# Intsights/PySubstringSearch

Hardware: AMD Instinct MI355X
Metric: queries/sec (batched) + index-build GB/s on 512MB chunk, 1/2/4/8 GPU (higher is better)
Workload: dtype u64

## Files before the change

### pysubstringsearch_amd/csrc/common.cpp

```cpp
#include "common.h"
#include "knobs.h"

#include <atomic>
#include <cstring>
#include <cstdio>
#include <cstdlib>
#include <algorithm>
#include <cerrno>
#include <unistd.h>

#include <mutex>
#include <vector>

namespace pss {

static thread_local std::string g_err;

void set_error(const char *fmt, ...)
{
    char buf[1024];
    va_list ap;
    va_start(ap, fmt);
    vsnprintf(buf, sizeof buf, fmt, ap);
    va_end(ap);
    g_err = buf;
}

const std::string &last_error() { return g_err; }

int DevBuf::reserve(size_t bytes)
{
    if (bytes <= cap) return PSS_OK;
    if (p) {
        (void)hipFree(p);
        p = nullptr;
        cap = 0;
    }
    size_t want = round_up(bytes, (size_t)1 << 20);
    hipError_t e = hipMalloc(&p, want);
    if (e != hipSuccess) {
        p = nullptr;
        set_error("hipMalloc(%zu bytes) failed: %s", want, hipGetErrorString(e));
        (void)hipGetLastError();
        return PSS_ENOMEM;
    }
    cap = want;
    return PSS_OK;
}

void DevBuf::release()
{
    if (p) (void)hipFree(p);
    p = nullptr;
    cap = 0;
}

int DeviceCtx::ensure_staging()
{
    if (stage[0]) return PSS_OK;
    PSS_HIP(hipStreamCreateWithFlags(&copy_stream, hipStreamNonBlocking));
    for (int i = 0; i < 2; ++i) {
        PSS_HIP(hipHostMalloc(&stage[i], kStage, hipHostMallocDefault));
        PSS_HIP(hipEventCreateWithFlags(&stage_ev[i], hipEventDisableTiming));
    }
    return PSS_OK;
}

int DeviceCtx::ensure_io_ring()
{
    PSS_TRY(ensure_staging());
    if (io_ring[0]) return PSS_OK;
    for (int i = 0; i < kIoPieces; ++i) {
        PSS_HIP(hipHostMalloc(&io_ring[i], kIoPiece, hipHostMallocPortable));
        PSS_HIP(hipEventCreateWithFlags(&io_ev[i], hipEventDisableTiming));
    }
    return PSS_OK;
}

IoPool &IoPool::get()
{
    static IoPool pool;
    return pool;
}

IoPool::IoPool()
{
    int k = 0;
    if (const char *e = knob("PSS_IO_THREADS")) k = atoi(e);
    if (k <= 0) {
        const unsigned hw = std::thread::hardware_concurrency();
        k = (int)std::min<unsigned>(16u, std::max<unsigned>(8u, hw / 8));
    }
    if (k > 64) k = 64;
    for (int i = 0; i < k; ++i) workers_.emplace_back([this] { run(); });
}

IoPool::~IoPool()
{
    {
        std::lock_guard<std::mutex> lk(mu_);
        stop_ = true;
    }
    cv_.notify_all();
    for (auto &t : workers_)
        if (t.joinable()) t.join();
}

void IoPool::submit(Batch *b, int fd, bool write, void *buf, size_t len, int64_t off, std::atomic<int> *done)
{
    {
        std::lock_guard<std::mutex> lk(b->mu);
        b->submitted += 1;
    }
    if (done) done->store(0, std::memory_order_relaxed);
    {
        std::lock_guard<std::mutex> lk(mu_);
        q_.push_back(Task{b, fd, write, buf, len, off, done});
    }
    cv_.notify_one();
}

void IoPool::submit_copy(Batch *b, void *dst, const void *src, size_t len, std::atomic<int> *done)
{
    submit(b, -2, true, dst, len, (int64_t)reinterpret_cast<intptr_t>(src), done);
}

void IoPool::run()
{
    for (;;) {
        Task t;
        {
            std::unique_lock<std::mutex> lk(mu_);
            cv_.wait(lk, [&] { return stop_ || !q_.empty(); });
            if (q_.empty()) return;
            t = q_.front();
            q_.pop_front();
        }
        int err = 0;
        size_t at = 0;
        uint8_t *p = static_cast<uint8_t *>(t.buf);
        if (t.fd == -2) {
            memcpy(t.buf, reinterpret_cast<const void *>((intptr_t)t.off), t.len);
            at = t.len;
        }
        while (at < t.len) {
            const ssize_t k = t.write ? pwrite(t.fd, p + at, t.len - at, (off_t)(t.off + (int64_t)at))
                                      : pread(t.fd, p + at, t.len - at, (off_t)(t.off + (int64_t)at));
            if (k < 0) {
                if (errno == EINTR) continue;
                err = errno ? errno : EIO;
                break;
            }
            if (k == 0) {
                err = t.write ? ENOSPC : ENODATA;
                break;
            }
            at += (size_t)k;
        }
        {
            std::lock_guard<std::mutex> lk(t.b->mu);
            if (err && !t.b->err) t.b->err = err;
            t.b->finished += 1;
            if (t.done) t.done->store(1, std::memory_order_release);
            t.b->cv.notify_all();
        }
    }
}

int IoPool::wait_all(Batch *b)
{
    std::unique_lock<std::mutex> lk(b->mu);
    b->cv.wait(lk, [&] { return b->finished == b->submitted; });
    return b->err;
}

void IoPool::wait_flag(Batch *b, std::atomic<int> *done)
{
    std::unique_lock<std::mutex> lk(b->mu);
    b->cv.wait(lk, [&] { return done->load(std::memory_order_acquire) != 0; });
}

int DeviceCtx::ensure_search_stage()
{
    if (search_stage) return PSS_OK;
    PSS_HIP(hipHostMalloc(&search_stage, kStageQ + kStageR, hipHostMallocDefault));
    return PSS_OK;
}

void SearchKnobs::load()
{
    *this = SearchKnobs{};
    no_small_path = knob("PSS_NO_SMALL_PATH") != nullptr;
    no_block_path = knob("PSS_NO_BLOCK_PATH") != nullptr;
    no_search_stage = knob("PSS_NO_SEARCH_STAGE") != nullptr;
    wave_search = knob("PSS_WAVE_SEARCH") != nullptr;
    no_group_search = knob("PSS_NO_GROUP_SEARCH") != nullptr;
    no_mid_pipeline = knob("PSS_NO_MID_PIPELINE") != nullptr;
    no_pinned_results = knob("PSS_NO_PINNED_RESULTS") != nullptr;
    small_path_events = knob("PSS_SEARCH_EVENTS") != nullptr;
    if (const char *e = knob("PSS_LANE_SEARCH_MIN")) lane_search_min = strtoull(e, nullptr, 0);
    if (const char *e = knob("PSS_ICASE_SEED_LETTERS")) icase_seed_letters = (uint32_t)std::min(6ul, std::max(1ul, strtoul(e, nullptr, 0)));
    if (const char *e = knob("PSS_RESIDENT_IDLE_US")) resident_idle_us = (uint32_t)strtoul(e, nullptr, 0);
    if (const char *e = knob("PSS_RESIDENT_LIFE_US")) resident_life_us = (uint32_t)strtoul(e, nullptr, 0);
}

static SearchKnobs g_knobs;
static std::once_flag g_knobs_once;
const SearchKnobs &search_knobs()
{
    std::call_once(g_knobs_once, []() { g_knobs.load(); });
    return g_knobs;
}
void reload_search_knobs()
{
    (void)search_knobs();
    g_knobs.load();
}

namespace {
struct PinnedBlock {
    void *p;
    size_t bytes;
};
std::mutex g_pool_mu;
std::vector<PinnedBlock> g_pool;
constexpr size_t kPoolMaxBlocks = 24;
size_t pool_max_bytes()
{
    static const size_t v = [] {
        const char *e = knob("PSS_PINNED_POOL_BYTES");
        return e ? (size_t)strtoull(e, nullptr, 0) : ((size_t)40 << 30);
    }();
    return v;
}
}

void *pinned_pool_alloc(size_t bytes, size_t *granted)
{
    {
        std::lock_guard<std::mutex> lk(g_pool_mu);
        int best = -1;
        for (int i = 0; i < (int)g_pool.size(); ++i)
            if (g_pool[i].bytes >= bytes && (best < 0 || g_pool[i].bytes < g_pool[best].bytes)) best = i;
        if (best >= 0 && g_pool[best].bytes <= 2 * bytes + ((size_t)64 << 20)) {
            PinnedBlock b = g_pool[best];
            g_pool.erase(g_pool.begin() + best);
            *granted = b.bytes;
            return b.p;
        }
    }
    void *p = nullptr;
    const size_t want = round_up(bytes + bytes / 8, (size_t)2 << 20);
    if (hipHostMalloc(&p, want, hipHostMallocPortable) != hipSuccess) {
        (void)hipGetLastError();
        return nullptr;
    }
    *granted = want;
    return p;
}

void pinned_pool_free(void *p, size_t granted)
{
    if (!p) return;
    std::vector<PinnedBlock> drop;
    bool kept = false;
    {
        std::lock_guard<std::mutex> lk(g_pool_mu);
        size_t held = 0;
        for (const auto &b : g_pool) held += b.bytes;
        if (granted <= pool_max_bytes()) {
            while (!g_pool.empty() && (g_pool.size() >= kPoolMaxBlocks || held + granted > pool_max_bytes())) {
                size_t k = 0;
                for (size_t i = 1; i < g_pool.size(); ++i)
                    if (g_pool[i].bytes < g_pool[k].bytes) k = i;
                held -= g_pool[k].bytes;
                drop.push_back(g_pool[k]);
                g_pool.erase(g_pool.begin() + (long)k);
            }
            g_pool.push_back({p, granted});
            kept = true;
        }
    }
    for (auto &b : drop) (void)hipHostFree(b.p);
    if (!kept) (void)hipHostFree(p);
}

void pinned_pool_trim()
{
    std::vector<PinnedBlock> drop;
    {
        std::lock_guard<std::mutex> lk(g_pool_mu);
        drop.swap(g_pool);
    }
    for (auto &b : drop) (void)hipHostFree(b.p);
}

static constexpr int kMaxDevices = 64;
static DeviceCtx g_ctx[kMaxDevices];
static DeviceCtx g_bctx[kMaxDevices];
static std::mutex g_ctx_mu;

static int init_ctx(DeviceCtx &c, int device)
{
    PSS_HIP(hipStreamCreateWithFlags(&c.stream, hipStreamNonBlocking));
    hipDeviceProp_t prop;
    PSS_HIP(hipGetDeviceProperties(&prop, device));
    c.num_cus = prop.multiProcessorCount > 0 ? prop.multiProcessorCount : 256;
    c.pinned_cap = DeviceCtx::kPinnedBytes;
    PSS_HIP(hipHostMalloc(&c.pinned, c.pinned_cap, hipHostMallocDefault));
    PSS_HIP(hipHostGetDevicePointer(&c.pinned_dev, c.pinned, 0));
    for (hipEvent_t &e : c.search_ev) PSS_HIP(hipEventCreate(&e));
    c.device = device;
    return PSS_OK;
}

static int get_ctx_of(DeviceCtx *table, int device, DeviceCtx **out)
{
    int count = 0;
    hipError_t e = hipGetDeviceCount(&count);
    if (e != hipSuccess || count <= 0) {
        (void)hipGetLastError();
        set_error("no usable HIP device (%s); libpss has no CPU fallback",
                  e != hipSuccess ? hipGetErrorString(e) : "device count is 0");
        return PSS_EDEVICE;
    }
    if (device < 0 || device >= count || device >= kMaxDevices) {
        set_error("device %d out of range (have %d)", device, count);
        return PSS_EINVAL;
    }
    PSS_HIP(hipSetDevice(device));
    std::lock_guard<std::mutex> lk(g_ctx_mu);
    DeviceCtx &c = table[device];
    if (c.device < 0) PSS_TRY(init_ctx(c, device));
    *out = &c;
    return PSS_OK;
}

int get_helper_ctx(DeviceCtx *parent, DeviceCtx **out)
{
    if (!parent->helper) {
        DeviceCtx *h = new DeviceCtx();
        const int rc = init_ctx(*h, parent->device);
        if (rc != PSS_OK) {
            delete h;
            return rc;
        }
        parent->helper = h;
    }
    *out = parent->helper;
    return PSS_OK;
}

int get_ctx(int device, DeviceCtx **out) { return get_ctx_of(g_ctx, device, out); }
int get_build_ctx(int device, DeviceCtx **out) { return get_ctx_of(g_bctx, device, out); }

int DeviceCtx::ensure_resident()
{
    if (resident.arena) return PSS_OK;
    PSS_HIP(hipStreamCreateWithFlags(&resident.stream, hipStreamNonBlocking));
    PSS_HIP(hipHostMalloc(&resident.arena, kPinnedBytes, hipHostMallocCoherent | hipHostMallocMapped));
    PSS_HIP(hipHostGetDevicePointer(&resident.arena_dev, resident.arena, 0));
    memset(resident.arena, 0, kPinnedBytes);
    return PSS_OK;
}

void DeviceCtx::Resident::post(const uint8_t *q, uint32_t plen)
{
    ResidentMailbox *mb = reinterpret_cast<ResidentMailbox *>(static_cast<uint8_t *>(arena) + kResidentMailboxOff);
    if (plen != kResidentStop) {
        if (plen <= sizeof mb->post.bytes) {
            memcpy(mb->post.bytes, q, plen);
        } else {
            memcpy(mb->query, q, plen);
            memset(mb->query + plen, 0, 32);
        }
    }
    mb->post.plen = plen;
    ++seq;
    __atomic_store_n(&mb->post.seq_b, seq, __ATOMIC_RELEASE);
    __atomic_store_n(&mb->post.seq_a, seq, __ATOMIC_RELEASE);
}

void DeviceCtx::stop_resident()
{
    if (!resident.running) return;
    resident.post(nullptr, kResidentStop);
    (void)hipStreamSynchronize(resident.stream);
    resident.running = false;
}

const KnobDef kKnobs[] = {
    {"PSS_KEY_CHARS", "0 (chosen)", "1|2|3|5|8|12|16", "builder: force the symbols packed into the initial sort key"},
    {"PSS_KEY_DROP", "-1 (chosen)", "0|1|3|7", "builder: force the low bits of the last key symbol that are left out"},
    {"PSS_NO_SAMPLE", "unset", "1", "builder: size the initial key from symbol counts even for large texts (no sizing sample)"},
    {"PSS_NO_TIES_PASS", "unset", "1", "builder: plain 8-byte-key LSD passes and key comparison in the rerank (no tie flags)"},
    {"PSS_MODE", "chosen", "dense|sparse|text", "builder: how ties are resolved -- doubling over an inverse suffix array, sparse (hash), text rounds"},
    {"PSS_TEXT_ROUNDS", "5", "0|1|2|3", "builder: text rounds at most before the rank rounds"},
    {"PSS_MSD", "-1 (screened)", "0|1|1", "initial sort: never / whenever the key fits the hybrid MSD radix sort (msd_sort.hip)"},
    {"PSS_MSD_LSD", "1", "0|1", "MSD sort: 0 = digits in MSD order with a second histogram pass (rounds 2-5); else LSD order, second pass by look-back"},
    {"PSS_MSD_KEY_CAP", "48", "", "MSD sort: largest key width tried (bits; the element format bounds it further)"},
    {"PSS_MSD_PARTIAL_SYMBOL", "unset", "1", "MSD sort: fill the element with the high bits of one more symbol than fits whole (fewer ties; measured slower on lines)"},
    {"PSS_MSD_NO_FUSE", "unset", "1", "MSD sort: ties flagged in the suffix array instead of emitted from the local sort"},
    {"PSS_MSD_NO_FINISH", "unset", "1", "MSD sort: small tie groups go to the rounds instead of being finished by one more text key after the local sort"},
    {"PSS_MSD_SLOW_LOCAL", "unset", "1", "MSD sort: the general (ballot LSD) local-sort kernel for every tile"},
    {"PSS_MSD_SCATTER", "unset", "1", "MSD sort in MSD order: the 8192-element partition kernels of round 2"},
    {"PSS_SS", "-1 (n >= 2^24, MSD declined)", "0|1", "initial sort: never / whenever the text has the size for it the sample sort over 16-byte elements"},
    {"PSS_SS_SEG", "1", "0", "sample sort: 0 = every tile merge-sorted as one array instead of bucket by bucket"},
    {"PSS_SS_WINDOW_PLAN", "unset", "1", "sample sort: tiles by the window rule of the MSD sort instead of the greedy plan"},
    {"PSS_SS_DEBUG", "unset", "", "sample sort: print where a bucket beyond a tile came from (diagnostic)"},
    {"PSS_NO_PLAN_CACHE", "unset", "1", "builder: forget between chunks which initial sort and alphabet the previous chunk took"},
    {"PSS_NO_PLAN_FRONT", "unset", "1", "builder: remember the sort but not the alphabet (separate alphabet and recode passes)"},
    {"PSS_RLE", "-1 (runs average >= 8 bytes)", "0|1|1", "builder: never / always the run-length path (rle_build.hip)"},
    {"PSS_RLE_SORT", "unset", "1", "run-length path: expansion by the stable radix sort instead of the matrix walk"},
    {"PSS_PERIOD", "-1 (when the text repeats one word)", "0", "builder: 0 = never the closed form for a text that repeats one word"},
    {"PSS_ANCHOR", "-1 (texts of >= 2^20 bytes)", "0|1|1", "builder: never / whenever ties outlive the text rounds the anchor round (anchor_impl.h)"},
    {"PSS_ANCHOR_OMEGA", "0 (as wide as the common prefix allows)", "9|12|17|33", "anchor round: force the window of the minimizers"},
    {"PSS_ANCHOR_MIN_OMEGA", "11", "3|7|9", "anchor round: narrowest window it accepts by itself"},
    {"PSS_ANCHOR_SIDE", "-1 (>= 2^24 bytes, sampled ties show copies)", "0|1", "anchor round: never / always sort the anchors beside the text round (second stream)"},
    {"PSS_ANCHOR_SIDE_PCT", "8", "", "anchor round: share of sampled tied pairs that must be copies for the side line"},
    {"PSS_ANCHOR_CAP_DIV", "5", "3|4", "anchor round: declines above n / this many anchors"},
    {"PSS_NO_PROBE", "unset", "1", "builder: always a text round before the anchor round (no sampling of the ties)"},
    {"PSS_PROBE_SKIP_PCT", "50", "0|20|90", "builder: no text rounds when more than this share of the sampled tied pairs are repeats"},
    {"PSS_NO_MID_TIER", "unset", "1", "rounds: groups above 512 members all take the chained radix sorts"},
    {"PSS_NO_MID_MERGE", "unset", "1", "rounds: groups of 513 .. 4096 members with a crowded bin take the chained sorts (no LDS merge sort)"},
    {"PSS_BIG_MERGE", "-1 (by the average size of the large groups)", "0|1|2", "rounds: groups above 4096 members through the segmented merge sort (2: in text rounds only)"},
    {"PSS_NO_BIG_MERGE", "unset", "", "rounds: overrides PSS_BIG_MERGE"},
    {"PSS_COUNT_SORT", "unset", "1", "rank rounds: groups ranked by counting instead of the merge sort"},
    {"PSS_PERIODIC", "1", "0", "rank rounds: 0 = no periodic keys for the large groups"},
    {"PSS_TIMING", "unset", "", "builder / Writer: per-round and per-stage trace on stderr"},
    {"PSS_DEVICES", "all visible", "0|0,0|0,0,0|all", "devices of Reader(path) / Writer(path) without a device argument: all | comma-separated ordinals"},
    {"PSS_DEVICE", "unset", "", "default device of a process (launchers' LOCAL_RANK etc. are honoured the same way)"},
    {"PSS_IO_THREADS", "8 .. 16 by core count", "2|5", "file path: threads of the I/O pool"},
    {"PSS_INGEST_BLOCK", "32 MiB", "16|40|300", "Writer: size of the direct reads of add_entries_from_file_lines"},
    {"PSS_INGEST_MIN_ROOM", "1 MiB", "1|20", "Writer: room a chunk must have left for one direct read"},
    {"PSS_WRITER_MMAP", "tmpfs: 1, else 0", "0|1", "Writer: records through a shared mapping (1) or pwrite (0)"},
    {"PSS_WRITER_MMAP_MIN", "1 MiB", "16", "Writer: smallest record that goes through the mapping"},
    {"PSS_WRITER_HOST_BUDGET", "8 GiB", "", "multi-device Writer: host text of the chunks in flight (one chunk always goes through)"},
    {"PSS_STRIPES", "8", "", "striped container format 2: stripe files of a Writer"},
    {"PSS_EXPERIMENT_NO_FILE", "unset", "", "measurement only: the record thread copies without writing the file"},
    {"PSS_RESULT_ORDER", "text", "sa", "Reader: 'sa' = the reference's order inside a chunk (suffix-array order of every entry's first hit)"},
    {"PSS_READER_HBM_BUDGET", "whatever hipMalloc grants minus 2 GiB", "", "Reader: suffix arrays beyond this many bytes of HBM stay in pinned host memory"},
    {"PSS_READER_AUTO_RESIDENCY", "1", "", "Reader: 0 = the residency manager never moves a suffix array by itself"},
    {"PSS_NO_KEY_SAMPLES", "unset", "", "Reader: no key-sample table"},
    {"PSS_SAMPLE_SHIFT", "11", "", "Reader: one key sample per 2^shift suffixes"},
    {"PSS_LINE_BLOCK_SHIFT", "8", "6|7|9|10", "Reader: the line index behind entry ids keeps one newline rank per 2^shift bytes of text (6 .. 10)"},
    {"PSS_NO_SMALL_PATH", "unset", "1", "search: no fused single-query kernels"},
    {"PSS_NO_BLOCK_PATH", "unset", "1", "search: small batches one wave per pair instead of one workgroup"},
    {"PSS_NO_SEARCH_STAGE", "unset", "1", "search: no pinned staging of queries and results"},
    {"PSS_WAVE_SEARCH", "unset", "1", "search: interval kernel one wave per pair at every batch size"},
    {"PSS_NO_GROUP_SEARCH", "unset", "1", "search: never 16 lanes per pair"},
    {"PSS_NO_MID_PIPELINE", "unset", "1", "search: always the general multi-kernel pipeline"},
    {"PSS_PINNED_POOL_BYTES", "40 GiB", "", "search: pinned host memory the result pool keeps between batches"},
    {"PSS_NO_PINNED_RESULTS", "unset", "1", "search: large results into pageable memory"},
    {"PSS_LANE_SEARCH_MIN", "8192", "1|100000", "search: pairs from which one lane per pair searches"},
    {"PSS_ICASE_SEED_LETTERS", "5", "1|2|3|4|5|6", "case-insensitive search: ASCII letters of a pattern's seed at most (2^letters spellings probed per pattern and chunk)"},
    {"PSS_SEARCH_EVENTS", "unset", "", "single-query path: HIP events around the fused kernel (fills ms_device; ~4 us per query)"},
    {"PSS_RESIDENT_IDLE_US", "1000", "", "low-latency mode: the resident kernel leaves after this long without a query"},
    {"PSS_RESIDENT_LIFE_US", "50000", "", "low-latency mode: ... and after this long in any case"},
    {"PSS_TRACE_RESIDENT", "unset", "", "libpss_trace.so only: print the resident kernel's phase stamps"},
    {"PSS_RCCL_LIB", "librccl.so of the process", "", "gather inside the C ABI: the RCCL library to load"},
    {"PSS_RCCL_TIMEOUT_MS", "60000", "", "gather inside the C ABI: bound of every wait for the peers"},
};
const int kNumKnobs = (int)(sizeof(kKnobs) / sizeof(kKnobs[0]));

const char *knob(const char *name)
{
    for (int i = 0; i < kNumKnobs; ++i)
        if (strcmp(kKnobs[i].name, name) == 0) return getenv(name);
    static std::atomic<bool> said{false};
    if (!said.exchange(true)) fprintf(stderr, "[pss] %s is not in the switch registry (knobs.h): treated as unset\n", name);
    return nullptr;
}

uint64_t workspace_bytes(int device)
{
    if (device < 0 || device >= kMaxDevices) return 0;
    std::lock_guard<std::mutex> lk(g_ctx_mu);
    uint64_t total = 0;
    for (DeviceCtx *table : {g_ctx, g_bctx}) {
        DeviceCtx &c = table[device];
        if (c.device < 0) continue;
        for (auto &s : c.slot) total += s.cap;
        if (c.helper)
            for (auto &s : c.helper->slot) total += s.cap;
    }
    return total;
}

void trim_all()
{
    std::vector<DeviceCtx *> live;
    {
        std::lock_guard<std::mutex> lk(g_ctx_mu);
        for (DeviceCtx *table : {g_ctx, g_bctx})
            for (int d = 0; d < kMaxDevices; ++d)
                if (table[d].device >= 0) live.push_back(&table[d]);
    }
    for (DeviceCtx *cp : live) {
        {
            DeviceCtx &c = *cp;
            std::lock_guard<std::recursive_mutex> lk2(c.mu);
            (void)hipSetDevice(c.device);
            c.stop_resident();
            for (auto &s : c.slot) s.release();
            if (c.helper)
                for (auto &s : c.helper->slot) s.release();
            c.small_hdr_ready = nullptr;
        }
    }
    pinned_pool_trim();
}

}
```

### pysubstringsearch_amd/csrc/common.h

```cpp
#pragma once
#include <hip/hip_runtime.h>

#include <cstdarg>
#include <cstddef>
#include <cstdint>
#include <cstdio>
#include <cstdlib>
#include <cstring>
#include <atomic>
#include <condition_variable>
#include <deque>
#include <mutex>
#include <string>
#include <thread>
#include <vector>

#include "../../include/pss.h"

#include "knobs.h"

namespace pss {

void set_error(const char *fmt, ...);
const std::string &last_error();

#define PSS_HIP(expr)                                                                   \
    do {                                                                                \
        hipError_t _e = (expr);                                                         \
        if (_e != hipSuccess) {                                                         \
            pss::set_error("%s failed: %s (%s:%d)", #expr, hipGetErrorString(_e), __FILE__, __LINE__); \
            return (_e == hipErrorOutOfMemory) ? PSS_ENOMEM : PSS_EDEVICE;              \
        }                                                                               \
    } while (0)

#define PSS_TRY(expr)               \
    do {                            \
        int _rc = (expr);           \
        if (_rc != PSS_OK) return _rc; \
    } while (0)

struct DevBuf {
    void *p = nullptr;
    size_t cap = 0;
    int reserve(size_t bytes);
    void release();
    template <typename T> T *as() const { return static_cast<T *>(p); }
};

struct SearchKnobs {
    bool no_small_path = false;
    bool no_block_path = false;
    bool no_search_stage = false;
    bool wave_search = false;
    bool no_group_search = false;
    bool no_mid_pipeline = false;
    bool no_pinned_results = false;
    bool small_path_events = false;
    uint64_t lane_search_min = 8192;
    uint32_t icase_seed_letters = 5;
    uint32_t resident_idle_us = 1000;
    uint32_t resident_life_us = 50000;
    void load();
};
const SearchKnobs &search_knobs();
void reload_search_knobs();

void *pinned_pool_alloc(size_t bytes, size_t *granted);
void pinned_pool_free(void *p, size_t granted);
void pinned_pool_trim();

struct ResidentMailbox {
    struct Post {
        volatile uint32_t seq_a;
        volatile uint32_t plen;
        uint8_t bytes[52];
        volatile uint32_t seq_b;
    } post;
    uint8_t query[256 + 64];
    volatile uint64_t done_seq_echo;
    volatile uint32_t exited;
    volatile uint32_t closing;
    volatile uint32_t pad2[12];
};
static_assert(offsetof(ResidentMailbox, done_seq_echo) % 8 == 0, "one aligned 8-byte store");
static inline uint32_t resident_query_checksum(const uint8_t *q, uint32_t plen)
{
    uint32_t h = 0x811C9DC5u ^ plen;
    for (uint32_t i = 0; i < plen; i += 8) {
        uint64_t w = 0;
        for (uint32_t k = 0; k < 8 && i + k < plen; ++k) w |= (uint64_t)q[i + k] << (8 * k);
        h = (h ^ (uint32_t)w) * 0x01000193u;
        h = (h ^ (uint32_t)(w >> 32)) * 0x01000193u;
    }
    return h;
}
static_assert(sizeof(ResidentMailbox::Post) == 64, "the posted line is one cache line");
constexpr uint32_t kResidentStop = 0xffffffffu;

struct DeviceCtx {
    std::recursive_mutex mu;
    int device = -1;
    hipStream_t stream = nullptr;
    int num_cus = 256;
    static constexpr int kSlots = 57;
    DevBuf slot[kSlots];
    static constexpr size_t kPinnedBytes = (size_t)640 << 10;
    void *pinned = nullptr;
    size_t pinned_cap = 0;
    void *pinned_dev = nullptr;
    static constexpr size_t kStageQ = (size_t)2 << 20, kStageR = (size_t)4 << 20;
    void *search_stage = nullptr;
    int ensure_search_stage();
    hipEvent_t search_ev[3] = {nullptr, nullptr, nullptr};
    void *small_hdr_ready = nullptr;
    struct Resident {
        hipStream_t stream = nullptr;
        void *arena = nullptr, *arena_dev = nullptr;
        bool running = false;
        const void *chunks = nullptr;
        uint32_t nc = 0, spread = 0;
        void *d_arena = nullptr;
        uint32_t seq = 0;
        uint64_t launches = 0, served = 0, torn = 0;
        void post(const uint8_t *q, uint32_t plen);
    } resident;
    static constexpr size_t kResidentMailboxOff = 24576;
    int ensure_resident();
    void stop_resident();
    uint32_t plan_present[8] = {};
    uint32_t plan_logn = 0;
    int plan_path = 0;
    uint8_t plan_lut[256] = {};
    uint32_t plan_sigma = 0;
    uint64_t ss_plan_tag = 0;
    uint32_t ss_plan_radix = 0;
    bool ss_refused_note = false;
    uint32_t ss_plan_skip = 0, ss_plan_backoff = 0;
    uint64_t side_plan_heff = 0;
    uint32_t side_plan_logn = 0;
    int side_plan_b = 0;
    double restart_ms = 0.0;
    int restart_depth = 0;
    static constexpr size_t kStage = (size_t)64 << 20;
    void *stage[2] = {nullptr, nullptr};
    hipStream_t copy_stream = nullptr;
    hipEvent_t stage_ev[2] = {nullptr, nullptr};
    int ensure_staging();
    static constexpr size_t kIoPiece = (size_t)16 << 20;
    static constexpr int kIoPieces = 12;
    void *io_ring[kIoPieces] = {};
    hipEvent_t io_ev[kIoPieces] = {};
    int ensure_io_ring();
    DeviceCtx *helper = nullptr;
};
int get_helper_ctx(DeviceCtx *parent, DeviceCtx **out);

class IoPool {
public:
    struct Batch {
        std::mutex mu;
        std::condition_variable cv;
        size_t submitted = 0, finished = 0;
        int err = 0;
    };
    static IoPool &get();
    void submit(Batch *b, int fd, bool write, void *buf, size_t len, int64_t off, std::atomic<int> *done = nullptr);
    void submit_copy(Batch *b, void *dst, const void *src, size_t len, std::atomic<int> *done = nullptr);
    static int wait_all(Batch *b);
    static void wait_flag(Batch *b, std::atomic<int> *done);
    int threads() const { return (int)workers_.size(); }
    ~IoPool();

private:
    IoPool();
    struct Task {
        Batch *b;
        int fd;
        bool write;
        void *buf;
        size_t len;
        int64_t off;
        std::atomic<int> *done;
    };
    void run();
    std::mutex mu_;
    std::condition_variable cv_;
    std::deque<Task> q_;
    bool stop_ = false;
    std::vector<std::thread> workers_;
};

int get_ctx(int device, DeviceCtx **out);
int get_build_ctx(int device, DeviceCtx **out);
void trim_all();
uint64_t workspace_bytes(int device);

static inline size_t round_up(size_t x, size_t a) { return (x + a - 1) / a * a; }

}
```

### pysubstringsearch_amd/csrc/msd_sort.h

```cpp
#pragma once
#include "common.h"
#include "radix_sort.h"

namespace pss {

struct MsdStats {
    uint32_t buckets = 0;
    uint32_t max_bucket = 0;
    uint32_t tiles = 0;
    uint32_t slow_tiles = 0;
    uint32_t bad_symbol = 0;
    uint32_t lookback = 0;
    uint32_t finished = 0;
    double ms_g1 = 0, ms_g2 = 0, ms_local = 0;
};

constexpr int MSD_FIN_MAX = 4;
struct MsdActive {
    uint32_t *pos, *idx, *grp;
    uint32_t *st_pos, *st_idx;
    uint32_t count = 0;
};

size_t msd_workspace_bytes(uint32_t n);
int msd_max_key_bits(uint32_t n);

struct MsdFront {
    const uint8_t *raw;
    const uint8_t *lut;
    uint32_t *bad;
};
int msd_suffix_sort(DeviceCtx *ctx, const TextKeys *text, uint32_t n, int key_bits, uint64_t *A[2], uint32_t *sa_out,
                    void *work, uint32_t *h_small, bool profile, MsdStats *stats, bool *accepted, MsdActive *active = nullptr,
                    const MsdFront *front = nullptr);


struct SsStats {
    uint32_t buckets = 0, max_bucket = 0, tiles = 0;
    uint32_t b1 = 0, b2 = 0, samples = 0;
    int key_chars = 0;
    double ms_sample = 0, ms_g1 = 0, ms_g2 = 0, ms_local = 0;
};
struct SsBuffers {
    void *A[2];
    uint16_t *digits;
    void *E0, *E;
    uint64_t *K[2];
    uint32_t *V[2];
    void *sort_work;
    const void *sample_in = nullptr;
    void *sample_keep = nullptr;
};
uint32_t ss_sample_count(uint32_t n);
int ss_key_chars(uint32_t n, uint32_t radix);
uint64_t ss_geometry_tag(uint32_t n, uint32_t radix);
int ss_suffix_sort(DeviceCtx *ctx, const TextKeys *text, uint32_t radix, uint32_t n, const SsBuffers &buf, uint32_t *sa_out,
                   void *work, uint32_t *h_small, bool profile, SsStats *stats, bool *accepted, MsdActive *active);

}
```

### pysubstringsearch_amd/csrc/msd_sort.hip

```cpp
#include "msd_sort.h"

#include <algorithm>
#include <vector>

#include "prims.h"
#include "scan.h"
#include "text_keys.h"

namespace pss {

constexpr int MSD_D = 10;
constexpr u32 MSD_BINS = 1u << MSD_D;
constexpr int MSD_BLOCK = 512;
constexpr int MSD_WAVES = MSD_BLOCK / kWave;
constexpr int MSD_IPT = 16;
constexpr u32 MSD_TILE = MSD_BLOCK * MSD_IPT;
constexpr u32 MSD_WIN = 6144;
#ifndef PSS_LS_WINDOW
#define PSS_LS_WINDOW 8
#endif
constexpr u32 MSD_TILE_CAP = 8184 - PSS_LS_WINDOW;
constexpr u32 MSD_MAX_BUCKET = 4088;
constexpr int MSD_TAG_BITS = MSD_D + 1;
constexpr u32 MSD_TAG_SPAN = 1u << MSD_TAG_BITS;
constexpr int MSD_RAW_TAG_BITS = 6;
constexpr u32 MSD_RAW_TAG_SPAN = 1u << MSD_RAW_TAG_BITS;
constexpr u32 MSD_G1_RANGES = 1024;
constexpr u32 MSD_G2_RANGE = 16 * MSD_TILE;

struct MsdRange {
    u32 seg, start, end;
};

struct MsdTile2 {
    u32 start, count, d_last;
};

struct MsdArgs {
    const u8 *codes;
    int code_bits, key_chars, plus_one, key_drop;
    u32 n;
    int key_bits;
    int idx_bits;
    u32 tiles_per_range1, num_ranges1;
    u32 *T;
    u32 *J1;
    u32 *J;
    MsdRange *ranges2;
    u32 *seg_first;
    u32 *counters;
    const u64 *dense;
    const u64 *in;
    u64 *out;
    int lsd;
    u32 *T2;
    const u32 *Jb;
    const struct MsdTile2 *tiles2;
    u32 *status;
    const u8 *raw;
    const u8 *lut;
    u8 *codes_out;
    u32 *bad;
};


template <bool FROM_TEXT>
__device__ __forceinline__ void msd_load_tile(const MsdArgs &a, u32 base, u32 valid, u64 (&elem)[MSD_IPT], u32 (&dig)[MSD_IPT],
                                              int shift2)
{
    const u32 tid = threadIdx.x;
    if (FROM_TEXT) {
        const u32 i0 = base + tid * MSD_IPT;
        u64 key[MSD_IPT] = {};
        if (i0 < a.n) text_keys16(a.codes, i0, a.code_bits, a.key_chars, a.plus_one, a.key_drop, a.n, key);
        const int rest_bits = a.key_bits - MSD_D;
        const u64 rest_mask = (1ull << rest_bits) - 1ull;
#pragma unroll
        for (int r = 0; r < MSD_IPT; ++r) {
            dig[r] = (u32)(key[r] >> rest_bits) & (MSD_BINS - 1u);
            elem[r] = ((key[r] & rest_mask) << a.idx_bits) | (u64)(i0 + r);
        }
    } else {
#pragma unroll
        for (int r = 0; r < MSD_IPT; ++r) {
            const u32 p = r * MSD_BLOCK + tid;
            elem[r] = p < valid ? a.in[base + p] : 0ull;
            dig[r] = (u32)(elem[r] >> shift2) & (MSD_BINS - 1u);
        }
    }
}

template <bool FROM_TEXT>
__device__ __forceinline__ bool msd_valid(u32 base, u32 valid, int r, u32 n)
{
    const u32 tid = threadIdx.x;
    (void)base;
    (void)n;
    return FROM_TEXT ? (tid * MSD_IPT + r < valid) : (r * MSD_BLOCK + tid < valid);
}

template <bool FROM_TEXT>
__global__ __launch_bounds__(MSD_BLOCK) void msd_hist_kernel(MsdArgs a)
{
    __shared__ u32 hist[MSD_BINS];
    __shared__ u32 histb[FROM_TEXT ? MSD_BINS : 1];
    const u32 tid = threadIdx.x, r = blockIdx.x;
    u32 e0, e1;
    if (FROM_TEXT) {
        if (r >= a.num_ranges1) return;
        e0 = r * a.tiles_per_range1 * MSD_TILE;
        const u64 end = (u64)(r + 1) * a.tiles_per_range1 * MSD_TILE;
        e1 = end < a.n ? (u32)end : a.n;
    } else {
        if (r >= a.counters[0]) return;
        e0 = a.ranges2[r].start;
        e1 = a.ranges2[r].end;
    }
    for (u32 i = tid; i < MSD_BINS; i += MSD_BLOCK) {
        hist[i] = 0;
        if (FROM_TEXT) histb[i] = 0;
    }
    __syncthreads();
    const int shift2 = a.idx_bits + a.key_bits - 2 * MSD_D;
    if (FROM_TEXT) {
        const int b = a.code_bits;
        const int top = a.lsd ? 2 * MSD_D : MSD_D;
        const int m = (top + b - 1) / b;
        const u32 wmask = (m * b >= 32) ? ~0u : ((1u << (m * b)) - 1u);
        const int down = m * b - top;
        uint4 nlo = make_uint4(0, 0, 0, 0), nhi = nlo;
        if (e0 + tid * MSD_IPT < e1) {
            const uint4 *p = reinterpret_cast<const uint4 *>(a.codes + e0 + tid * MSD_IPT);
            nlo = p[0];
            nhi = p[1];
        }
        for (u32 base = e0; base < e1; base += MSD_TILE) {
            const u32 i0 = base + tid * MSD_IPT;
            const uint4 lo = nlo, hi = nhi;
            if ((u64)i0 + MSD_TILE < e1) {
                const uint4 *p = reinterpret_cast<const uint4 *>(a.codes + i0 + MSD_TILE);
                nlo = p[0];
                nhi = p[1];
            }
            if (i0 >= e1) continue;
            const u64 q[4] = {(u64)lo.x | ((u64)lo.y << 32), (u64)lo.z | ((u64)lo.w << 32),
                              (u64)hi.x | ((u64)hi.y << 32), (u64)hi.z | ((u64)hi.w << 32)};
            auto sym = [&](u32 j) -> u32 { return (u32)(q[j >> 3] >> ((j & 7u) * 8u)) & 0xffu; };
            u32 win = 0;
            for (int t = 0; t < m; ++t) win = (win << b) | sym((u32)t);
#pragma unroll
            for (int r = 0; r < MSD_IPT; ++r) {
                if (r > 0) win = ((win << b) | sym((u32)(m - 1 + r))) & wmask;
                if (i0 + r < e1) {
                    const u32 tp = win >> down;
                    atomicAdd(&hist[tp & (MSD_BINS - 1u)], 1u);
                    if (a.lsd) atomicAdd(&histb[tp >> MSD_D], 1u);
                }
            }
        }
    } else {
        for (u32 base = e0; base < e1; base += MSD_TILE) {
            const u32 valid = min(MSD_TILE, e1 - base);
            u64 elem[MSD_IPT];
            u32 dig[MSD_IPT];
            msd_load_tile<FROM_TEXT>(a, base, valid, elem, dig, shift2);
#pragma unroll
            for (int k = 0; k < MSD_IPT; ++k)
                if (msd_valid<FROM_TEXT>(base, valid, k, a.n)) atomicAdd(&hist[dig[k]], 1u);
        }
    }
    __syncthreads();
    for (u32 i = tid; i < MSD_BINS; i += MSD_BLOCK) {
        if (FROM_TEXT) {
            a.T[(size_t)i * a.num_ranges1 + r] = hist[i];
            if (a.lsd) a.T2[(size_t)i * a.num_ranges1 + r] = histb[i];
        } else {
            a.T[(size_t)r * MSD_BINS + i] = hist[i];
        }
    }
}

__global__ __launch_bounds__(MSD_BLOCK) void msd_hist_raw_kernel(MsdArgs a)
{
    __shared__ u32 hist[MSD_BINS];
    __shared__ u32 histb[MSD_BINS];
    __shared__ u8 s_lut[256];
    const u32 tid = threadIdx.x, r = blockIdx.x;
    if (r >= a.num_ranges1) return;
    const u32 e0 = r * a.tiles_per_range1 * MSD_TILE;
    const u64 end = (u64)(r + 1) * a.tiles_per_range1 * MSD_TILE;
    const u32 e1 = end < a.n ? (u32)end : a.n;
    for (u32 i = tid; i < MSD_BINS; i += MSD_BLOCK) hist[i] = histb[i] = 0;
    if (tid < 256) s_lut[tid] = a.lut[tid];
    __syncthreads();
    const int b = a.code_bits;
    const int top = a.lsd ? 2 * MSD_D : MSD_D;
    const int m = (top + b - 1) / b;
    const u32 wmask = (m * b >= 32) ? ~0u : ((1u << (m * b)) - 1u);
    const int down = m * b - top;
    auto tr = [&](u32 w) -> u32 {
        return (u32)s_lut[w & 0xffu] | ((u32)s_lut[(w >> 8) & 0xffu] << 8) | ((u32)s_lut[(w >> 16) & 0xffu] << 16) |
               ((u32)s_lut[w >> 24] << 24);
    };
    auto load32 = [&](u32 i, uint4 &lo, uint4 &hi) {
        if ((u64)i + 32 <= a.n) {
            const uint4 *p = reinterpret_cast<const uint4 *>(a.raw + i);
            lo = p[0];
            hi = p[1];
        } else {
            u32 w[8] = {};
            for (u32 k = 0; k < 32 && i + k < a.n; ++k) w[k >> 2] |= (u32)a.raw[i + k] << (8u * (k & 3u));
            lo = make_uint4(w[0], w[1], w[2], w[3]);
            hi = make_uint4(w[4], w[5], w[6], w[7]);
        }
    };
    bool bad = false;
    uint4 nlo = make_uint4(0, 0, 0, 0), nhi = nlo;
    if (e0 + tid * MSD_IPT < e1) load32(e0 + tid * MSD_IPT, nlo, nhi);
    for (u32 base = e0; base < e1; base += MSD_TILE) {
        const u32 i0 = base + tid * MSD_IPT;
        uint4 lo = nlo, hi = nhi;
        if ((u64)i0 + MSD_TILE < e1) load32(i0 + MSD_TILE, nlo, nhi);
        if (i0 >= e1) continue;
        lo = make_uint4(tr(lo.x), tr(lo.y), tr(lo.z), tr(lo.w));
        if (m <= 5) hi = make_uint4(tr(hi.x), 0u, 0u, 0u);
        else hi = make_uint4(tr(hi.x), tr(hi.y), tr(hi.z), tr(hi.w));
        const u32 own = min(16u, a.n - i0);
        if (own == 16) {
            *reinterpret_cast<uint4 *>(a.codes_out + i0) = lo;
            const u32 z = ((lo.x - 0x01010101u) & ~lo.x) | ((lo.y - 0x01010101u) & ~lo.y) | ((lo.z - 0x01010101u) & ~lo.z) |
                          ((lo.w - 0x01010101u) & ~lo.w);
            bad |= (z & 0x80808080u) != 0;
        } else {
            const u32 w[4] = {lo.x, lo.y, lo.z, lo.w};
            for (u32 k = 0; k < own; ++k) {
                const u8 c = (u8)(w[k >> 2] >> (8u * (k & 3u)));
                a.codes_out[i0 + k] = c;
                bad |= c == 0;
            }
            u32 ww[8] = {lo.x, lo.y, lo.z, lo.w, hi.x, hi.y, hi.z, hi.w};
            for (u32 k = own; k < 32; ++k) ww[k >> 2] &= ~(0xffu << (8u * (k & 3u)));
            lo = make_uint4(ww[0], ww[1], ww[2], ww[3]);
            hi = make_uint4(ww[4], ww[5], ww[6], ww[7]);
        }
        if (own == 16 && (u64)i0 + 32 > a.n) {
            u32 ww[4] = {hi.x, hi.y, hi.z, hi.w};
            for (u32 k = 0; k < 16; ++k)
                if (i0 + 16 + k >= a.n) ww[k >> 2] &= ~(0xffu << (8u * (k & 3u)));
            hi = make_uint4(ww[0], ww[1], ww[2], ww[3]);
        }
        const u64 q[4] = {(u64)lo.x | ((u64)lo.y << 32), (u64)lo.z | ((u64)lo.w << 32),
                          (u64)hi.x | ((u64)hi.y << 32), (u64)hi.z | ((u64)hi.w << 32)};
        auto sym = [&](u32 j) -> u32 { return (u32)(q[j >> 3] >> ((j & 7u) * 8u)) & 0xffu; };
        u32 win = 0;
        for (int t = 0; t < m; ++t) win = (win << b) | sym((u32)t);
#pragma unroll
        for (int k = 0; k < MSD_IPT; ++k) {
            if (k > 0) win = ((win << b) | sym((u32)(m - 1 + k))) & wmask;
            if (i0 + k < e1) {
                const u32 tp = win >> down;
                atomicAdd(&hist[tp & (MSD_BINS - 1u)], 1u);
                if (a.lsd) atomicAdd(&histb[tp >> MSD_D], 1u);
            }
        }
    }
    if (__ballot(bad) && (tid & 63u) == 0) atomicOr(a.bad, 1u);
    __syncthreads();
    for (u32 i = tid; i < MSD_BINS; i += MSD_BLOCK) {
        a.T[(size_t)i * a.num_ranges1 + r] = hist[i];
        if (a.lsd) a.T2[(size_t)i * a.num_ranges1 + r] = histb[i];
    }
}

__global__ __launch_bounds__(256) void msd_offsets1_kernel(u32 *T, u32 num_ranges, u32 *totals)
{
    __shared__ u32 scr[256 / kWave + 1];
    const u32 d = blockIdx.x, tid = threadIdx.x;
    u32 *row = T + (size_t)d * num_ranges;
    u32 v[4], sum = 0;
#pragma unroll
    for (int j = 0; j < 4; ++j) {
        const u32 r = tid * 4 + j;
        v[j] = r < num_ranges ? row[r] : 0u;
        sum += v[j];
    }
    u32 total = 0;
    u32 run = block_excl_sum<256 / kWave>(sum, scr, &total);
#pragma unroll
    for (int j = 0; j < 4; ++j) {
        const u32 r = tid * 4 + j;
        if (r < num_ranges) row[r] = run;
        run += v[j];
    }
    if (tid == 0) totals[d] = total;
}
__global__ __launch_bounds__(MSD_BINS) void msd_offsets1b_kernel(const u32 *totals, u32 *J1, u32 n)
{
    __shared__ u32 scr[MSD_BINS / kWave + 1];
    const u32 d = threadIdx.x;
    J1[d] = block_excl_sum<MSD_BINS / kWave>(totals[d], scr, nullptr);
    if (d == 0) J1[MSD_BINS] = n;
}

__global__ __launch_bounds__(MSD_BINS) void msd_offsets_kernel(u32 *T, const u32 *seg_first, const u32 *seg_start, u32 *joint,
                                                                u32 num_ranges_fixed, u32 n, u32 nseg)
{
    __shared__ u32 scr[MSD_BINS / kWave + 1];
    const u32 seg = blockIdx.x, d = threadIdx.x;
    const u32 r0 = seg_first ? seg_first[seg] : 0u;
    const u32 r1 = seg_first ? seg_first[seg + 1] : num_ranges_fixed;
    const u32 base = seg_start ? seg_start[seg] : 0u;
    u32 run = 0;
    for (u32 r = r0; r < r1; ++r) {
        const u32 c = T[(size_t)r * MSD_BINS + d];
        T[(size_t)r * MSD_BINS + d] = run;
        run += c;
    }
    const u32 binbase = base + block_excl_sum<MSD_BINS / kWave>(run, scr, nullptr);
    joint[(size_t)seg * MSD_BINS + d] = binbase;
    if (seg == nseg - 1 && d == 0) joint[(size_t)nseg * MSD_BINS] = n;
    for (u32 r = r0; r < r1; ++r) T[(size_t)r * MSD_BINS + d] += binbase;
}

__global__ __launch_bounds__(MSD_BINS) void msd_ranges_kernel(const u32 *J1, MsdRange *ranges, u32 *seg_first, u32 *counters)
{
    __shared__ u32 scr[MSD_BINS / kWave + 1];
    const u32 seg = threadIdx.x;
    const u32 s = J1[seg], e = J1[seg + 1];
    const u32 nr = (e - s + MSD_G2_RANGE - 1) / MSD_G2_RANGE;
    u32 total = 0;
    const u32 first = block_excl_sum<MSD_BINS / kWave>(nr, scr, &total);
    seg_first[seg] = first;
    if (seg == MSD_BINS - 1) seg_first[MSD_BINS] = total;
    if (seg == 0) counters[0] = total;
    for (u32 k = 0; k < nr; ++k) {
        const u32 rs = s + k * MSD_G2_RANGE;
        ranges[first + k] = MsdRange{seg, rs, min(e, rs + MSD_G2_RANGE)};
    }
}

template <bool FROM_TEXT>
__global__ __launch_bounds__(MSD_BLOCK, 4) void msd_scatter_kernel(MsdArgs a)
{
    __shared__ __attribute__((aligned(16))) u64 exch[MSD_TILE];
    __shared__ u32 hist[MSD_BINS], s_delta[MSD_BINS], s_off[MSD_BINS];
    __shared__ u16 s_start[MSD_BINS];
    __shared__ u32 scr[MSD_WAVES + 1];
    const u32 tid = threadIdx.x, r = blockIdx.x;
    u32 e0, e1;
    u32 tag0 = 0, tag1 = 0;
    if (FROM_TEXT) {
        if (r >= a.num_ranges1) return;
        e0 = r * a.tiles_per_range1 * MSD_TILE;
        const u64 end = (u64)(r + 1) * a.tiles_per_range1 * MSD_TILE;
        e1 = end < a.n ? (u32)end : a.n;
    } else {
        if (r >= a.counters[0]) return;
        e0 = a.ranges2[r].start;
        e1 = a.ranges2[r].end;
        const u64 *dn = a.dense + (size_t)a.ranges2[r].seg * MSD_BINS;
        tag0 = ((u32)dn[2 * tid] & (MSD_TAG_SPAN - 1u)) << 16;
        tag1 = ((u32)dn[2 * tid + 1] & (MSD_TAG_SPAN - 1u)) << 16;
        hist[2 * tid] = tag0;
        hist[2 * tid + 1] = tag1;
    }
    for (u32 i = tid; i < MSD_BINS; i += MSD_BLOCK) {
        if (FROM_TEXT) hist[i] = 0;
        s_off[i] = FROM_TEXT ? a.T[(size_t)i * a.num_ranges1 + r] + a.J1[i] : a.T[(size_t)r * MSD_BINS + i];
    }
    __syncthreads();
    const int shift2 = a.idx_bits + a.key_bits - 2 * MSD_D;
    const u64 low_mask2 = (1ull << shift2) - 1ull;
    for (u32 base = e0; base < e1; base += MSD_TILE) {
        const u32 valid = min(MSD_TILE, e1 - base);
        u64 elem[MSD_IPT];
        u32 dig[MSD_IPT];
        u32 rank[MSD_IPT];
        msd_load_tile<FROM_TEXT>(a, base, valid, elem, dig, shift2);
#pragma unroll
        for (int k = 0; k < MSD_IPT; ++k)
            rank[k] = msd_valid<FROM_TEXT>(base, valid, k, a.n) ? (atomicAdd(&hist[dig[k]], 1u) & 0xffffu) : 0u;
        __syncthreads();
        {
            const u32 c0 = hist[2 * tid] & 0xffffu, c1 = hist[2 * tid + 1] & 0xffffu;
            const u32 ex = block_excl_sum<MSD_WAVES>(c0 + c1, scr, nullptr);
            s_start[2 * tid] = (u16)ex;
            s_start[2 * tid + 1] = (u16)(ex + c0);
            const u32 o0 = s_off[2 * tid], o1 = s_off[2 * tid + 1];
            s_delta[2 * tid] = o0 - ex;
            s_delta[2 * tid + 1] = o1 - (ex + c0);
            s_off[2 * tid] = o0 + c0;
            s_off[2 * tid + 1] = o1 + c1;
            hist[2 * tid] = tag0;
            hist[2 * tid + 1] = tag1;
        }
        __syncthreads();
#pragma unroll
        for (int k = 0; k < MSD_IPT; ++k) {
            if (msd_valid<FROM_TEXT>(base, valid, k, a.n)) {
                const u32 lp = (u32)s_start[dig[k]] + rank[k];
                if (FROM_TEXT) exch[lp] = ((elem[k] >> a.idx_bits) << 23) | ((u64)dig[k] << 13) | (u64)(tid * MSD_IPT + k);
                else exch[lp] = elem[k];
            }
        }
        __syncthreads();
#pragma unroll
        for (int k = 0; k < MSD_IPT; ++k) {
            const u32 p = k * MSD_BLOCK + tid;
            if (p < valid) {
                u64 e = exch[p];
                u32 d;
                if (FROM_TEXT) {
                    d = (u32)(e >> 13) & (MSD_BINS - 1u);
                    e = ((e >> 23) << a.idx_bits) | (u64)(base + ((u32)e & (MSD_TILE - 1u)));
                } else {
                    d = (u32)(e >> shift2) & (MSD_BINS - 1u);
                    e = (e & low_mask2) | ((u64)(hist[d] >> 16) << shift2);
                }
                a.out[s_delta[d] + p] = e;
            }
        }
    }
}

constexpr u32 MSD_TILE2 = 16384;
constexpr int MSD_PIECES2 = MSD_TILE2 / MSD_TILE;

template <bool FROM_TEXT, int BLOCK, bool LSD = false>
__global__ __launch_bounds__(BLOCK) void msd_scatter2_kernel(MsdArgs a)
{
    constexpr int IPT = MSD_TILE2 / BLOCK;
    constexpr int BPT = MSD_BINS / BLOCK;
    __shared__ __attribute__((aligned(16))) u64 exch[MSD_TILE];
    __shared__ u32 hist[MSD_BINS], s_delta[MSD_BINS], s_off[MSD_BINS];
    __shared__ u16 s_start[MSD_BINS];
    __shared__ u32 scr[BLOCK / kWave + 1];
    const u32 tid = threadIdx.x, r = blockIdx.x;
    u32 e0, e1;
    u32 tag[BPT];
#pragma unroll
    for (int j = 0; j < BPT; ++j) tag[j] = 0;
    if (FROM_TEXT) {
        if (r >= a.num_ranges1) return;
        e0 = r * a.tiles_per_range1 * MSD_TILE;
        const u64 end = (u64)(r + 1) * a.tiles_per_range1 * MSD_TILE;
        e1 = end < a.n ? (u32)end : a.n;
    } else {
        if (r >= a.counters[0]) return;
        e0 = a.ranges2[r].start;
        e1 = a.ranges2[r].end;
#pragma unroll
        for (int j = 0; j < BPT; ++j)
            tag[j] = ((u32)a.dense[(size_t)a.ranges2[r].seg * MSD_BINS + BPT * tid + j] & (MSD_TAG_SPAN - 1u)) << 16;
    }
#pragma unroll
    for (int j = 0; j < BPT; ++j) {
        const u32 i = BPT * tid + j;
        hist[i] = tag[j];
        s_off[i] = FROM_TEXT ? a.T[(size_t)i * a.num_ranges1 + r] + a.J1[i] : a.T[(size_t)r * MSD_BINS + i];
    }
    __syncthreads();
    const int shift2 = a.idx_bits + a.key_bits - 2 * MSD_D;
    const u64 low_mask2 = (1ull << shift2) - 1ull;
    const int rest_bits = a.key_bits - MSD_D;
    const u64 rest_mask = (1ull << rest_bits) - 1ull;
    for (u32 base = e0; base < e1; base += MSD_TILE2) {
        const u32 valid = min(MSD_TILE2, e1 - base);
        u64 elem[IPT];
        u32 lp[IPT];
        if (FROM_TEXT) {
#pragma unroll
            for (int g = 0; g < IPT / 16; ++g) {
                const u32 i0 = base + tid * IPT + g * 16;
                u64 key[16] = {};
                if (i0 < a.n) text_keys16(a.codes, i0, a.code_bits, a.key_chars, a.plus_one, a.key_drop, a.n, key);
#pragma unroll
                for (int k = 0; k < 16; ++k) {
                    const u32 pos = tid * IPT + g * 16 + k;
                    u32 d;
                    u64 keep;
                    if (LSD) {
                        d = (u32)(key[k] >> (rest_bits - MSD_D)) & (MSD_BINS - 1u);
                        keep = ((key[k] >> rest_bits) << (rest_bits - MSD_D)) | (key[k] & (rest_mask >> MSD_D));
                    } else {
                        d = (u32)(key[k] >> rest_bits) & (MSD_BINS - 1u);
                        keep = key[k] & rest_mask;
                    }
                    elem[g * 16 + k] = (keep << 24) | ((u64)d << 14) | (u64)pos;
                    lp[g * 16 + k] = pos < valid ? ((atomicAdd(&hist[d], 1u) & 0xffffu) | (d << 22)) : 0xffffffffu;
                }
            }
        } else {
#pragma unroll
            for (int k = 0; k < IPT; ++k) {
                const u32 p = k * BLOCK + tid;
                elem[k] = p < valid ? a.in[base + p] : 0ull;
            }
#pragma unroll
            for (int k = 0; k < IPT; ++k) {
                const u32 p = k * BLOCK + tid;
                const u32 d = (u32)(elem[k] >> shift2) & (MSD_BINS - 1u);
                lp[k] = p < valid ? ((atomicAdd(&hist[d], 1u) & 0xffffu) | (d << 22)) : 0xffffffffu;
            }
        }
        __syncthreads();
        {
            u32 c[BPT], sum = 0;
#pragma unroll
            for (int j = 0; j < BPT; ++j) {
                c[j] = hist[BPT * tid + j] & 0xffffu;
                sum += c[j];
            }
            u32 ex = block_excl_sum<BLOCK / kWave>(sum, scr, nullptr);
#pragma unroll
            for (int j = 0; j < BPT; ++j) {
                const u32 i = BPT * tid + j;
                s_start[i] = (u16)ex;
                const u32 o = s_off[i];
                s_delta[i] = o - ex;
                s_off[i] = o + c[j];
                hist[i] = tag[j];
                ex += c[j];
            }
        }
        __syncthreads();
#pragma unroll
        for (int k = 0; k < IPT; ++k)
            if (lp[k] != 0xffffffffu) lp[k] = (lp[k] & 0xffffu) + (u32)s_start[lp[k] >> 22];
#pragma unroll
        for (int h = 0; h < MSD_PIECES2; ++h) {
            if (h * MSD_TILE >= valid) break;
            if (h) __syncthreads();
#pragma unroll
            for (int k = 0; k < IPT; ++k) {
                const u32 q = lp[k] - h * MSD_TILE;
                if (q < MSD_TILE) exch[q] = elem[k];
            }
            __syncthreads();
#pragma unroll
            for (int k = 0; k < (int)(MSD_TILE / BLOCK); ++k) {
                const u32 q = k * BLOCK + tid, p = h * MSD_TILE + q;
                if (p < valid) {
                    u64 e = exch[q];
                    u32 d;
                    if (FROM_TEXT) {
                        d = (u32)(e >> 14) & (MSD_BINS - 1u);
                        e = ((e >> 24) << a.idx_bits) | (u64)(base + ((u32)e & (MSD_TILE2 - 1u)));
                    } else {
                        d = (u32)(e >> shift2) & (MSD_BINS - 1u);
                        e = (e & low_mask2) | ((u64)(hist[d] >> 16) << shift2);
                    }
                    a.out[s_delta[d] + p] = e;
                }
            }
        }
    }
}

constexpr u32 LB_A = 1u << 30, LB_P = 2u << 30, LB_STATE = 3u << 30, LB_VALUE = LB_A - 1u;
constexpr int LB_WINDOW = 4;

struct LbAsk {
    u32 v[LB_WINDOW];
};
__device__ __forceinline__ void lb_ask(const u32 *status, u32 p, LbAsk &q)
{
#pragma unroll
    for (u32 w = 0; w < (u32)LB_WINDOW; ++w) {
        const u32 r = p > w ? p - 1 - w : 0u;
        q.v[w] = __hip_atomic_load(&status[(size_t)r * MSD_BINS + threadIdx.x], __ATOMIC_RELAXED, __HIP_MEMORY_SCOPE_AGENT);
    }
}
__device__ __forceinline__ void lb_begin(u32 *status, u32 t, u32 c, LbAsk &q)
{
    if (t == 0) return;
    __hip_atomic_store(&status[(size_t)t * MSD_BINS + threadIdx.x], LB_A | c, __ATOMIC_RELAXED, __HIP_MEMORY_SCOPE_AGENT);
    lb_ask(status, t, q);
}
__device__ __forceinline__ u32 lb_finish(u32 *status, u32 t, u32 c, u32 first, LbAsk &q)
{
    u32 off = first;
    if (t != 0) {
        u32 sum = 0, p = t;
        for (;;) {
            const u32 p0 = p;
            bool stop = false, done = false;
#pragma unroll
            for (u32 w = 0; w < (u32)LB_WINDOW; ++w) {
                if (!stop && w < p0) {
                    const u32 st = q.v[w] & LB_STATE;
                    if (st == 0) {
                        stop = true;
                    } else {
                        sum += q.v[w] & LB_VALUE;
                        --p;
                        if (st == LB_P) done = stop = true;
                    }
                }
            }
            if (done || p == 0) break;
            lb_ask(status, p, q);
        }
        off = sum;
    }
    __hip_atomic_store(&status[(size_t)t * MSD_BINS + threadIdx.x], LB_P | (off + c), __ATOMIC_RELAXED, __HIP_MEMORY_SCOPE_AGENT);
    return off;
}


__global__ __launch_bounds__(MSD_BINS) void msd_tiles2_kernel(const u32 *J1, MsdTile2 *tiles, u32 *counters)
{
    __shared__ u32 scr[MSD_BINS / kWave + 1];
    const u32 d = threadIdx.x;
    const u32 s = J1[d], e = J1[d + 1];
    const u32 nr = (e - s + MSD_TILE2 - 1) / MSD_TILE2;
    u32 total = 0, D = 0;
    const u32 first = block_excl_sum<MSD_BINS / kWave>(nr, scr, &total);
    const u32 dn = block_excl_sum<MSD_BINS / kWave>(nr ? 1u : 0u, scr, &D);
    if (d == 0) counters[0] = total + (MSD_BINS - D);
    if (nr == 0) {
        const u32 dd = D + (d - dn);
        tiles[total + (d - dn)] = MsdTile2{s, 0u, dd | 0x80000000u};
    }
    for (u32 k = 0; k < nr; ++k) {
        const u32 ts = s + k * MSD_TILE2;
        tiles[first + k] = MsdTile2{ts, min(MSD_TILE2, e - ts), dn | (k + 1 == nr ? 0x80000000u : 0u)};
    }
}

__global__ __launch_bounds__(1024) void msd_scatter_lb_kernel(MsdArgs a)
{
    constexpr int BLOCK = 1024;
    constexpr int IPT = MSD_TILE2 / BLOCK;
    __shared__ __attribute__((aligned(16))) u64 exch[MSD_TILE];
    __shared__ u32 hist[MSD_BINS], s_delta[MSD_BINS];
    __shared__ u16 s_start[MSD_BINS];
    __shared__ u32 scr[BLOCK / kWave + 1];
    __shared__ u32 s_ticket;
    const u32 tid = threadIdx.x;
    const u32 nt = a.counters[0];
    const int shift2 = a.idx_bits + a.key_bits - 2 * MSD_D;
    const u64 low_mask2 = (1ull << shift2) - 1ull;
    hist[tid] = 0;
    __syncthreads();
    for (;;) {
        if (tid == 0) s_ticket = atomicAdd(&a.counters[8], 1u);
        __syncthreads();
        const u32 t = s_ticket;
        if (t >= nt) break;
        const MsdTile2 td = a.tiles2[t];
        const u32 base = td.start, valid = td.count;
        u64 elem[IPT];
        u32 lp[IPT];
#pragma unroll
        for (int k = 0; k < IPT; ++k) {
            const u32 p = k * BLOCK + tid;
            elem[k] = p < valid ? a.in[base + p] : 0ull;
        }
#pragma unroll
        for (int k = 0; k < IPT; ++k) {
            const u32 p = k * BLOCK + tid;
            const u32 d = (u32)(elem[k] >> shift2) & (MSD_BINS - 1u);
            lp[k] = p < valid ? (atomicAdd(&hist[d], 1u) | (d << 22)) : 0xffffffffu;
        }
        __syncthreads();
        const u32 c = hist[tid];
        LbAsk ask;
        lb_begin(a.status, t, c, ask);
        const u32 ex = block_excl_sum<BLOCK / kWave>(c, scr, nullptr);
        s_start[tid] = (u16)ex;
        hist[tid] = 0;
        __syncthreads();
        const u64 tag = (u64)(td.d_last & (MSD_RAW_TAG_SPAN - 1u)) << shift2;
#pragma unroll
        for (int k = 0; k < IPT; ++k)
            if (lp[k] != 0xffffffffu) lp[k] = (lp[k] & 0xffffu) + (u32)s_start[lp[k] >> 22];
#pragma unroll
        for (int h = 0; h < MSD_PIECES2; ++h) {
            if (h && h * MSD_TILE >= valid) break;
            if (h) __syncthreads();
#pragma unroll
            for (int k = 0; k < IPT; ++k) {
                const u32 q = lp[k] - h * MSD_TILE;
                if (q < MSD_TILE) exch[q] = elem[k];
            }
            if (h == 0) {
                if (t == 0 && tid == 0) a.J[0] = 0;
                const u32 off = lb_finish(a.status, t, c, a.Jb[tid], ask);
                if (td.d_last >> 31) a.J[(size_t)tid * MSD_BINS + (td.d_last & (MSD_BINS - 1u)) + 1u] = off + c;
                s_delta[tid] = off - ex;
            }
            __syncthreads();
#pragma unroll
            for (int k = 0; k < (int)(MSD_TILE / BLOCK); ++k) {
                const u32 q = k * BLOCK + tid, p = h * MSD_TILE + q;
                if (p < valid) {
                    const u64 e = exch[q];
                    const u32 d = (u32)(e >> shift2) & (MSD_BINS - 1u);
                    a.out[s_delta[d] + p] = (e & low_mask2) | tag;
                }
            }
        }
    }
}


struct InNonEmpty {
    const u32 *J;
    __device__ u64 operator()(u64 j) const { return J[j + 1] > J[j] ? 1u : 0u; }
};

__global__ __launch_bounds__(256) void msd_compact_kernel(const u32 *J, u32 nb, const u64 *rank, u32 *cstart, u32 *counters, u32 *cj)
{
    u32 mx = 0;
    for (u32 j = blockIdx.x * blockDim.x + threadIdx.x; j < nb; j += gridDim.x * blockDim.x) {
        const u32 s = J[j], e = J[j + 1];
        if (e > s) {
            cstart[rank[j]] = s;
            if (cj) cj[rank[j]] = j;
            mx = max(mx, e - s);
        }
    }
    mx = wave_incl_max(mx);
    if (lane_id() == kWave - 1 && mx) atomicMax(&counters[1], mx);
}

struct TilePlan {
    u32 win, cap;
    const u32 *cj;
};
__device__ __forceinline__ bool msd_tile_head(const u32 *cstart, u32 ne, u32 n, u32 k, TilePlan tp)
{
    if (tp.cj) {
        if (k == 0 || (tp.cj[k] >> MSD_RAW_TAG_BITS) != (tp.cj[k - 1] >> MSD_RAW_TAG_BITS)) return true;
    } else if ((k & (MSD_TAG_SPAN - 1u)) == 0) {
        return true;
    }
    const u32 w = cstart[k] / tp.win;
    if (cstart[k - 1] / tp.win != w) return true;
    if (k + 1 < ne && cstart[k + 1] / tp.win == w) return false;
    u32 lo = 0, hi = k;
    const u32 ws = w * tp.win;
    while (lo < hi) {
        const u32 mid = (lo + hi) >> 1;
        if (cstart[mid] < ws) lo = mid + 1; else hi = mid;
    }
    const u32 end = k + 1 < ne ? cstart[k + 1] : n;
    return end - cstart[lo] > tp.cap;
}

struct InTileHead {
    const u32 *cstart;
    u32 ne, n;
    TilePlan tp;
    __device__ u64 operator()(u64 k) const { return msd_tile_head(cstart, ne, n, (u32)k, tp) ? 1u : 0u; }
};

struct InTileHeadDev {
    const u32 *cstart;
    const u64 *nep;
    u32 n;
    TilePlan tp;
    __device__ u64 operator()(u64 k) const
    {
        const u32 ne = (u32)*nep;
        return (k < ne && msd_tile_head(cstart, ne, n, (u32)k, tp)) ? 1u : 0u;
    }
};
__global__ __launch_bounds__(256) void msd_tiles_dev_kernel(const u32 *cstart, const u64 *nep, u32 n, const u64 *rank, const u64 *total,
                                                              u32 *tile_first, TilePlan tp)
{
    const u32 ne = (u32)*nep;
    if (blockIdx.x == 0 && threadIdx.x == 0) tile_first[*total] = ne;
    for (u32 k = blockIdx.x * blockDim.x + threadIdx.x; k < ne; k += gridDim.x * blockDim.x) {
        if (msd_tile_head(cstart, ne, n, k, tp)) tile_first[rank[k]] = k;
    }
}

__global__ __launch_bounds__(256) void msd_tiles_kernel(const u32 *cstart, u32 ne, u32 n, const u64 *rank, const u64 *total,
                                                          u32 *tile_first, TilePlan tp)
{
    if (blockIdx.x == 0 && threadIdx.x == 0) tile_first[*total] = ne;
    for (u32 k = blockIdx.x * blockDim.x + threadIdx.x; k < ne; k += gridDim.x * blockDim.x) {
        if (msd_tile_head(cstart, ne, n, k, tp)) tile_first[rank[k]] = k;
    }
}

struct MsdTile {
    u32 e0, count, tag0, nb;
};


struct MsdEmit {
    u32 *st_pos, *st_idx;
    u32 *blk_cnt;
};

__device__ __forceinline__ void msd_emit_tile(const u64 *exch, u32 count, u32 e0, int idx_bits, u32 *sa_out, const MsdEmit *em,
                                              u32 *s_count)
{
    const u32 tid = threadIdx.x, lane = tid & 63u;
    const u32 imask = (u32)((1ull << idx_bits) - 1ull);
    const u32 rows = (count + MSD_BLOCK - 1) / MSD_BLOCK;
#pragma unroll 1
    for (u32 r = 0; r < rows; ++r) {
        const u32 p = r * MSD_BLOCK + tid;
        const bool valid = p < count;
        u64 x = 0;
        bool tie = false;
        if (valid) {
            x = exch[p];
            tie = p > 0 && (exch[p - 1] >> idx_bits) == (x >> idx_bits);
            sa_out[e0 + p] = ((u32)x & imask) | ((tie && em == nullptr) ? 0x80000000u : 0u);
        }
        if (em != nullptr) {
            const u64 tm = __ballot(tie);
            const bool tie_next = lane < 63 ? ((tm >> (lane + 1)) & 1ull) != 0
                                            : (p + 1 < count && (exch[p + 1] >> idx_bits) == (x >> idx_bits));
            if (valid && (tie || tie_next)) {
                const u32 slot = e0 + atomicAdd(s_count, 1u);
                em->st_pos[slot] = e0 + p;
                em->st_idx[slot] = ((u32)x & imask) | (tie ? 0x80000000u : 0u);
            }
        }
    }
}

struct InBlkCnt {
    const u32 *c;
    __device__ u64 operator()(u64 t) const { return (u64)(c[t] & 0xffffu) | ((u64)(c[t] >> 16) << 32); }
};

constexpr u32 GA_WORDS = MSD_TILE / 32;
__global__ __launch_bounds__(256) void msd_gather_kernel(const MsdTile *tiles, const u32 *blk_cnt, const u64 *dst_off, u32 nt,
                                                           const u32 *st_pos, const u32 *st_idx, u32 *pos, u32 *idx, u32 *grp)
{
    __shared__ u32 s_occ[4][GA_WORDS], s_head[4][GA_WORDS], s_pre[4][GA_WORDS];
    const u32 w = wave_id(), lane = lane_id();
    const u32 t = blockIdx.x * 4 + w;
    if (t >= nt) return;
    const u32 c = blk_cnt[t] & 0xffffu;
    if (c == 0) return;
    const u32 e0 = tiles[t].e0;
    const u64 d = dst_off[t] & 0xffffffffull;
    u32 *occ = s_occ[w], *head = s_head[w], *pre = s_pre[w];
    for (u32 i = lane; i < GA_WORDS; i += kWave) occ[i] = head[i] = 0;
    __builtin_amdgcn_fence(__ATOMIC_ACQ_REL, "wavefront");
    __builtin_amdgcn_wave_barrier();
    for (u32 i = lane; i < c; i += kWave) {
        const u32 q = st_pos[e0 + i] - e0;
        atomicOr(&occ[q >> 5], 1u << (q & 31u));
        if (!(st_idx[e0 + i] >> 31)) atomicOr(&head[q >> 5], 1u << (q & 31u));
    }
    __builtin_amdgcn_fence(__ATOMIC_ACQ_REL, "wavefront");
    __builtin_amdgcn_wave_barrier();
    {
        const u32 c0 = __popc(occ[4 * lane]), c1 = __popc(occ[4 * lane + 1]), c2 = __popc(occ[4 * lane + 2]),
                  c3 = __popc(occ[4 * lane + 3]);
        const u32 ex = wave_incl_sum(c0 + c1 + c2 + c3) - (c0 + c1 + c2 + c3);
        pre[4 * lane] = ex;
        pre[4 * lane + 1] = ex + c0;
        pre[4 * lane + 2] = ex + c0 + c1;
        pre[4 * lane + 3] = ex + c0 + c1 + c2;
    }
    __builtin_amdgcn_fence(__ATOMIC_ACQ_REL, "wavefront");
    __builtin_amdgcn_wave_barrier();
    for (u32 i = lane; i < c; i += kWave) {
        const u32 ps = st_pos[e0 + i], q = ps - e0;
        const u32 below = (q & 31u) ? (occ[q >> 5] & ((1u << (q & 31u)) - 1u)) : 0u;
        const u32 rank = pre[q >> 5] + __popc(below);
        u32 wi = q >> 5;
        u32 m = head[wi] & ((q & 31u) == 31u ? ~0u : ((2u << (q & 31u)) - 1u));
        while (m == 0 && wi > 0) m = head[--wi];
        const u32 hq = wi * 32 + (31u - (u32)__builtin_clz(m | 1u));
        pos[d + rank] = ps;
        idx[d + rank] = st_idx[e0 + i] & 0x7fffffffu;
        grp[d + rank] = e0 + hq + 1;
    }
}


constexpr int FIN_MAX = MSD_FIN_MAX;
constexpr u32 FIN_WORDS = GA_WORDS + 2;
struct MsdFinish {
    const u8 *codes;
    int code_bits, key_syms, plus_one;
    u32 h0, n;
};

__global__ __launch_bounds__(256) void msd_finish_kernel(const MsdTile *tiles, u32 *blk_cnt, u32 nt, u32 *st_pos, u32 *st_idx,
                                                           u32 *sa_out, MsdFinish f)
{
    __shared__ u32 s_tie[4][FIN_WORDS], s_done[4][GA_WORDS];
    const u32 w = wave_id(), lane = lane_id();
    const u32 t = blockIdx.x * 4 + w;
    if (t >= nt) return;
    const u32 c = blk_cnt[t] & 0xffffu;
    const u32 e0 = tiles[t].e0;
    if (c == 0) return;
    u32 ps0 = 0, v0 = 0;
    if (lane < c) {
        ps0 = st_pos[e0 + lane];
        v0 = st_idx[e0 + lane];
    }
    auto record = [&](u32 i, u32 &ps, u32 &v) {
        if (i < (u32)kWave) {
            ps = ps0;
            v = v0;
        } else {
            ps = st_pos[e0 + i];
            v = st_idx[e0 + i];
        }
    };
    u32 *tie = s_tie[w], *done = s_done[w];
    for (u32 i = lane; i < FIN_WORDS; i += kWave) tie[i] = 0;
    for (u32 i = lane; i < GA_WORDS; i += kWave) done[i] = 0;
    __builtin_amdgcn_fence(__ATOMIC_ACQ_REL, "wavefront");
    __builtin_amdgcn_wave_barrier();
    for (u32 i = lane; i < c; i += kWave) {
        u32 ps, v;
        record(i, ps, v);
        const u32 q = ps - e0;
        if (v >> 31) atomicOr(&tie[q >> 5], 1u << (q & 31u));
    }
    __builtin_amdgcn_fence(__ATOMIC_ACQ_REL, "wavefront");
    __builtin_amdgcn_wave_barrier();
    bool settled = false;
    for (u32 i = lane; i < c; i += kWave) {
        u32 ps, v;
        record(i, ps, v);
        if (v >> 31) continue;
        const u32 q = ps - e0, a = q + 1u;
        const u64 win = (((u64)tie[(a >> 5) + 1u] << 32) | (u64)tie[a >> 5]) >> (a & 31u);
        const u32 g = win == ~0ull ? 65u : 1u + (u32)__builtin_ctzll(~win);
        if (g > (u32)FIN_MAX) continue;
        u32 sfx[FIN_MAX], rk[FIN_MAX];
        u64 key[FIN_MAX];
#pragma unroll
        for (int j = 0; j < FIN_MAX; ++j) {
            sfx[j] = 0;
            key[j] = 0;
            rk[j] = 0;
            if ((u32)j < g) {
                sfx[j] = j == 0 ? v : sa_out[ps + j];
                const u64 at = (u64)sfx[j] + f.h0;
                if (at < f.n) key[j] = text_key_at(f.codes, (u32)at, f.code_bits, f.key_syms, f.plus_one, f.n);
            }
        }
        bool same = false;
#pragma unroll
        for (int j = 0; j < FIN_MAX; ++j) {
#pragma unroll
            for (int l = j + 1; l < FIN_MAX; ++l) {
                if ((u32)l < g) {
                    same |= key[j] == key[l];
                    rk[l] += key[j] < key[l] ? 1u : 0u;
                    rk[j] += key[j] < key[l] ? 0u : 1u;
                }
            }
        }
        if (same) continue;
        settled = true;
#pragma unroll
        for (int j = 0; j < FIN_MAX; ++j) {
            if ((u32)j < g) {
                sa_out[ps + rk[j]] = sfx[j];
                atomicOr(&done[(q + j) >> 5], 1u << ((q + j) & 31u));
            }
        }
    }
    __builtin_amdgcn_fence(__ATOMIC_ACQ_REL, "wavefront");
    __builtin_amdgcn_wave_barrier();
    if (__ballot(settled) == 0) return;
    u32 kept = 0;
    for (u32 base = 0; base < c; base += kWave) {
        const u32 i = base + lane;
        u32 ps = 0, v = 0;
        bool keep = false;
        if (i < c) {
            record(i, ps, v);
            const u32 q = ps - e0;
            keep = ((done[q >> 5] >> (q & 31u)) & 1u) == 0;
        }
        const u64 km = __ballot(keep);
        __builtin_amdgcn_fence(__ATOMIC_ACQ_REL, "wavefront");
        __builtin_amdgcn_wave_barrier();
        if (keep) {
            const u32 o = e0 + kept + mbcnt(km);
            st_pos[o] = ps;
            st_idx[o] = v;
        }
        kept += (u32)__popcll(km);
    }
    if (lane == 0) blk_cnt[t] = kept | ((c - kept) << 16);
}


__global__ __launch_bounds__(MSD_BLOCK) void msd_local_sort_kernel(const u64 *in, const MsdTile *tiles, int rem_bits, int idx_bits,
                                                                     u32 *sa_out, const u32 *tile_list, int fused, MsdEmit em_val)
{
    const MsdEmit *em = fused ? &em_val : nullptr;
    __shared__ __attribute__((aligned(16))) u64 exch[MSD_TILE];
    __shared__ u32 wave_hist[MSD_WAVES][256];
    __shared__ u32 scr[MSD_WAVES + 1];
    const u32 tid = threadIdx.x, lane = tid & 63u, wave = tid >> 6;
    const u32 t = tile_list ? tile_list[blockIdx.x] : blockIdx.x;
    const MsdTile td = tiles[t];
    const u32 e0 = td.e0, count = td.count;
    for (u32 i = tid; i < MSD_WAVES * 256; i += MSD_BLOCK) (&wave_hist[0][0])[i] = 0;
    __syncthreads();
    int seg_bits = 0;
    while ((1u << seg_bits) < td.nb) ++seg_bits;
    const u64 tag_base = (u64)td.tag0 << (rem_bits + idx_bits);
    u64 key[MSD_IPT];
#pragma unroll
    for (int r = 0; r < MSD_IPT; ++r) {
        const u32 p = wave * (kWave * MSD_IPT) + r * kWave + lane;
        key[r] = p < count ? in[e0 + p] - tag_base : ~0ull;
    }
    const int sort_bits = rem_bits + seg_bits;
    for (int shift = idx_bits; shift < idx_bits + sort_bits; shift += 8) {
        const int left = idx_bits + sort_bits - shift;
        const u32 dmask = left >= 8 ? 0xffu : ((1u << left) - 1u);
        u32 rank[MSD_IPT], prev[MSD_IPT];
#pragma unroll
        for (int r = 0; r < MSD_IPT; ++r) {
            const bool pad = wave * (kWave * MSD_IPT) + r * kWave + lane >= count;
            const u32 d = pad ? dmask : ((u32)(key[r] >> shift) & dmask);
            const u64 peers = match_digit8(d, ~0ull);
            const u32 below = mbcnt(peers);
            prev[r] = 0;
            if (below == 0) prev[r] = atomicAdd(&wave_hist[wave][d], (u32)__popcll(peers));
            rank[r] = below | ((u32)__builtin_ctzll(peers) << 16);
        }
#pragma unroll
        for (int r = 0; r < MSD_IPT; ++r) rank[r] = __shfl(prev[r], (int)(rank[r] >> 16)) + (rank[r] & 0xffffu);
        __syncthreads();
        {
            u32 c[MSD_WAVES];
            u32 total = 0;
            if (tid < 256) {
#pragma unroll
                for (int w = 0; w < MSD_WAVES; ++w) {
                    c[w] = wave_hist[w][tid];
                    total += c[w];
                }
            }
            const u32 incl = wave_incl_sum(total);
            if (lane == kWave - 1) scr[wave] = incl;
            __syncthreads();
            if (tid < 256) {
                u32 run = incl - total;
                for (u32 w = 0; w < wave; ++w) run += scr[w];
#pragma unroll
                for (int w = 0; w < MSD_WAVES; ++w) {
                    wave_hist[w][tid] = run;
                    run += c[w];
                }
            }
        }
        __syncthreads();
#pragma unroll
        for (int r = 0; r < MSD_IPT; ++r) {
            const bool pad = wave * (kWave * MSD_IPT) + r * kWave + lane >= count;
            const u32 d = pad ? dmask : ((u32)(key[r] >> shift) & dmask);
            exch[wave_hist[wave][d] + rank[r]] = key[r];
        }
        __syncthreads();
        for (u32 i = tid; i < MSD_WAVES * 256; i += MSD_BLOCK) (&wave_hist[0][0])[i] = 0;
#pragma unroll
        for (int r = 0; r < MSD_IPT; ++r) key[r] = exch[wave * (kWave * MSD_IPT) + r * kWave + lane];
        __syncthreads();
    }
    if (sort_bits <= 0) {
#pragma unroll
        for (int r = 0; r < MSD_IPT; ++r) exch[wave * (kWave * MSD_IPT) + r * kWave + lane] = key[r];
        __syncthreads();
    }
    if (tid == 0) scr[0] = 0;
    __syncthreads();
    msd_emit_tile(exch, count, e0, idx_bits, sa_out, em, &scr[0]);
    __syncthreads();
    if (em && tid == 0) em->blk_cnt[t] = scr[0];
}


#ifndef PSS_LS_BIN_BITS
#define PSS_LS_BIN_BITS 12
#endif
constexpr int LS_BIN_BITS = PSS_LS_BIN_BITS;
constexpr u32 LS_BINS = 1u << LS_BIN_BITS;
constexpr u32 LS_WORDS = LS_BINS / 2;
constexpr u32 LS_KMAX = 64;
#ifndef PSS_LS_GROUP
#define PSS_LS_GROUP 1
#endif
constexpr int LS_GROUP = PSS_LS_GROUP;
constexpr int LS_WINDOW = PSS_LS_WINDOW;

__global__ __launch_bounds__(256) void msd_tile_desc_kernel(const u32 *cstart, const u32 *tile_first, u32 nt, u32 ne, u32 n,
                                                              MsdTile *tiles, const u32 *cj, const u64 *ntp, const u64 *nep)
{
    const u32 t = blockIdx.x * blockDim.x + threadIdx.x;
    if (ntp) {
        nt = (u32)*ntp;
        ne = (u32)*nep;
    }
    if (t >= nt) return;
    const u32 k0 = tile_first[t], k1 = tile_first[t + 1];
    const u32 e0 = cstart[k0], e1 = k1 < ne ? cstart[k1] : n;
    if (cj) {
        const u32 t0 = cj[k0] & (MSD_RAW_TAG_SPAN - 1u), t1 = cj[k1 - 1] & (MSD_RAW_TAG_SPAN - 1u);
        tiles[t] = MsdTile{e0, e1 - e0, t0, t1 - t0 + 1u};
    } else {
        tiles[t] = MsdTile{e0, e1 - e0, k0 & (MSD_TAG_SPAN - 1u), k1 - k0};
    }
}

__device__ __forceinline__ void keep_load(u64 &v) { asm volatile("" : "+v"(v)); }

__device__ __forceinline__ void lds_barrier()
{
    asm volatile("s_waitcnt lgkmcnt(0)\n\ts_barrier" ::: "memory");
}

__global__ __launch_bounds__(MSD_BLOCK, 4) void msd_local_fast_kernel(const u64 *in, const MsdTile *tiles, u32 nt, int rem_bits,
                                                                     int idx_bits, u32 *sa_out, u32 *fail_list, u32 *fail_count,
                                                                     int fused, MsdEmit em_val, const u64 *nt_dev,
                                                                     const u32 *counters_dev, const u32 *bad_dev)
{
    if (nt_dev) {
        if (counters_dev[1] > MSD_MAX_BUCKET || (bad_dev && *bad_dev)) return;
        nt = (u32)*nt_dev;
    }
    const MsdEmit *em = fused ? &em_val : nullptr;
    __shared__ __attribute__((aligned(16))) u64 lds_all[MSD_TILE + LS_WORDS];
    u64 *const exch = lds_all;
    u32 *const hist = reinterpret_cast<u32 *>(lds_all + MSD_TILE);
    u32 *const hist2 = hist + LS_WORDS;
    u32 *const scr = reinterpret_cast<u32 *>(&exch[MSD_TILE - 8]);
    u32 &s_fail = scr[MSD_WAVES + 2];
    const u32 tid = threadIdx.x;
    const u32 stride = gridDim.x;
    u32 t = blockIdx.x;
    if (t >= nt) return;
    MsdTile cur = tiles[t];
    MsdTile nxt = t + stride < nt ? tiles[t + stride] : MsdTile{0, 0, 0, 0};
    u64 pe[MSD_IPT];
    auto prefetch = [&](const MsdTile &d) {
#pragma unroll
        for (int r = 0; r < MSD_IPT; ++r) {
            const u32 p = r * MSD_BLOCK + tid;
            pe[r] = p < d.count ? in[d.e0 + p] : 0ull;
        }
    };
    prefetch(cur);
    for (u32 i = tid; i < LS_WORDS; i += MSD_BLOCK) hist[i] = 0;
    if (tid == 0) {
        s_fail = 0;
        scr[MSD_WAVES + 3] = 0;
    }
    lds_barrier();
    u32 prev_t = 0;
    bool prev_ok = false;
    for (;;) {
        const u32 count = cur.count, e0 = cur.e0;
        const u32 rows = (count + MSD_BLOCK - 1) / MSD_BLOCK;
        int seg_bits = 0;
        while ((1u << seg_bits) < cur.nb) ++seg_bits;
        const u64 tag_base = (u64)cur.tag0 << (rem_bits + idx_bits);
        const int sort_bits = rem_bits + seg_bits;
        const int bin_shift = idx_bits + (sort_bits > LS_BIN_BITS ? sort_bits - LS_BIN_BITS : 0);
        u64 e[MSD_IPT];
#pragma unroll
        for (int r = 0; r < MSD_IPT; ++r) {
            e[r] = ~0ull;
            if ((u32)r < rows) {
                const u32 p = r * MSD_BLOCK + tid;
                if (p < count) {
                    e[r] = pe[r] - tag_base;
                    const u32 bin = (u32)(e[r] >> bin_shift);
                    atomicAdd(&hist[bin >> 1], 1u << (16u * (bin & 1u)));
                }
            }
        }
        const bool more = t + stride < nt;
        if (more) prefetch(nxt);
        lds_barrier();
        if (tid == 0) {
            if (em && prev_ok) em->blk_cnt[prev_t] = scr[MSD_WAVES + 3];
            s_fail = 0;
            scr[MSD_WAVES + 3] = 0;
        }
        {
            constexpr int LS_WPT = LS_WORDS / MSD_BLOCK;
            static_assert(LS_WPT * MSD_BLOCK == (int)LS_WORDS && LS_WPT >= 1, "bins split evenly over the threads");
            u32 c[2 * LS_WPT];
            u32 sum = 0;
#pragma unroll
            for (int j = 0; j < LS_WPT; ++j) {
                const u32 wv = hist[LS_WPT * tid + j];
                c[2 * j] = wv & 0xffffu;
                c[2 * j + 1] = wv >> 16;
                sum += c[2 * j] + c[2 * j + 1];
            }
            const u32 incl = wave_incl_sum(sum);
            if (lane_id() == kWave - 1) scr[wave_id()] = incl;
            lds_barrier();
            u32 ex = incl - sum;
            for (int w = 0; w < wave_id(); ++w) ex += scr[w];
#pragma unroll
            for (int j = 0; j < LS_WPT; ++j) {
                const u32 lo = ex, hi = ex + c[2 * j];
                hist[LS_WPT * tid + j] = hist2[LS_WPT * tid + j] = lo | (hi << 16);
                ex = hi + c[2 * j + 1];
            }
        }
        lds_barrier();
#pragma unroll
        for (int r = 0; r < MSD_IPT; ++r) {
            if ((u32)r < rows) {
                const u32 p = r * MSD_BLOCK + tid;
                if (p < count) {
                    const u32 bin = (u32)(e[r] >> bin_shift), sh = 16u * (bin & 1u);
                    exch[(atomicAdd(&hist2[bin >> 1], 1u << sh) >> sh) & 0xffffu] = e[r];
                }
            }
        }
        if (tid < (u32)LS_WINDOW) exch[count + tid] = ~0ull;
        lds_barrier();
        const u16 *const starts16 = reinterpret_cast<const u16 *>(hist);
        u32 rk[MSD_IPT];
#pragma unroll
        for (int g = 0; g < MSD_IPT; g += LS_GROUP) {
            if ((u32)g < rows) {
                u64 x[LS_GROUP];
                u32 s0[LS_GROUP], sm[LS_GROUP];
#pragma unroll
                for (int j = 0; j < LS_GROUP; ++j) x[j] = exch[(g + j) * MSD_BLOCK + tid];
#pragma unroll
                for (int j = 0; j < LS_GROUP; ++j) {
                    const u32 bin = (u32)(x[j] >> bin_shift) & (LS_BINS - 1u);
                    s0[j] = starts16[bin];
                }
                u64 y[LS_GROUP][LS_WINDOW];
#pragma unroll
                for (int j = 0; j < LS_GROUP; ++j) {
#pragma unroll
                    for (int k = 0; k < LS_WINDOW; ++k) y[j][k] = exch[s0[j] + k];
                }
#pragma unroll
                for (int j = 0; j < LS_GROUP; ++j) {
                    u32 c = 0;
#pragma unroll
                    for (int k = 0; k < LS_WINDOW; ++k) {
                        keep_load(y[j][k]);
                        c += y[j][k] < x[j] ? 1u : 0u;
                    }
                    sm[j] = c;
                }
#pragma unroll
                for (int j = 0; j < LS_GROUP; ++j) {
                    const u32 p = (g + j) * MSD_BLOCK + tid;
                    if (p < count && ((y[j][LS_WINDOW - 1] ^ x[j]) >> bin_shift) == 0) {
                        const u32 bin = (u32)(x[j] >> bin_shift) & (LS_BINS - 1u);
                        const u32 s1 = bin + 1u < LS_BINS ? (u32)starts16[min(bin + 1u, LS_BINS - 1u)] : count;
                        const u32 len = s1 - s0[j];
                        if (len > LS_KMAX) {
                            s_fail = 1;
                        } else {
                            for (u32 q = s0[j] + LS_WINDOW; q < s0[j] + len; ++q) sm[j] += exch[q] < x[j] ? 1u : 0u;
                        }
                    }
                    e[g + j] = x[j];
                    rk[g + j] = s0[j] + sm[j];
                }
            } else {
#pragma unroll
                for (int j = 0; j < LS_GROUP; ++j) rk[g + j] = 0;
            }
        }
        lds_barrier();
        const bool failed = s_fail != 0;
        if (failed) {
            if (tid == 0) fail_list[atomicAdd(fail_count, 1u)] = t;
        } else {
#pragma unroll
            for (int r = 0; r < MSD_IPT; ++r) {
                if ((u32)r < rows) {
                    const u32 p = r * MSD_BLOCK + tid;
                    if (p < count) exch[rk[r]] = e[r];
                }
            }
        }
        for (u32 i = tid; i < LS_WORDS; i += MSD_BLOCK) hist[i] = 0;
        lds_barrier();
        if (!failed) {
            const u32 imask = (u32)((1ull << idx_bits) - 1ull);
            u32 *const s_count = &scr[MSD_WAVES + 3];
#pragma unroll
            for (int g = 0; g < MSD_IPT; g += LS_GROUP) {
                if ((u32)g < rows) {
                    u64 cur[LS_GROUP], prv[LS_GROUP], nxt[LS_GROUP];
#pragma unroll
                    for (int j = 0; j < LS_GROUP; ++j) {
                        const u32 p = (g + j) * MSD_BLOCK + tid;
                        cur[j] = exch[p];
                        prv[j] = exch[p ? p - 1 : 0];
                        nxt[j] = exch[p + 1];
                    }
#pragma unroll
                    for (int j = 0; j < LS_GROUP; ++j) {
                        keep_load(cur[j]);
                        keep_load(prv[j]);
                        keep_load(nxt[j]);
                    }
#pragma unroll
                    for (int j = 0; j < LS_GROUP; ++j) {
                        const u32 p = (g + j) * MSD_BLOCK + tid;
                        if (p < count) {
                            const u64 kx = cur[j] >> idx_bits;
                            const bool tie = p > 0 && (prv[j] >> idx_bits) == kx;
                            const u32 sfx = (u32)cur[j] & imask;
                            sa_out[e0 + p] = sfx | ((tie && em == nullptr) ? 0x80000000u : 0u);
                            if (em != nullptr) {
                                const bool tie_next = p + 1 < count && (nxt[j] >> idx_bits) == kx;
                                if (tie || tie_next) {
                                    const u32 slot = e0 + atomicAdd(s_count, 1u);
                                    em->st_pos[slot] = e0 + p;
                                    em->st_idx[slot] = sfx | (tie ? 0x80000000u : 0u);
                                }
                            }
                        }
                    }
                }
            }
        }
        prev_t = t;
        prev_ok = !failed;
        if (!more) break;
        t += stride;
        cur = nxt;
        nxt = t + stride < nt ? tiles[t + stride] : MsdTile{0, 0, 0, 0};
    }
    if (em) {
        lds_barrier();
        if (tid == 0 && prev_ok) em->blk_cnt[prev_t] = scr[MSD_WAVES + 3];
    }
}

#include "ss_sort_impl.h"


static size_t msd_max_tiles(uint32_t n)
{
    return (size_t)n / (SS_WIN / 2) + ((size_t)MSD_BINS * MSD_BINS) / MSD_RAW_TAG_SPAN + 8;
}

static size_t msd_max_tiles2(uint32_t n) { return (size_t)n / MSD_TILE2 + MSD_BINS + 8; }

static bool msd_use_lsd(uint32_t n)
{
    const char *e = knob("PSS_MSD_LSD");
    return !(e && atoi(e) == 0) && n < (1u << 30);
}

size_t msd_workspace_bytes(uint32_t n)
{
    const size_t max_ranges2 = (size_t)n / MSD_G2_RANGE + MSD_BINS + 8;
    const size_t nbk = (size_t)MSD_BINS * MSD_BINS;
    return max_ranges2 * MSD_BINS * 4
           + (MSD_BINS + 8) * 4
           + (nbk + 8) * 4
           + max_ranges2 * sizeof(MsdRange) + (MSD_BINS + 8) * 4 + 64
           + (nbk + 8) * 8
           + (nbk + 8) * 4
           + (msd_max_tiles(n) + 32) * 8
           + (msd_max_tiles(n) + 32) * 16
           + (msd_max_tiles(n) + 32) * sizeof(MsdTile)
           + (SC_MAX_BLOCKS + 8) * 8 + 8192
           + (size_t)MSD_BINS * MSD_G1_RANGES * 4 + (MSD_BINS + 8) * 4
           + msd_max_tiles2(n) * (sizeof(MsdTile2) + (size_t)MSD_BINS * 4)
           + (nbk + 8) * 4 + 4096;
}

int msd_max_key_bits(uint32_t n)
{
    int ib = 1;
    while ((1ull << ib) < (u64)n) ++ib;
    const int after2 = 64 + MSD_D - (msd_use_lsd(n) ? MSD_RAW_TAG_BITS : MSD_TAG_BITS) - ib + MSD_D;
    return std::min(after2, 64 + MSD_D - ib);
}

int msd_suffix_sort(DeviceCtx *ctx, const TextKeys *text, uint32_t n, int key_bits, uint64_t *A[2], uint32_t *sa_out,
                    void *work, uint32_t *h_small, bool profile, MsdStats *stats, bool *accepted, MsdActive *active,
                    const MsdFront *front)
{
    *accepted = false;
    hipStream_t s = ctx->stream;
    int ib = 1;
    while ((1ull << ib) < (u64)n) ++ib;
    if (key_bits < 2 * MSD_D + 1 || key_bits > msd_max_key_bits(n) || n < 2) {
        set_error("msd_suffix_sort: key of %d bits does not fit (n = %u)", key_bits, n);
        return PSS_EINVAL;
    }
    const size_t max_ranges2 = (size_t)n / MSD_G2_RANGE + MSD_BINS + 8;
    const size_t nbk = (size_t)MSD_BINS * MSD_BINS;
    u8 *w = static_cast<u8 *>(work);
    size_t o = 0;
    auto carve = [&](size_t bytes) { u8 *p = w + o; o = round_up(o + bytes, 256); return p; };
    u32 *T = reinterpret_cast<u32 *>(carve(max_ranges2 * MSD_BINS * 4));
    u32 *J1 = reinterpret_cast<u32 *>(carve((MSD_BINS + 8) * 4));
    u32 *J = reinterpret_cast<u32 *>(carve((nbk + 8) * 4));
    MsdRange *ranges2 = reinterpret_cast<MsdRange *>(carve(max_ranges2 * sizeof(MsdRange)));
    u32 *seg_first = reinterpret_cast<u32 *>(carve((MSD_BINS + 8) * 4));
    u32 *counters = reinterpret_cast<u32 *>(carve(64));
    u64 *ranks = reinterpret_cast<u64 *>(carve((nbk + 8) * 8));
    u32 *cstart = reinterpret_cast<u32 *>(carve((nbk + 8) * 4));
    const size_t max_tiles = msd_max_tiles(n);
    MsdTile *tiles_all = reinterpret_cast<MsdTile *>(carve((max_tiles + 16) * sizeof(MsdTile)));
    u32 *tile_first = reinterpret_cast<u32 *>(carve((max_tiles + 16) * 8));
    u32 *blk_cnt = reinterpret_cast<u32 *>(carve((max_tiles + 8) * 4));
    u64 *dst_off = reinterpret_cast<u64 *>(carve((max_tiles + 8) * 8));
    u64 *partial = reinterpret_cast<u64 *>(carve((SC_MAX_BLOCKS + 8) * 8));
    u64 *d_total = partial + SC_MAX_BLOCKS;
    const bool lsd = msd_use_lsd(n);
    const size_t max_tiles2 = msd_max_tiles2(n);
    u32 *T2 = nullptr, *Jb = nullptr, *status = nullptr, *cj = nullptr;
    MsdTile2 *tiles2 = nullptr;
    if (lsd) {
        T2 = reinterpret_cast<u32 *>(carve((size_t)MSD_BINS * MSD_G1_RANGES * 4));
        Jb = reinterpret_cast<u32 *>(carve((MSD_BINS + 8) * 4));
        tiles2 = reinterpret_cast<MsdTile2 *>(carve(max_tiles2 * sizeof(MsdTile2)));
        status = reinterpret_cast<u32 *>(carve(max_tiles2 * MSD_BINS * 4));
        cj = reinterpret_cast<u32 *>(carve((nbk + 8) * 4));
    }

    MsdArgs a;
    memset(&a, 0, sizeof a);
    a.codes = text->codes;
    a.code_bits = text->code_bits;
    a.key_chars = text->key_chars;
    a.plus_one = text->plus_one;
    a.key_drop = text->drop;
    a.n = n;
    a.key_bits = key_bits;
    a.idx_bits = ib;
    const u32 num_tiles = (u32)(((u64)n + MSD_TILE - 1) / MSD_TILE);
    a.tiles_per_range1 = (num_tiles + MSD_G1_RANGES - 1) / MSD_G1_RANGES;
    a.num_ranges1 = (num_tiles + a.tiles_per_range1 - 1) / a.tiles_per_range1;
    a.T = T;
    a.J1 = J1;
    a.J = J;
    a.ranges2 = ranges2;
    a.seg_first = seg_first;
    a.counters = counters;
    a.lsd = lsd ? 1 : 0;
    a.T2 = T2;
    a.Jb = Jb;
    a.tiles2 = tiles2;
    a.status = status;

    hipEvent_t ev[8] = {};
    int nev = 0;
    struct EvGuard {
        hipEvent_t *e;
        int *n;
        ~EvGuard()
        {
            for (int i = 0; i < *n; ++i) (void)hipEventDestroy(e[i]);
        }
    } guard{ev, &nev};
    auto mark = [&]() -> int {
        if (profile && nev < 8) {
            PSS_HIP(hipEventCreate(&ev[nev]));
            PSS_HIP(hipEventRecord(ev[nev], s));
            ++nev;
        }
        return PSS_OK;
    };

    PSS_HIP(hipMemsetAsync(counters, 0, 64, s));
    a.out = A[0];
    if (front) {
        a.raw = front->raw;
        a.lut = front->lut;
        a.codes_out = const_cast<u8 *>(text->codes);
        a.bad = front->bad;
        hipLaunchKernelGGL(msd_hist_raw_kernel, dim3(a.num_ranges1), dim3(MSD_BLOCK), 0, s, a);
    } else {
        hipLaunchKernelGGL(msd_hist_kernel<true>, dim3(a.num_ranges1), dim3(MSD_BLOCK), 0, s, a);
    }
    static_assert(MSD_G1_RANGES <= 1024, "msd_offsets1_kernel takes four ranges per thread");
    hipLaunchKernelGGL(msd_offsets1_kernel, dim3(MSD_BINS), dim3(256), 0, s, T, a.num_ranges1, seg_first);
    hipLaunchKernelGGL(msd_offsets1b_kernel, dim3(1), dim3(MSD_BINS), 0, s, (const u32 *)seg_first, J1, n);
    if (lsd) {
        hipLaunchKernelGGL(msd_offsets1_kernel, dim3(MSD_BINS), dim3(256), 0, s, T2, a.num_ranges1, seg_first);
        hipLaunchKernelGGL(msd_offsets1b_kernel, dim3(1), dim3(MSD_BINS), 0, s, (const u32 *)seg_first, Jb, n);
        PSS_HIP(hipMemsetAsync(status, 0, max_tiles2 * MSD_BINS * 4, s));
    }
    PSS_TRY(mark());
    const bool wide = lsd || !(knob("PSS_MSD_SCATTER") && atoi(knob("PSS_MSD_SCATTER")) == 1);
    if (lsd) hipLaunchKernelGGL((msd_scatter2_kernel<true, 1024, true>), dim3(a.num_ranges1), dim3(1024), 0, s, a);
    else if (wide) hipLaunchKernelGGL((msd_scatter2_kernel<true, 1024>), dim3(a.num_ranges1), dim3(1024), 0, s, a);
    else hipLaunchKernelGGL(msd_scatter_kernel<true>, dim3(a.num_ranges1), dim3(MSD_BLOCK), 0, s, a);
    PSS_TRY(mark());
    a.in = A[0];
    a.out = A[1];
    if (lsd) {
        hipLaunchKernelGGL(msd_tiles2_kernel, dim3(1), dim3(MSD_BINS), 0, s, (const u32 *)J1, tiles2, counters);
        PSS_TRY(mark());
        const u32 grid2 = std::min<u32>((u32)max_tiles2, (u32)ctx->num_cus);
        hipLaunchKernelGGL(msd_scatter_lb_kernel, dim3(grid2), dim3(1024), 0, s, a);
        PSS_TRY(mark());
    } else {
        hipLaunchKernelGGL(msd_ranges_kernel, dim3(1), dim3(MSD_BINS), 0, s, J1, ranges2, seg_first, counters);
        a.dense = ranks;
        hipLaunchKernelGGL(msd_hist_kernel<false>, dim3((u32)max_ranges2), dim3(MSD_BLOCK), 0, s, a);
        hipLaunchKernelGGL(msd_offsets_kernel, dim3(MSD_BINS), dim3(MSD_BINS), 0, s, T, (const u32 *)seg_first, (const u32 *)J1, J,
                           0u, n, MSD_BINS);
    }
    PSS_TRY(device_excl_scan(ctx, InNonEmpty{J}, nbk, partial, d_total, ranks));
    hipLaunchKernelGGL(msd_compact_kernel, dim3(1024), dim3(256), 0, s, J, (u32)nbk, ranks, cstart, counters, cj);
    const int rem_bits = key_bits - 2 * MSD_D;
    MsdEmit em{};
    const int fused = active != nullptr;
    if (fused) em = MsdEmit{active->st_pos, active->st_idx, blk_cnt};
    const bool one_trip = lsd && !knob("PSS_MSD_SLOW_LOCAL");
    u64 *d_total2 = d_total + 1;
    u32 *const fail_list_dev = tile_first + max_tiles + 16;
    if (one_trip) {
        const TilePlan tpd{MSD_WIN, MSD_TILE_CAP, cj};
        PSS_TRY(device_excl_scan(ctx, InTileHeadDev{cstart, d_total, n, tpd}, nbk, partial, d_total2, ranks));
        hipLaunchKernelGGL(msd_tiles_dev_kernel, dim3(1024), dim3(256), 0, s, cstart, (const u64 *)d_total, n, ranks, (const u64 *)d_total2,
                           tile_first, tpd);
        hipLaunchKernelGGL(msd_tile_desc_kernel, dim3((u32)((max_tiles + 255) / 256)), dim3(256), 0, s, cstart, tile_first, 0u, 0u, n,
                           tiles_all, (const u32 *)cj, (const u64 *)d_total2, (const u64 *)d_total);
        PSS_TRY(mark());
        hipLaunchKernelGGL(msd_local_fast_kernel, dim3(2u * (u32)ctx->num_cus), dim3(MSD_BLOCK), 0, s, A[1], (const MsdTile *)tiles_all, 0u,
                           rem_bits, ib, sa_out, fail_list_dev, counters + 4, fused, em, (const u64 *)d_total2, (const u32 *)counters,
                           front ? (const u32 *)front->bad : (const u32 *)nullptr);
        PSS_TRY(mark());
        PSS_HIP(hipMemcpyAsync(h_small + 8, d_total2, 8, hipMemcpyDeviceToHost, s));
        PSS_HIP(hipMemcpyAsync(h_small + 10, counters + 4, 4, hipMemcpyDeviceToHost, s));
    }
    PSS_HIP(hipMemcpyAsync(h_small, d_total, 8, hipMemcpyDeviceToHost, s));
    PSS_HIP(hipMemcpyAsync(h_small + 2, counters, 16, hipMemcpyDeviceToHost, s));
    if (front) PSS_HIP(hipMemcpyAsync(h_small + 6, front->bad, 4, hipMemcpyDeviceToHost, s));
    PSS_HIP(hipStreamSynchronize(s));
    const u32 ne = h_small[0];
    const u32 maxb = h_small[3];
    if (stats) {
        stats->buckets = ne;
        stats->max_bucket = maxb;
        stats->bad_symbol = front ? h_small[6] : 0u;
    }
    if (front && h_small[6]) return PSS_OK;
    if (maxb > MSD_MAX_BUCKET) return PSS_OK;
    if (!lsd) {
        PSS_TRY(mark());
        if (wide) hipLaunchKernelGGL((msd_scatter2_kernel<false, 1024>), dim3((u32)max_ranges2), dim3(1024), 0, s, a);
        else hipLaunchKernelGGL(msd_scatter_kernel<false>, dim3((u32)max_ranges2), dim3(MSD_BLOCK), 0, s, a);
        PSS_TRY(mark());
    }
    const auto local_sort = msd_local_sort_kernel;
    const auto local_fast = msd_local_fast_kernel;
    u32 nt = 0;
    u32 *fail_list = fail_list_dev;
    if (one_trip) {
        nt = h_small[8];
        if ((size_t)nt > max_tiles) {
            set_error("msd_suffix_sort: %u tiles planned, tables hold %zu (internal error)", nt, max_tiles);
            return PSS_EDEVICE;
        }
        const u32 nfail = h_small[10];
        if (stats) stats->slow_tiles = nfail;
        if (nfail)
            hipLaunchKernelGGL(local_sort, dim3(nfail), dim3(MSD_BLOCK), 0, s, A[1], (const MsdTile *)tiles_all, rem_bits,
                               ib, sa_out, (const u32 *)fail_list, fused, em);
    } else {
    const TilePlan tp{MSD_WIN, MSD_TILE_CAP, cj};
    PSS_TRY(device_excl_scan(ctx, InTileHead{cstart, ne, n, tp}, ne, partial, d_total, ranks));
    hipLaunchKernelGGL(msd_tiles_kernel, dim3(1024), dim3(256), 0, s, cstart, ne, n, ranks, (const u64 *)d_total, tile_first, tp);
    PSS_HIP(hipMemcpyAsync(h_small, d_total, 8, hipMemcpyDeviceToHost, s));
    PSS_HIP(hipStreamSynchronize(s));
    nt = h_small[0];
    if ((size_t)nt > max_tiles) {
        set_error("msd_suffix_sort: %u tiles planned, tables hold %zu (internal error)", nt, max_tiles);
        return PSS_EDEVICE;
    }
    PSS_TRY(mark());
    fail_list = tile_first + nt + 8;
    hipLaunchKernelGGL(msd_tile_desc_kernel, dim3((nt + 255) / 256), dim3(256), 0, s, cstart, tile_first, nt, ne, n, tiles_all,
                       (const u32 *)cj, (const u64 *)nullptr, (const u64 *)nullptr);
    if (knob("PSS_MSD_SLOW_LOCAL")) {
        hipLaunchKernelGGL(local_sort, dim3(nt), dim3(MSD_BLOCK), 0, s, A[1], (const MsdTile *)tiles_all, rem_bits, ib,
                           sa_out, (const u32 *)nullptr, fused, em);
    } else {
        MsdTile *tiles = tiles_all;
        const u32 grid = std::min<u32>(nt, 2u * (u32)ctx->num_cus);
        hipLaunchKernelGGL(local_fast, dim3(grid), dim3(MSD_BLOCK), 0, s, A[1], (const MsdTile *)tiles, nt, rem_bits, ib,
                           sa_out, fail_list, counters + 4, fused, em, (const u64 *)nullptr, (const u32 *)nullptr, (const u32 *)nullptr);
        PSS_TRY(mark());
        PSS_HIP(hipMemcpyAsync(h_small, counters + 4, 4, hipMemcpyDeviceToHost, s));
        PSS_HIP(hipStreamSynchronize(s));
        const u32 nfail = h_small[0];
        if (stats) stats->slow_tiles = nfail;
        if (nfail)
            hipLaunchKernelGGL(local_sort, dim3(nfail), dim3(MSD_BLOCK), 0, s, A[1], (const MsdTile *)tiles_all, rem_bits,
                               ib, sa_out, (const u32 *)fail_list, fused, em);
    }
    if (knob("PSS_MSD_SLOW_LOCAL")) PSS_TRY(mark());
    }
    if (fused) {
        const bool finish = knob("PSS_MSD_NO_FINISH") == nullptr;
        if (finish) {
            const int ks = std::min(64 / text->code_bits, 16);
            const MsdFinish fin{text->codes, text->code_bits, ks, text->plus_one,
                                (u32)(text->drop ? text->key_chars - 1 : text->key_chars), n};
            hipLaunchKernelGGL(msd_finish_kernel, dim3((nt + 3) / 4), dim3(256), 0, s, (const MsdTile *)tiles_all, blk_cnt, nt,
                               active->st_pos, active->st_idx, sa_out, fin);
        }
        PSS_TRY(device_excl_scan(ctx, InBlkCnt{blk_cnt}, nt, partial, d_total, dst_off));
        hipLaunchKernelGGL(msd_gather_kernel, dim3((nt + 3) / 4), dim3(256), 0, s, (const MsdTile *)tiles_all, blk_cnt, dst_off, nt,
                           active->st_pos, active->st_idx, active->pos, active->idx, active->grp);
        PSS_HIP(hipMemcpyAsync(h_small, d_total, 8, hipMemcpyDeviceToHost, s));
        PSS_HIP(hipStreamSynchronize(s));
        active->count = h_small[0];
        if (stats) stats->finished = h_small[1];
    }
    PSS_HIP(hipGetLastError());
    if (stats) {
        stats->tiles = nt;
        stats->lookback = lsd ? 1u : 0u;
    }
    if (profile && nev >= 6) {
        PSS_HIP(hipStreamSynchronize(s));
        float ms = 0.f;
        PSS_HIP(hipEventElapsedTime(&ms, ev[0], ev[1]));
        if (stats) stats->ms_g1 = ms;
        PSS_HIP(hipEventElapsedTime(&ms, ev[2], ev[3]));
        if (stats) stats->ms_g2 = ms;
        PSS_HIP(hipEventElapsedTime(&ms, ev[4], ev[5]));
        if (stats) stats->ms_local = ms;
    }
    *accepted = true;
    return PSS_OK;
}


struct SsGeometry {
    u32 B1, B2, os, S;
    int ib, kc, key_bits;
    u64 plo, phi;
};
static bool ss_geometry(uint32_t n, uint32_t radix, SsGeometry *g)
{
    if (n < (1u << 16) || n > (1u << 30) || radix < 2 || radix > 257) return false;
    int ib = 1;
    while ((1ull << ib) < (u64)n) ++ib;
    const unsigned __int128 limit = (unsigned __int128)1 << (128 - ib);
    unsigned __int128 pw = 1;
    int kc = 0;
    while (kc < SS_MAX_CHARS && pw <= limit / radix) {
        pw *= radix;
        ++kc;
    }
    if (kc < 2) return false;
    unsigned __int128 lead = 1;
    for (int i = 0; i + 1 < kc; ++i) lead *= radix;
    g->plo = (u64)lead;
    g->phi = (u64)(lead >> 64);
    int kb = 0;
    while (kb < 128 && ((pw - 1) >> kb) != 0) ++kb;
    g->key_bits = kb;
    int lb = 4;
    while (((u64)512 << lb) < (u64)n && lb < 20) ++lb;
    const u32 B1 = 1u << ((lb + 1) / 2), B2 = 1u << (lb / 2);
    const u32 os = ((u64)n > (u64)768 * B1 * B2) ? 8u : 4u;
    g->B1 = B1;
    g->B2 = B2;
    g->os = os;
    g->S = os * B1 * B2;
    g->ib = ib;
    g->kc = kc;
    return (u64)g->S * 4 <= (u64)n;
}
uint32_t ss_sample_count(uint32_t n)
{
    SsGeometry g;
    return ss_geometry(n, 257, &g) ? g.S : 0u;
}
uint64_t ss_geometry_tag(uint32_t n, uint32_t radix)
{
    SsGeometry g;
    if (!ss_geometry(n, radix, &g)) return 0;
    return ((uint64_t)g.S << 32) | ((uint64_t)g.B1 << 20) | ((uint64_t)g.B2 << 8) | ((uint64_t)g.ib << 2) | (uint64_t)(g.os == 8) | ((uint64_t)g.kc << 58);
}
int ss_key_chars(uint32_t n, uint32_t radix)
{
    SsGeometry g;
    return ss_geometry(n, radix, &g) ? g.kc : 0;
}

int ss_suffix_sort(DeviceCtx *ctx, const TextKeys *text, uint32_t radix, uint32_t n, const SsBuffers &buf, uint32_t *sa_out,
                   void *work, uint32_t *h_small, bool profile, SsStats *stats, bool *accepted, MsdActive *active)
{
    *accepted = false;
    hipStream_t s = ctx->stream;
    SsGeometry g;
    if (!ss_geometry(n, radix, &g)) return PSS_OK;
    static_assert(SS_SBLOCK == (int)MSD_BINS, "one bin per thread in the scatter passes");
    const size_t max_ranges2 = (size_t)n / MSD_G2_RANGE + MSD_BINS + 8;
    const size_t nbk = (size_t)MSD_BINS * MSD_BINS;
    u8 *w = static_cast<u8 *>(work);
    size_t o = 0;
    auto carve = [&](size_t bytes) { u8 *p = w + o; o = round_up(o + bytes, 256); return p; };
    u32 *T = reinterpret_cast<u32 *>(carve(max_ranges2 * MSD_BINS * 4));
    u32 *J1 = reinterpret_cast<u32 *>(carve((MSD_BINS + 8) * 4));
    u32 *J = reinterpret_cast<u32 *>(carve((nbk + 8) * 4));
    MsdRange *ranges2 = reinterpret_cast<MsdRange *>(carve(max_ranges2 * sizeof(MsdRange)));
    u32 *seg_first = reinterpret_cast<u32 *>(carve((MSD_BINS + 8) * 4));
    u32 *counters = reinterpret_cast<u32 *>(carve(64));
    u64 *ranks = reinterpret_cast<u64 *>(carve((nbk + 8) * 8));
    u32 *cstart = reinterpret_cast<u32 *>(carve((nbk + 8) * 4));
    const size_t max_tiles = msd_max_tiles(n);
    MsdTile *tiles_all = reinterpret_cast<MsdTile *>(carve((max_tiles + 16) * sizeof(MsdTile)));
    u32 *tile_first = reinterpret_cast<u32 *>(carve((max_tiles + 16) * 8));
    u32 *blk_cnt = reinterpret_cast<u32 *>(carve((max_tiles + 8) * 4));
    u64 *dst_off = reinterpret_cast<u64 *>(carve((max_tiles + 8) * 8));
    u64 *partial = reinterpret_cast<u64 *>(carve((SC_MAX_BLOCKS + 8) * 8));
    u64 *d_total = partial + SC_MAX_BLOCKS;

    hipEvent_t ev[8] = {};
    int nev = 0;
    struct EvGuard {
        hipEvent_t *e;
        int *n;
        ~EvGuard()
        {
            for (int i = 0; i < *n; ++i) (void)hipEventDestroy(e[i]);
        }
    } guard{ev, &nev};
    auto mark = [&]() -> int {
        if (profile && nev < 8) {
            PSS_HIP(hipEventCreate(&ev[nev]));
            PSS_HIP(hipEventRecord(ev[nev], s));
            ++nev;
        }
        return PSS_OK;
    };

    SsText tx{text->codes, n, text->code_bits, g.kc, text->plus_one, g.ib, radix, g.plo, g.phi};
    const u32 S = g.S;
    E16 *E0 = static_cast<E16 *>(buf.E0), *E = static_cast<E16 *>(buf.E);
    PSS_TRY(mark());
    if (buf.sample_in) {
        E = const_cast<E16 *>(static_cast<const E16 *>(buf.sample_in));
    } else {
    hipLaunchKernelGGL(ss_sample_kernel, dim3((S + 255) / 256), dim3(256), 0, s, tx, S, E0, buf.K[0], buf.V[0]);
    if (S <= 8192) {
        std::vector<E16> hs(S);
        PSS_HIP(hipMemcpyAsync(hs.data(), E0, (size_t)S * 16, hipMemcpyDeviceToHost, s));
        PSS_HIP(hipStreamSynchronize(s));
        std::sort(hs.begin(), hs.end(), [](const E16 &x, const E16 &y) { return x.hi < y.hi || (x.hi == y.hi && x.lo < y.lo); });
        PSS_HIP(hipMemcpyAsync(E, hs.data(), (size_t)S * 16, hipMemcpyHostToDevice, s));
        PSS_HIP(hipStreamSynchronize(s));
    } else {
        u64 *K[2] = {buf.K[0], buf.K[1]};
        u32 *V[2] = {buf.V[0], buf.V[1]};
        SortStats ss1;
        int d1 = 0, d2 = 0;
        PSS_TRY(radix_sort_pairs(ctx, K, V, S, 64, 0xffu, nullptr, 0, buf.sort_work, &d1, false, &ss1));
        hipLaunchKernelGGL(ss_gather_hi_kernel, dim3((S + 255) / 256), dim3(256), 0, s, E0, (const u32 *)V[d1], S, K[d1]);
        const int hi_bits = std::min(64, std::max(1, g.key_bits + g.ib - 64));
        PSS_TRY(radix_sort_pairs(ctx, K, V, S, hi_bits, 0xffu, nullptr, d1, buf.sort_work, &d2, false, &ss1));
        hipLaunchKernelGGL(ss_gather_elems_kernel, dim3((S + 255) / 256), dim3(256), 0, s, E0, (const u32 *)V[d2], S, E);
    }
    if (buf.sample_keep) PSS_HIP(hipMemcpyAsync(buf.sample_keep, E, (size_t)S * 16, hipMemcpyDeviceToDevice, s));
    }
    PSS_TRY(mark());

    SsArgs a;
    memset(&a, 0, sizeof a);
    a.text = tx;
    a.sample = E;
    a.B1 = g.B1;
    a.B2 = g.B2;
    a.spb = S / g.B1;
    a.st2 = g.os;
    a.zl = (u32)std::max(0, std::min(64 - SS_CELL_BITS, 128 - g.key_bits - g.ib));
    const u32 num_tiles = (u32)(((u64)n + SS_DTILE1 - 1) / SS_DTILE1);
    a.tiles_per_range1 = (num_tiles + MSD_G1_RANGES - 1) / MSD_G1_RANGES;
    a.num_ranges1 = (num_tiles + a.tiles_per_range1 - 1) / a.tiles_per_range1;
    a.T = T;
    a.J1 = J1;
    a.ranges2 = ranges2;
    a.counters = counters;
    a.digits = buf.digits;
    PSS_HIP(hipMemsetAsync(counters, 0, 64, s));
    hipLaunchKernelGGL(ss_digits1_kernel, dim3(a.num_ranges1), dim3(SS_DBLOCK), 0, s, a);
    hipLaunchKernelGGL(msd_offsets1_kernel, dim3(MSD_BINS), dim3(256), 0, s, T, a.num_ranges1, seg_first);
    hipLaunchKernelGGL(msd_offsets1b_kernel, dim3(1), dim3(MSD_BINS), 0, s, (const u32 *)seg_first, J1, n);
    a.out = static_cast<E16 *>(buf.A[0]);
    hipLaunchKernelGGL(ss_scatter_kernel<true>, dim3(a.num_ranges1), dim3(SS_SBLOCK), 0, s, a);
    PSS_TRY(mark());
    hipLaunchKernelGGL(msd_ranges_kernel, dim3(1), dim3(MSD_BINS), 0, s, (const u32 *)J1, ranges2, seg_first, counters);
    a.in = static_cast<const E16 *>(buf.A[0]);
    a.out = static_cast<E16 *>(buf.A[1]);
    hipLaunchKernelGGL(ss_digits2_kernel, dim3((u32)max_ranges2), dim3(SS_DBLOCK), 0, s, a);
    hipLaunchKernelGGL(msd_offsets_kernel, dim3(MSD_BINS), dim3(MSD_BINS), 0, s, T, (const u32 *)seg_first, (const u32 *)J1, J,
                       0u, n, MSD_BINS);
    PSS_TRY(device_excl_scan(ctx, InNonEmpty{J}, nbk, partial, d_total, ranks));
    hipLaunchKernelGGL(msd_compact_kernel, dim3(1024), dim3(256), 0, s, J, (u32)nbk, ranks, cstart, counters, (u32 *)nullptr);
    PSS_HIP(hipMemcpyAsync(h_small, d_total, 8, hipMemcpyDeviceToHost, s));
    PSS_HIP(hipMemcpyAsync(h_small + 2, counters, 16, hipMemcpyDeviceToHost, s));
    PSS_HIP(hipStreamSynchronize(s));
    const u32 ne = h_small[0];
    const u32 maxb = h_small[3];
    if (stats) {
        stats->buckets = ne;
        stats->max_bucket = maxb;
        stats->b1 = g.B1;
        stats->b2 = g.B2;
        stats->samples = S;
        stats->key_chars = g.kc;
    }
    if (maxb > SS_MAX_BUCKET && knob("PSS_SS_DEBUG")) {
        std::vector<u32> hj1(MSD_BINS + 1), hj((size_t)nbk + 1);
        (void)hipMemcpy(hj1.data(), J1, (MSD_BINS + 1) * 4, hipMemcpyDeviceToHost);
        (void)hipMemcpy(hj.data(), J, ((size_t)nbk + 1) * 4, hipMemcpyDeviceToHost);
        u32 m1 = 0, a1 = 0;
        for (u32 i = 0; i < g.B1; ++i) { const u32 c = hj1[i + 1] - hj1[i]; if (c > m1) { m1 = c; a1 = i; } }
        fprintf(stderr, "[pss] ss declined: n=%u S=%u B1=%u B2=%u kc=%d ib=%d | largest first-level bucket %u (#%u, average %u) | joint buckets above the cap:", n, S,
                g.B1, g.B2, g.kc, g.ib, m1, a1, n / g.B1);
        int shown = 0;
        for (u64 i = 0; i < nbk && shown < 12; ++i) {
            const u32 c = hj[i + 1] - hj[i];
            if (c > SS_MAX_BUCKET) { fprintf(stderr, " #%llu:%u@%u", (unsigned long long)i, c, hj[i]); ++shown; }
        }
        fprintf(stderr, "\n");
    }
    if (maxb > SS_MAX_BUCKET) return PSS_OK;
    hipLaunchKernelGGL(ss_scatter_kernel<false>, dim3((u32)max_ranges2), dim3(SS_SBLOCK), 0, s, a);
    PSS_TRY(mark());
    const char *seg_env = knob("PSS_SS_SEG");
    const bool seg = !knob("PSS_SS_WINDOW_PLAN") && !(seg_env && atoi(seg_env) == 0);
    u32 *pstart = nullptr;
    if (knob("PSS_SS_WINDOW_PLAN")) {
        const TilePlan tp{SS_WIN, SS_TILE_CAP, nullptr};
        PSS_TRY(device_excl_scan(ctx, InTileHead{cstart, ne, n, tp}, ne, partial, d_total, ranks));
        hipLaunchKernelGGL(msd_tiles_kernel, dim3(1024), dim3(256), 0, s, cstart, ne, n, ranks, (const u64 *)d_total, tile_first, tp);
    } else {
        const size_t row = (size_t)ne + 1;
        u32 *pl = reinterpret_cast<u32 *>(buf.A[0]);
        const u32 *starts = cstart;
        u32 total = n, cap = SS_TILE_CAP;
        if (seg) {
            PSS_TRY(device_excl_scan(ctx, InPad8{cstart, ne, n}, ne, partial, d_total, ranks));
            PSS_HIP(hipMemcpyAsync(h_small, d_total, 8, hipMemcpyDeviceToHost, s));
            pstart = pl;
            hipLaunchKernelGGL(ss_pad_starts_kernel, dim3((u32)((row + 255) / 256)), dim3(256), 0, s, (const u64 *)ranks, (const u64 *)d_total, ne,
                               pstart);
            PSS_HIP(hipStreamSynchronize(s));
            total = h_small[0];
            starts = pstart;
            cap = SS_TILE;
            pl += round_up(row, 64);
        }
        const u32 nseg = (u32)(((u64)total + SS_PLAN_SEG - 1) / SS_PLAN_SEG);
        u32 levels = 0;
        while ((1u << levels) < nseg) ++levels;
        u32 *nxt = pl, *heads = pl + row, *jumps = pl + 2 * row;
        const u32 gb = (u32)((row + 255) / 256);
        PSS_HIP(hipMemsetAsync(heads, 0, row * 4, s));
        hipLaunchKernelGGL(ss_plan_next_kernel, dim3(gb), dim3(256), 0, s, starts, ne, total, cap, nxt);
        hipLaunchKernelGGL(ss_plan_exit_kernel, dim3(gb), dim3(256), 0, s, starts, ne, (const u32 *)nxt, jumps);
        for (u32 i = 1; i < levels; ++i)
            hipLaunchKernelGGL(ss_plan_double_kernel, dim3(gb), dim3(256), 0, s, (const u32 *)(jumps + (size_t)(i - 1) * row), (u32)row,
                               jumps + (size_t)i * row);
        hipLaunchKernelGGL(ss_plan_mark_kernel, dim3((nseg + 255) / 256), dim3(256), 0, s, starts, ne, (const u32 *)nxt,
                           (const u32 *)jumps, levels, nseg, heads);
        PSS_TRY(device_excl_scan(ctx, InU32{heads}, ne, partial, d_total, ranks));
        hipLaunchKernelGGL(ss_plan_tiles_kernel, dim3(1024), dim3(256), 0, s, (const u32 *)heads, ne, (const u64 *)ranks,
                           (const u64 *)d_total, tile_first);
    }
    PSS_HIP(hipMemcpyAsync(h_small, d_total, 8, hipMemcpyDeviceToHost, s));
    PSS_HIP(hipStreamSynchronize(s));
    const u32 nt = h_small[0];
    if ((size_t)nt > max_tiles) {
        set_error("ss_suffix_sort: %u tiles planned, tables hold %zu (internal error)", nt, max_tiles);
        return PSS_EDEVICE;
    }
    hipLaunchKernelGGL(msd_tile_desc_kernel, dim3((nt + 255) / 256), dim3(256), 0, s, cstart, tile_first, nt, ne, n, tiles_all,
                       (const u32 *)nullptr, (const u64 *)nullptr, (const u64 *)nullptr);
    (void)active;
    (void)blk_cnt;
    (void)dst_off;
    PSS_TRY(mark());
    if (pstart)
        hipLaunchKernelGGL(ss_local_seg_kernel, dim3(nt), dim3(SL_BLOCK), 0, s, (const E16 *)buf.A[1], (const MsdTile *)tiles_all, nt, g.ib,
                           (const u32 *)cstart, (const u32 *)pstart, (const u32 *)tile_first, ne, n, sa_out);
    else
        hipLaunchKernelGGL(ss_local_kernel, dim3(nt), dim3(SL_BLOCK), 0, s, (const E16 *)buf.A[1], (const MsdTile *)tiles_all, nt, g.ib,
                           sa_out);
    PSS_TRY(mark());
    hipLaunchKernelGGL(ss_boundary_kernel, dim3((nt + 255) / 256), dim3(256), 0, s, (const MsdTile *)tiles_all, nt, tx, sa_out);
    PSS_HIP(hipGetLastError());
    if (stats) stats->tiles = nt;
    if (profile && nev >= 6 && stats) {
        PSS_HIP(hipStreamSynchronize(s));
        float ms = 0.f;
        PSS_HIP(hipEventElapsedTime(&ms, ev[0], ev[1]));
        stats->ms_sample = ms;
        PSS_HIP(hipEventElapsedTime(&ms, ev[1], ev[2]));
        stats->ms_g1 = ms;
        PSS_HIP(hipEventElapsedTime(&ms, ev[2], ev[3]));
        stats->ms_g2 = ms;
        PSS_HIP(hipEventElapsedTime(&ms, ev[4], ev[5]));
        stats->ms_local = ms;
    }
    *accepted = true;
    return PSS_OK;
}

}
```

### pysubstringsearch_amd/csrc/sa_build.hip

```cpp
#include "prims.h"
#include "msd_sort.h"
#include "rle_build.h"
#include "radix_sort.h"
#include "sa_build.h"
#include "scan.h"
#include "text_keys.h"
#include "anchor_impl.h"

#include <algorithm>
#include <cmath>
#include <string>
#include <thread>

namespace pss {


constexpr u32 DUP_SAMPLES = 8192, DUP_SLOTS = 16384;
__global__ __launch_bounds__(1024) void dup_screen_kernel(const u8 *T, u32 n, u32 *dups)
{
    __shared__ u32 table[DUP_SLOTS];
    for (u32 i = threadIdx.x; i < DUP_SLOTS; i += 1024) table[i] = 0;
    __syncthreads();
    u32 mine = 0;
    if (n >= 64) {
        const u32 stride = (n - 32) / DUP_SAMPLES;
        for (u32 k = threadIdx.x; k < DUP_SAMPLES; k += 1024) {
            u64 x = ((u64)k + 1) * 0x9E3779B97F4A7C15ull;
            x ^= x >> 29;
            x *= 0xBF58476D1CE4E5B9ull;
            x ^= x >> 32;
            const u32 pos = stride ? k * stride + (u32)(x % stride) : k % (n - 32);
            const u64 a = load_u64_unaligned(T + pos), b = load_u64_unaligned(T + pos + 8);
            u64 hsh = (a ^ (b * 0x9E3779B97F4A7C15ull)) * 0xD6E8FEB86659FD93ull;
            hsh ^= hsh >> 32;
            u32 f = (u32)hsh;
            if (f == 0) f = 1;
            u32 slot = (f * 2654435761u) >> (32 - 14);
            static_assert(DUP_SLOTS == (1u << 14), "14-bit slot");
            for (;;) {
                const u32 old = atomicCAS(&table[slot], 0u, f);
                if (old == 0u) break;
                if (old == f) { ++mine; break; }
                slot = (slot + 1) & (DUP_SLOTS - 1);
            }
        }
    }
    const u32 tot = wave_incl_sum(mine);
    if (lane_id() == kWave - 1 && tot) atomicAdd(dups, tot);
}

__global__ __launch_bounds__(256) void sa_symbols_kernel(const u8 *T, u32 n, u32 *present, u32 *counts, u32 *runs)
{
    __shared__ u32 seen[256];
    __shared__ u32 cnt[256];
    const u32 tid = threadIdx.x;
    seen[tid] = 0;
    cnt[tid] = 0;
    u32 nruns = 0;
    __syncthreads();
    const u32 nvec = n / 16;
    const uint4 *Tv = reinterpret_cast<const uint4 *>(T);
    const bool aligned = ((uintptr_t)T & 15) == 0;
    if (aligned) {
        auto take = [&](const uint4 v, u32 i) {
            const u32 w[4] = {v.x, v.y, v.z, v.w};
            const bool sample = (i & 15u) == 0;
            u32 prev = __shfl_up(v.w >> 24, 1);
            if (lane_id() == 0) prev = i ? (u32)T[i * 16 - 1] : (~v.x & 0xffu);
#pragma unroll
            for (int k = 0; k < 4; ++k) {
                const u32 diff = w[k] ^ ((w[k] << 8) | prev);
                prev = w[k] >> 24;
                nruns += (u32)__popc((((diff & 0x7f7f7f7fu) + 0x7f7f7f7fu) | diff) & 0x80808080u);
#pragma unroll
                for (int s = 0; s < 32; s += 8) {
                    const u32 c = (w[k] >> s) & 0xffu;
                    if (!seen[c]) seen[c] = 1;
                    if (sample) atomicAdd(&cnt[c], 1u);
                }
            }
        };
        const u32 stride = gridDim.x * blockDim.x;
        u32 i = blockIdx.x * blockDim.x + tid;
        for (; (u64)(i - lane_id() + kWave - 1) + 3ull * stride < nvec; i += 4 * stride) {
            const uint4 v0 = Tv[i], v1 = Tv[i + stride], v2 = Tv[i + 2 * stride], v3 = Tv[i + 3 * stride];
            take(v0, i);
            take(v1, i + stride);
            take(v2, i + 2 * stride);
            take(v3, i + 3 * stride);
        }
        for (; i < nvec; i += stride) take(Tv[i], i);
    }
    const u32 tail0 = aligned ? nvec * 16 : 0;
    for (u32 i = tail0 + blockIdx.x * blockDim.x + tid; i < n; i += gridDim.x * blockDim.x) {
        const u32 c = T[i];
        if (!seen[c]) seen[c] = 1;
        atomicAdd(&cnt[c], 1u);
        if (i == 0 || (u32)T[i - 1] != c) ++nruns;
    }
    __syncthreads();
    if (seen[tid]) present[tid] = 1;
    if (cnt[tid]) atomicAdd(&counts[tid], cnt[tid]);
#pragma unroll
    for (int o = 32; o > 0; o >>= 1) nruns += __shfl_xor(nruns, o);
    if (lane_id() == 0 && nruns) atomicAdd(runs, nruns);
}

__global__ __launch_bounds__(256) void sa_recode_kernel(const u8 *T, u32 n, u32 n_pad, const u8 *lut, u8 *codes)
{
    __shared__ u8 s_lut[256];
    s_lut[threadIdx.x] = lut[threadIdx.x];
    __syncthreads();
    const u32 nvec = n_pad / 16;
    const bool aligned = ((uintptr_t)T & 15) == 0;
    for (u32 v = blockIdx.x * blockDim.x + threadIdx.x; v < nvec; v += gridDim.x * blockDim.x) {
        const u32 i0 = v * 16;
        u32 w[4] = {0, 0, 0, 0};
        if (aligned && i0 + 16 <= n) {
            const uint4 x = reinterpret_cast<const uint4 *>(T)[v];
            w[0] = x.x; w[1] = x.y; w[2] = x.z; w[3] = x.w;
#pragma unroll
            for (int k = 0; k < 4; ++k) {
                u32 o = 0;
#pragma unroll
                for (int s = 0; s < 32; s += 8) o |= (u32)s_lut[(w[k] >> s) & 0xffu] << s;
                w[k] = o;
            }
        } else {
#pragma unroll
            for (int k = 0; k < 4; ++k) {
                u32 o = 0;
#pragma unroll
                for (int s = 0; s < 4; ++s) {
                    const u32 i = i0 + k * 4 + s;
                    const u32 c = (i < n) ? (u32)s_lut[T[i]] : 0u;
                    o |= c << (s * 8);
                }
                w[k] = o;
            }
        }
        reinterpret_cast<uint4 *>(codes)[v] = make_uint4(w[0], w[1], w[2], w[3]);
    }
}

#include "sa_rerank_impl.h"

#include "sa_rounds_impl.h"

#include "sa_plan_impl.h"

#include "sa_refine_impl.h"

int suffix_rounds_integer(DeviceCtx *ctx, uint32_t m, uint64_t *K[2], uint32_t *V[2], int cur, uint32_t *SA_out,
                          pss_sa_stats *st)
{
    const Knobs knobs = Knobs::read();
    PSS_TRY(ctx->slot[S_ISA].reserve((size_t)m * 4 + 64));
    PSS_TRY(ctx->slot[S_P0].reserve((size_t)m * 4));
    PSS_TRY(ctx->slot[S_P1].reserve((size_t)m * 4));
    PSS_TRY(ctx->slot[S_GRP].reserve((size_t)m * 4));
    const size_t sort_ws = radix_sort_workspace_bytes();
    PSS_TRY(ctx->slot[S_WORK].reserve(sort_ws + 65536));
    u8 *work = ctx->slot[S_WORK].as<u8>();
    u8 *small = work + sort_ws;
    RoundsIO io;
    io.n = m;
    io.SA = SA_out;
    io.K[0] = K[0]; io.K[1] = K[1];
    io.V[0] = V[0]; io.V[1] = V[1];
    io.ISA = ctx->slot[S_ISA].as<u32>();
    io.P[0] = ctx->slot[S_P0].as<u32>(); io.P[1] = ctx->slot[S_P1].as<u32>();
    io.GRP = ctx->slot[S_GRP].as<u32>();
    io.codes = nullptr;
    io.b = 8; io.plus_one = 0; io.key_chars = 1; io.key_drop = 0;
    io.h0 = 1;
    io.cur = cur;
    io.final_buf = -1;
    io.v_scratch = nullptr;
    io.ties = false;
    io.msd_fused = false;
    io.msd_active = 0;
    io.no_sparse = false;
    io.work = work;
    io.d_agg_head = reinterpret_cast<u32 *>(small + 4096);
    io.d_agg_cnt = reinterpret_cast<u32 *>(small + 8192);
    io.d_red = reinterpret_cast<u64 *>(small + 12288);
    io.d_counters = reinterpret_cast<u32 *>(small + 12288 + 64);
    io.h_small = static_cast<u32 *>(ctx->pinned);
    io.profile = false;
    SortStats ss;
    pss_sa_stats local;
    memset(&local, 0, sizeof local);
    PSS_TRY(refine_rounds(ctx, knobs, io, ss, st ? *st : local));
    return PSS_OK;
}

int sa_build_device(DeviceCtx *ctx, const void *d_T, void *d_SA, int32_t n_in, uint32_t flags, pss_sa_stats *stats)
{
    pss_sa_stats st;
    memset(&st, 0, sizeof st);
    if (n_in < 0 || (n_in > 0 && (d_T == nullptr || d_SA == nullptr))) {
        set_error("pss_sa_build: bad arguments");
        return PSS_EINVAL;
    }
    const u32 n = (u32)n_in;
    const bool profile = flags & 1u;
    if (flags & 8u) {
        ctx->plan_path = 0;
        ctx->ss_plan_skip = ctx->ss_plan_backoff = 0;
        ctx->side_plan_heff = 0;
        flags &= ~8u;
    }
    const Knobs knobs = Knobs::read();
    hipStream_t s = ctx->stream;
    if (n < 2) {
        if (n == 1) PSS_HIP(hipMemsetAsync(d_SA, 0, 4, s));
        PSS_HIP(hipStreamSynchronize(s));
        if (stats) *stats = st;
        return PSS_OK;
    }
    const u8 *T = static_cast<const u8 *>(d_T);
    u32 *SA = static_cast<u32 *>(d_SA);

    const size_t n_pad = round_up((size_t)n, 16) + 64;
    PSS_TRY(ctx->slot[S_CODES].reserve(n_pad));
    PSS_TRY(ctx->slot[S_K0].reserve((size_t)n * 8));
    PSS_TRY(ctx->slot[S_K1].reserve((size_t)n * 8));
    PSS_TRY(ctx->slot[S_V0].reserve((size_t)n * 4));
    PSS_TRY(ctx->slot[S_V1].reserve((size_t)n * 4));
    PSS_TRY(ctx->slot[S_ISA].reserve((size_t)n * 4 + 64));
    PSS_TRY(ctx->slot[S_P0].reserve(std::max((size_t)n * 4, msd_workspace_bytes(n))));
    PSS_TRY(ctx->slot[S_P1].reserve((size_t)n * 4));
    PSS_TRY(ctx->slot[S_GRP].reserve((size_t)n * 4));
    const size_t sort_ws = radix_sort_workspace_bytes();
    PSS_TRY(ctx->slot[S_WORK].reserve(sort_ws + 65536));
    u8 *work = ctx->slot[S_WORK].as<u8>();
    u8 *small = work + sort_ws;
    u32 *d_present = reinterpret_cast<u32 *>(small);
    u8 *d_lut = small + 2048;
    u32 *d_agg_head = reinterpret_cast<u32 *>(small + 4096);
    u32 *d_agg_cnt = reinterpret_cast<u32 *>(small + 8192);
    u64 *d_red = reinterpret_cast<u64 *>(small + 12288);
    u32 *d_counters = reinterpret_cast<u32 *>(small + 12288 + 64);

    u8 *codes = ctx->slot[S_CODES].as<u8>();
    u64 *K[2] = {ctx->slot[S_K0].as<u64>(), ctx->slot[S_K1].as<u64>()};
    u32 *V[2] = {ctx->slot[S_V0].as<u32>(), ctx->slot[S_V1].as<u32>()};
    u32 *ISA = ctx->slot[S_ISA].as<u32>();
    u32 *P[2] = {ctx->slot[S_P0].as<u32>(), ctx->slot[S_P1].as<u32>()};
    u32 *GRP = ctx->slot[S_GRP].as<u32>();
    u32 *h_small = static_cast<u32 *>(ctx->pinned);

    BuildTimer timer;
    PSS_HIP(hipEventCreate(&timer.ev0));
    PSS_HIP(hipEventCreate(&timer.ev1));
    PSS_HIP(hipEventCreate(&timer.ev_mid));
    PSS_HIP(hipEventRecord(timer.ev0, s));
    if (ctx->restart_depth == 0) {
        ctx->restart_ms = 0.0;
        ctx->ss_refused_note = false;
    }
    SideAnchors side;
    auto start_over = [&](uint32_t new_flags) -> int {
        side.join();
        PSS_HIP(hipEventRecord(timer.ev1, s));
        PSS_HIP(hipStreamSynchronize(s));
        float gone = 0.f;
        PSS_HIP(hipEventElapsedTime(&gone, timer.ev0, timer.ev1));
        ctx->restart_ms += gone;
        ctx->restart_depth += 1;
        const int rc = sa_build_device(ctx, d_T, d_SA, n_in, new_flags, stats);
        ctx->restart_depth -= 1;
        return rc;
    };

    const int grid_stream = ctx->num_cus * 8;
    u32 *d_runs = d_counters + 40;
    uint32_t logn = 0;
    while ((2u << logn) <= n && logn < 31) ++logn;
    const bool plain = knobs.key_chars == 0 && !knobs.no_sample && !knobs.no_flags && knobs.msd < 0 && knobs.ss < 0 &&
                       knobs.key_drop < 0 && knobs.mode < 0 && !knobs.no_msd_fuse && !knobs.no_plan && knobs.rle < 0 &&
                       knobs.period != 0 && (flags & 2u) == 0;
    const bool fronted = plain && !knobs.no_front && n >= (1u << 24) && ctx->plan_path == 1 && ctx->plan_logn == logn &&
                         (reinterpret_cast<uintptr_t>(T) & 15u) == 0;
    if (!fronted) {
        PSS_HIP(hipMemsetAsync(d_present, 0, 2048, s));
        PSS_HIP(hipMemsetAsync(d_runs, 0, 4, s));
        hipLaunchKernelGGL(sa_symbols_kernel, dim3(grid_stream), dim3(256), 0, s, T, n, d_present, d_present + 256, d_runs);
        const bool screen_dups = plain && !knobs.no_front && (flags & 4u) == 0 && n >= (1u << 24);
        PSS_HIP(hipMemsetAsync(d_runs + 1, 0, 4, s));
        if (screen_dups) hipLaunchKernelGGL(dup_screen_kernel, dim3(1), dim3(1024), 0, s, T, n, d_runs + 1);
        PSS_HIP(hipMemcpyAsync(h_small, d_present, 2048, hipMemcpyDeviceToHost, s));
        PSS_HIP(hipMemcpyAsync(h_small + 512, d_runs, 8, hipMemcpyDeviceToHost, s));
        u8 *h_head = static_cast<u8 *>(ctx->pinned) + 32768;
        const u32 head_len = std::min<u32>(n, kPeriodProbe);
        const bool look_for_period = knobs.period != 0 && n >= 4 * kPeriodProbe;
        if (look_for_period) PSS_HIP(hipMemcpyAsync(h_head, T, head_len, hipMemcpyDeviceToHost, s));
        PSS_HIP(hipStreamSynchronize(s));
        const u32 text_runs = h_small[512];
        st.runs = text_runs;
        if (knobs.rle == 1 || (knobs.rle < 0 && n >= 4096 && (u64)text_runs * 8 <= (u64)n)) {
            RleStats rls;
            PSS_TRY(rle_suffix_array(ctx, T, n, text_runs, SA, profile, &rls, &st));
            st.rle = rls.columns ? 2 : 1;
            st.rle_id_bits = rls.id_bits;
            st.rle_ms_table = rls.ms_table;
            st.rle_ms_reduced = rls.ms_reduced;
            st.rle_ms_expand = rls.ms_expand;
            for (int c = 0; c < 256; ++c) st.sigma += h_small[c] ? 1u : 0u;
            PSS_HIP(hipEventRecord(timer.ev1, s));
            PSS_HIP(hipStreamSynchronize(s));
            float ms = 0.f;
            PSS_HIP(hipEventElapsedTime(&ms, timer.ev0, timer.ev1));
            st.ms_total = ms + ctx->restart_ms;
            st.ms_restarts = ctx->restart_ms;
            if (stats) *stats = st;
            return PSS_OK;
        }
        if (look_for_period) {
            const u32 p = period_of_head(h_head, head_len);
            if (p) {
                u32 m = 0;
                PSS_TRY(period_extent(ctx, T, n, p, &m));
                st.period = p;
                st.period_extent = m;
                bool accepted = false;
                if (n - m <= kPeriodTailMax) {
                    std::vector<u8> word(h_head, h_head + p);
                    PSS_TRY(period_suffix_array(ctx, T, n, p, m, word.data(), SA, &accepted));
                }
                if (accepted) {
                    st.period_path = 1;
                    for (int c = 0; c < 256; ++c) st.sigma += h_small[c] ? 1u : 0u;
                    PSS_HIP(hipEventRecord(timer.ev1, s));
                    PSS_HIP(hipStreamSynchronize(s));
                    float ms = 0.f;
                    PSS_HIP(hipEventElapsedTime(&ms, timer.ev0, timer.ev1));
                    st.ms_total = ms + ctx->restart_ms;
            st.ms_restarts = ctx->restart_ms;
                    if (stats) *stats = st;
                    return PSS_OK;
                }
            }
        }
    }
    u8 lut[256];
    u32 sigma = 0;
    if (fronted) {
        memcpy(lut, ctx->plan_lut, 256);
        sigma = ctx->plan_sigma;
    } else {
        for (int c = 0; c < 256; ++c) lut[c] = h_small[c] ? (u8)(++sigma) : 0;
    }
    int b = 1;
    while ((1u << b) <= sigma) ++b;
    int plus_one = 0;
    if (sigma == 256) {
        b = 9;
        plus_one = 1;
        for (int c = 0; c < 256; ++c) lut[c] = (u8)c;
    }
    int kmax = 64 / b;
    if (kmax > 16) kmax = 16;
    bool fresh = false;
    if (!fronted && plain && !knobs.no_front && (flags & 4u) == 0 && n >= (1u << 24) && sigma >= 2 && sigma < 256 &&
        (reinterpret_cast<uintptr_t>(T) & 15u) == 0) {
        double tot = 0, c2 = 0;
        for (int c = 0; c < 256; ++c) tot += h_small[256 + c];
        for (int c = 0; c < 256 && tot > 0; ++c) {
            const double pr = h_small[256 + c] / tot;
            c2 += pr * pr;
        }
        fresh = tot > 0 && c2 < 0.035 && h_small[513] < 8;
        st.dup_screen = h_small[513];
    }
    const bool front_any = fronted || fresh;
    int key_chars = front_any ? kmax : choose_key_chars(h_small + 256, n, b, kmax);
    const bool forced_chars = knobs.key_chars >= 1 && knobs.key_chars <= kmax;
    if (forced_chars) key_chars = knobs.key_chars;
    st.sigma = sigma;
    st.code_bits = (u32)b;
    st.key_chars = (u32)key_chars;
    memcpy(h_small + 1024, lut, 256);
    PSS_HIP(hipMemcpyAsync(d_lut, h_small + 1024, 256, hipMemcpyHostToDevice, s));
    u32 *d_bad = d_counters + 44;
    if (front_any) {
        const size_t tail0 = (size_t)n & ~(size_t)15;
        PSS_HIP(hipMemsetAsync(codes + tail0, 0, n_pad - tail0, s));
        PSS_HIP(hipMemsetAsync(d_bad, 0, 4, s));
    } else {
        hipLaunchKernelGGL(sa_recode_kernel, dim3(grid_stream), dim3(256), 0, s, T, n, (u32)n_pad, d_lut, codes);
        if (plain && knobs.side != 0 && knobs.anchor != 0 && ctx->side_plan_heff != 0 && ctx->side_plan_logn == logn &&
            ctx->side_plan_b == b && n >= (1u << 24) && (flags & 2u) == 0) {
            int kt0 = 64 / b;
            if (kt0 > 16) kt0 = 16;
            const int kc0 = ss_key_chars(n, plus_one ? 257u : sigma + 1u);
            if (kc0 > 0 && (u64)kc0 + (u64)kt0 == ctx->side_plan_heff) {
                PSS_HIP(hipEventRecord(timer.ev_mid, s));
                PSS_TRY(side_start(ctx, knobs, side, n, codes, b, plus_one, ctx->side_plan_heff, timer.ev_mid));
            }
        }
    }

    SortStats ss;
    int key_drop = 0;
    bool msd_screen_ok = false, sampled = false;
    uint32_t present_bits[8] = {};
    for (int c = 0; c < 256; ++c)
        if (plus_one || lut[c]) present_bits[c >> 5] |= 1u << (c & 31);
    int hint = 0;
    if (front_any) hint = 1;
    else if (plain && n >= (1u << 24) && ctx->plan_path && ctx->plan_logn == logn && memcmp(ctx->plan_present, present_bits, 32) == 0)
        hint = ctx->plan_path;
    st.plan_hint = (uint64_t)(fronted ? 2 : (fresh ? 3 : hint));
    if (hint) {
        sampled = true;
        msd_screen_ok = hint == 1;
    } else if (n >= (1u << 24) && !forced_chars && knobs.key_chars == 0 && !knobs.no_sample) {
        PSS_TRY(size_initial_key(ctx, codes, n, b, kmax, plus_one, K, V, work, d_counters + 16, h_small, profile, &ss,
                                 &key_chars, &key_drop, &msd_screen_ok));
        st.key_chars = (u32)key_chars;
        sampled = true;
    }
    if (knobs.key_drop >= 0 && knobs.key_drop < b && key_chars > 1) key_drop = knobs.key_drop;
    TextKeys tk{codes, b, key_chars, plus_one, key_drop};
    const int key_bits0 = key_chars * b - key_drop;
    st.key_bits = (u64)key_bits0;
    const int passes0 = (key_bits0 + 7) / 8;
    const int final_buf = (passes0 - 1) & 1;
    u32 *const v_scratch = V[final_buf];
    V[final_buf] = SA;
    int cur = 0;
    const bool ties = passes0 >= 2 && !knobs.no_flags;
    bool msd_done = false, msd_fused = false;
    u32 msd_active = 0;
    if (ties && knobs.msd != 0) {
        const char *cap_env = knob("PSS_MSD_KEY_CAP");
        const int key_cap = cap_env ? atoi(cap_env) : 48;
        const bool whole = knob("PSS_MSD_PARTIAL_SYMBOL") == nullptr;
        int kb = std::min(msd_max_key_bits(n), std::max(key_cap, 21));
        int kc = std::min(whole ? kb / b : (kb + b - 1) / b, kmax);
        int mdrop = kc * b - kb;
        if (mdrop < 0 || kc <= 1) {
            kb = kc * b;
            mdrop = 0;
        }
        const bool fits = kc >= 1 && kb >= 21 && !plus_one;
        const bool auto_ok = sampled && msd_screen_ok && (hint == 1 || (key_bits0 <= 48 && kb + 8 >= key_bits0));
        if (fits && (knobs.msd == 1 || (knobs.msd < 0 && auto_ok))) {
            TextKeys mk{codes, b, kc, plus_one, mdrop};
            MsdStats ms;
            bool accepted = false;
            PSS_TRY(ctx->slot[S_GRP2].reserve((size_t)n * 4));
            MsdActive act;
            act.pos = ctx->slot[S_P1].as<u32>();
            act.idx = (final_buf == 0) ? V[1] : V[0];
            act.grp = ctx->slot[S_GRP2].as<u32>();
            act.st_pos = reinterpret_cast<u32 *>(K[0]);
            act.st_idx = reinterpret_cast<u32 *>(K[0]) + n;
            const MsdFront front{T, d_lut, d_bad};
            PSS_TRY(msd_suffix_sort(ctx, &mk, n, kb, K, SA, ctx->slot[S_P0].p, h_small, profile, &ms, &accepted,
                                    knobs.no_msd_fuse ? nullptr : &act, front_any ? &front : nullptr));
            if (front_any && !accepted) {
                ctx->plan_path = 0;
                return start_over(fresh ? (flags | 4u) : flags);
            }
            msd_fused = accepted && !knobs.no_msd_fuse;
            msd_active = act.count;
            st.msd_buckets = ms.buckets;
            st.msd_max_bucket = ms.max_bucket;
            if (accepted) {
                msd_done = true;
                key_chars = kc;
                key_drop = mdrop;
                st.key_chars = (u32)kc;
                st.key_bits = (u64)kb;
                st.msd = 1;
                st.msd_tiles = ms.tiles;
                st.msd_slow_tiles = ms.slow_tiles;
                st.msd_lookback = ms.lookback;
                st.msd_finished = ms.finished;
                st.msd_ms_g1 = ms.ms_g1;
                st.msd_ms_g2 = ms.ms_g2;
                st.msd_ms_local = ms.ms_local;
                cur = final_buf;
                ss.launches = 3;
                ss.elems = 3ull * n;
            }
        }
    }
    if (front_any && !msd_done) {
        ctx->plan_path = 0;
        return start_over(fresh ? (flags | 4u) : flags);
    }
    if (!msd_done && ties && knobs.ss != 0 && (knobs.ss == 1 || (n >= (1u << 24) && !forced_chars && knobs.key_chars == 0)) &&
        ss_sample_count(n) != 0) {
        const u32 S = ss_sample_count(n);
        bool ss_room = ctx->slot[S_SSA].reserve((size_t)n * 16 + 256) == PSS_OK && ctx->slot[S_SSB].reserve((size_t)n * 16 + 256) == PSS_OK;
        if (!ss_room) {
            (void)hipGetLastError();
            ctx->slot[S_SSA].release();
            ctx->slot[S_SSB].release();
            set_error("%s", "");
            st.ss_declined_nomem = 1;
        }
        if (ss_room) {
        PSS_TRY(ctx->slot[S_GRP2].reserve((size_t)n * 4));
        SsBuffers sb;
        sb.A[0] = ctx->slot[S_SSA].p;
        sb.A[1] = ctx->slot[S_SSB].p;
        sb.digits = reinterpret_cast<uint16_t *>(ctx->slot[S_P1].p);
        sb.E0 = GRP;
        sb.E = ISA;
        sb.K[0] = K[0]; sb.K[1] = K[1];
        sb.V[0] = v_scratch; sb.V[1] = (final_buf == 0) ? V[1] : V[0];
        sb.sort_work = work;
        const u32 radix = plus_one ? 257u : sigma + 1u;
        const u64 tag = ss_geometry_tag(n, radix);
        const bool planned = hint == 2 && tag != 0 && ctx->ss_plan_tag == tag && ctx->ss_plan_radix == radix && ctx->slot[S_SSPLAN].p != nullptr &&
                             ctx->ss_plan_skip == 0;
        if (planned) sb.sample_in = ctx->slot[S_SSPLAN].p;
        else if (plain && ctx->slot[S_SSPLAN].reserve((size_t)S * 16) == PSS_OK) sb.sample_keep = ctx->slot[S_SSPLAN].p;
        ctx->ss_plan_tag = 0;
        MsdActive act;
        act.pos = ctx->slot[S_P1].as<u32>();
        act.idx = (final_buf == 0) ? V[1] : V[0];
        act.grp = ctx->slot[S_GRP2].as<u32>();
        act.st_pos = reinterpret_cast<u32 *>(K[0]);
        act.st_idx = reinterpret_cast<u32 *>(K[0]) + n;
        TextKeys sk{codes, b, 0, plus_one, 0};
        SsStats sst;
        bool accepted = false;
        PSS_TRY(ss_suffix_sort(ctx, &sk, plus_one ? 257u : sigma + 1u, n, sb, SA, ctx->slot[S_P0].p, h_small, profile, &sst, &accepted,
                               &act));
        if (planned && !accepted) {
            ctx->ss_plan_backoff = std::min(63u, 2 * ctx->ss_plan_backoff + 1);
            ctx->ss_plan_skip = ctx->ss_plan_backoff;
            ctx->ss_refused_note = true;
            ctx->plan_path = 0;
            return start_over(flags);
        } else if (accepted) {
            if (planned) ctx->ss_plan_backoff = 0;
            else if (hint == 2 && ctx->ss_plan_skip) --ctx->ss_plan_skip;
        }
        st.ss_buckets = sst.buckets;
        st.ss_max_bucket = sst.max_bucket;
        st.ss_samples = sst.samples;
        if (accepted) {
            msd_done = true;
            msd_fused = false;
            key_chars = sst.key_chars;
            key_drop = 0;
            st.key_chars = (u32)key_chars;
            st.key_bits = (u64)key_chars * b;
            st.ss = 1;
            st.ss_tiles = sst.tiles;
            st.ss_ms_sample = sst.ms_sample;
            st.ss_ms_g1 = sst.ms_g1;
            st.ss_ms_g2 = sst.ms_g2;
            st.ss_ms_local = sst.ms_local;
            cur = final_buf;
            ss.launches = 4;
            ss.elems = 4ull * n;
            if (sb.sample_in || sb.sample_keep) {
                ctx->ss_plan_tag = tag;
                ctx->ss_plan_radix = radix;
            }
            st.ss_planned = sb.sample_in ? 1 : 0;
        }
        }
    }
    if (hint && !msd_done) {
        ctx->plan_path = 0;
        return start_over(flags);
    }
    if (plain && n >= (1u << 24) && !fronted) {
        ctx->plan_path = st.msd ? 1 : (st.ss && ctx->ss_plan_tag != 0 ? 2 : 0);
        ctx->plan_logn = logn;
        memcpy(ctx->plan_present, present_bits, 32);
        memcpy(ctx->plan_lut, lut, 256);
        ctx->plan_sigma = sigma;
    }
    if (msd_done) {
    } else if (ties) PSS_TRY(suffix_sort_flags(ctx, K, V, n, key_bits0, &tk, work, &cur, profile, &ss));
    else PSS_TRY(radix_sort_pairs(ctx, K, V, n, key_bits0, 0xffffffffu, &tk, 0, work, &cur, profile, &ss));
    st.initial_passes = (u32)ss.launches;
    PSS_HIP(hipEventRecord(timer.ev_mid, s));
    RoundsIO io;
    io.n = n;
    io.SA = SA;
    io.K[0] = K[0]; io.K[1] = K[1];
    io.V[0] = V[0]; io.V[1] = V[1];
    io.ISA = ISA;
    io.P[0] = P[0]; io.P[1] = P[1];
    io.GRP = GRP;
    io.codes = codes;
    io.b = b; io.plus_one = plus_one; io.key_chars = key_chars; io.key_drop = key_drop;
    io.h0 = (u64)(key_drop ? key_chars - 1 : key_chars);
    io.cur = cur;
    io.final_buf = final_buf;
    io.v_scratch = v_scratch;
    io.ties = ties;
    io.msd_fused = msd_fused;
    io.msd_active = msd_active;
    io.no_sparse = st.ss != 0;
    io.work = work;
    io.d_agg_head = d_agg_head; io.d_agg_cnt = d_agg_cnt; io.d_red = d_red; io.d_counters = d_counters; io.h_small = h_small;
    io.profile = profile;
    io.side = &side;
    PSS_TRY(refine_rounds(ctx, knobs, io, ss, st));
    side.join();
    if (side.started && st.anchor_side == 0) st.anchor_side = 2;
    if (plain && n >= (1u << 24)) {
        ctx->side_plan_heff = st.anchor_side == 1 ? side.h_eff : 0;
        ctx->side_plan_logn = logn;
        ctx->side_plan_b = b;
    }
    PSS_HIP(hipEventRecord(timer.ev1, s));
    PSS_HIP(hipStreamSynchronize(s));
    float ms = 0.f;
    PSS_HIP(hipEventElapsedTime(&ms, timer.ev0, timer.ev1));
    st.ss_plan_refused = ctx->ss_refused_note ? 1 : 0;
    st.ms_total = ms + ctx->restart_ms;
            st.ms_restarts = ctx->restart_ms;
    PSS_HIP(hipEventElapsedTime(&ms, timer.ev0, timer.ev_mid));
    st.ms_initial = ms;
    st.ms_sort = ss.ms;
    st.sort_launches = ss.launches;
    st.sort_elems = ss.elems;
    st.ms_pairs = ss.ms_pairs;
    st.pairs_launches = ss.pairs_launches;
    st.pairs_elems = ss.pairs_elems;
    st.ms_text = ss.ms_text;
    st.text_launches = ss.text_launches;
    for (int i = 0; i < 9; ++i) {
        st.fs_ms[i] = ss.fs_ms[i];
        st.fs_launches[i] = ss.fs_launches[i];
        st.fs_elems[i] = ss.fs_elems[i];
    }
    if (stats) *stats = st;
    return PSS_OK;
}

}
```

### pysubstringsearch_amd/csrc/sa_plan_impl.h

```cpp

__global__ __launch_bounds__(256) void sample_keys_kernel(const u8 *codes, u32 n, u32 S, int b, int kmax, int plus_one,
                                                            u64 *keys, u32 *vals)
{
    const u32 t = blockIdx.x * blockDim.x + threadIdx.x;
    if (t >= S) return;
    const u32 stride = n / S;
    u64 x = ((u64)t + 1) * 0x9E3779B97F4A7C15ull;
    x ^= x >> 29;
    x *= 0xBF58476D1CE4E5B9ull;
    x ^= x >> 32;
    const u32 pos = t * stride + (u32)(x % stride);
    const int bits = kmax * b;
    keys[t] = text_key_at(codes, pos, b, kmax, plus_one, n) << (64 - bits);
    vals[t] = t;
}

constexpr u32 kMsdScreenRun = 48;
__global__ __launch_bounds__(256) void sample_ties_kernel(const u64 *keys, u32 S, u32 *tied )
{
    __shared__ u32 s_c[8];
    if (threadIdx.x < 8) s_c[threadIdx.x] = 0;
    __syncthreads();
    u32 c[8] = {};
    u32 crowded = 0, distinct = 0;
    for (u32 t = blockIdx.x * blockDim.x + threadIdx.x; t < S; t += gridDim.x * blockDim.x) {
        const u64 k = keys[t];
        const u64 dp = t > 0 ? (keys[t - 1] ^ k) : ~0ull, dn = t + 1 < S ? (keys[t + 1] ^ k) : ~0ull;
        const int lz = max(dp ? __builtin_clzll(dp) : 64, dn ? __builtin_clzll(dn) : 64);
#pragma unroll
        for (int w = 0; w < 8; ++w) c[w] += lz >= 8 * (w + 1) ? 1u : 0u;
        if (t + kMsdScreenRun < S && ((keys[t + kMsdScreenRun] ^ k) >> 44) == 0) ++crowded;
        if (t == 0 || (dp >> 44) != 0) ++distinct;
    }
    if (crowded) atomicAdd(&tied[8], crowded);
    if (distinct) atomicAdd(&tied[9], distinct);
#pragma unroll
    for (int w = 0; w < 8; ++w)
        if (c[w]) atomicAdd(&s_c[w], c[w]);
    __syncthreads();
    if (threadIdx.x < 8 && s_c[threadIdx.x]) atomicAdd(&tied[threadIdx.x], s_c[threadIdx.x]);
}


static void rerank_geometry(u32 m, RerankArgs &a)
{
    a.m = m;
    a.num_tiles = (u32)(((u64)m + RR_TILE - 1) / RR_TILE);
    a.tiles_per_range = (a.num_tiles + RR_MAX_RANGES - 1) / RR_MAX_RANGES;
    if (a.tiles_per_range == 0) a.tiles_per_range = 1;
    a.num_ranges = (a.num_tiles + a.tiles_per_range - 1) / a.tiles_per_range;
}

enum Slot { S_CODES = 0, S_K0, S_K1, S_V0, S_V1, S_ISA, S_P0, S_P1, S_GRP, S_WORK, S_GRP2 = 26, S_BIG = 27, S_SCR = 29, S_SSA = 30, S_SSB = 31, S_ANC = 32 , S_X0 = 39 , S_SSPLAN = 48, S_PER = 49, S_BGT = 54, S_ANCW = 55 };

static int choose_key_chars(const u32 *counts, u32 n, int b, int kmax)
{
    double tot = 0, c = 0;
    for (int i = 0; i < 256; ++i) tot += counts[i];
    if (tot <= 0) return kmax;
    for (int i = 0; i < 256; ++i) {
        const double p = counts[i] / tot;
        c += p * p;
    }
    if (c >= 0.999999) return kmax;
    const double need = (12.0 + log2((double)n)) / -log2(c);
    int k = (int)ceil(need);
    if (k < 1) k = 1;
    if (k > kmax) k = kmax;
    const int passes = (k * b + 7) / 8;
    k = (passes * 8) / b;
    if (k > kmax) k = kmax;
    if ((kmax * b + 7) / 8 - passes <= 1) k = kmax;
    return k;
}

struct Knobs {
    int key_chars = 0;
    int key_drop = -1;
    bool no_sample = false;
    bool no_flags = false;
    int mode = -1;
    int text_rounds_max = 5;
    int msd = -1;
    bool no_plan = false;
    bool no_front = false;
    int ss = -1;
    bool no_msd_fuse = false;
    bool no_mid_tier = false;
    int big_merge = -1;
    bool no_mid_merge = false;
    int period = -1;
    int rle = -1;
    int anchor = -1;
    int anchor_omega = 0;
    bool no_probe = false;
    int anchor_min_omega = 11;
    int probe_skip_pct = 50;
    int side = -1;
    int side_pct = 8;
    int anchor_cap_div = 5;
    bool count_sort = false;
    bool no_periodic = false;
    bool timing = false;
    static Knobs read()
    {
        Knobs k;
        if (const char *e = knob("PSS_KEY_CHARS")) k.key_chars = atoi(e);
        if (const char *e = knob("PSS_KEY_DROP")) k.key_drop = atoi(e);
        k.no_sample = knob("PSS_NO_SAMPLE") != nullptr;
        k.no_flags = knob("PSS_NO_TIES_PASS") != nullptr;
        if (const char *e = knob("PSS_MODE")) {
            if (!strcmp(e, "dense")) k.mode = 0;
            else if (!strcmp(e, "sparse")) k.mode = 1;
            else if (!strcmp(e, "text")) k.mode = 2;
        }
        if (const char *e = knob("PSS_TEXT_ROUNDS")) k.text_rounds_max = atoi(e);
        if (const char *e = knob("PSS_MSD")) k.msd = atoi(e);
        if (const char *e = knob("PSS_SS")) k.ss = atoi(e);
        k.no_plan = knob("PSS_NO_PLAN_CACHE") != nullptr;
        k.no_front = knob("PSS_NO_PLAN_FRONT") != nullptr;
        k.no_msd_fuse = knob("PSS_MSD_NO_FUSE") != nullptr;
        k.no_mid_tier = knob("PSS_NO_MID_TIER") != nullptr;
        k.no_mid_merge = knob("PSS_NO_MID_MERGE") != nullptr;
        if (const char *e = knob("PSS_BIG_MERGE")) k.big_merge = atoi(e);
        if (knob("PSS_NO_BIG_MERGE")) k.big_merge = 0;
        if (const char *e = knob("PSS_RLE")) k.rle = atoi(e);
        if (const char *e = knob("PSS_PERIOD")) k.period = atoi(e);
        if (const char *e = knob("PSS_ANCHOR")) k.anchor = atoi(e);
        if (const char *e = knob("PSS_ANCHOR_OMEGA")) k.anchor_omega = atoi(e);
        k.no_probe = knob("PSS_NO_PROBE") != nullptr;
        if (const char *e = knob("PSS_PROBE_SKIP_PCT")) k.probe_skip_pct = atoi(e);
        if (const char *e = knob("PSS_ANCHOR_MIN_OMEGA")) k.anchor_min_omega = std::max(2, atoi(e));
        if (const char *e = knob("PSS_ANCHOR_SIDE")) k.side = atoi(e);
        if (const char *e = knob("PSS_ANCHOR_SIDE_PCT")) k.side_pct = atoi(e);
        if (const char *e = knob("PSS_ANCHOR_CAP_DIV")) k.anchor_cap_div = std::min(5, std::max(3, atoi(e)));
        k.count_sort = knob("PSS_COUNT_SORT") != nullptr;
        { const char *e = knob("PSS_PERIODIC"); k.no_periodic = e && atoi(e) == 0; }
        k.timing = knob("PSS_TIMING") != nullptr;
        return k;
    }
};

struct BuildTimer {
    hipEvent_t ev0 = nullptr, ev1 = nullptr, ev_mid = nullptr;
    ~BuildTimer()
    {
        if (ev0) (void)hipEventDestroy(ev0);
        if (ev1) (void)hipEventDestroy(ev1);
        if (ev_mid) (void)hipEventDestroy(ev_mid);
    }
};

static int size_initial_key(DeviceCtx *ctx, const u8 *codes, u32 n, int b, int kmax, int plus_one, u64 *K[2], u32 *V[2],
                            void *work, u32 *d_tied, u32 *h_small, bool profile, SortStats *ss, int *key_chars,
                            int *key_drop, bool *msd_screen_ok)
{
    hipStream_t s = ctx->stream;
    const u32 S = 1u << 21;
    const int bits_max = kmax * b, pmax = (bits_max + 7) / 8;
    PSS_HIP(hipMemsetAsync(d_tied, 0, 64, s));
    hipLaunchKernelGGL(sample_keys_kernel, dim3(S / 256), dim3(256), 0, s, codes, n, S, b, kmax, plus_one, K[0], V[0]);
    u32 mask = 0;
    for (int p = 0; p < 8; ++p)
        if (8 * (p + 1) > 64 - 8 * (pmax - 1)) mask |= 1u << p;
    int sd = 0;
    const u64 launches = ss->launches, elems = ss->elems;
    PSS_TRY(radix_sort_pairs(ctx, K, V, S, 64, mask, nullptr, 0, work, &sd, profile, ss));
    ss->launches = launches;
    ss->elems = elems;
    hipLaunchKernelGGL(sample_ties_kernel, dim3(256), dim3(256), 0, s, K[sd], S, d_tied);
    PSS_HIP(hipMemcpyAsync(h_small, d_tied, 64, hipMemcpyDeviceToHost, s));
    PSS_HIP(hipStreamSynchronize(s));
    *msd_screen_ok = h_small[8] == 0 && h_small[9] != 0 && (double)n / (double)h_small[9] <= 3400.0;
    *key_chars = kmax;
    *key_drop = 0;
    for (int p = 2; p < pmax; ++p) {
        const double est = (double)h_small[p - 1] / S * ((double)n / S);
        if (est <= 0.02) {
            *key_chars = (8 * p + b - 1) / b;
            *key_drop = *key_chars * b - 8 * p;
            break;
        }
    }
    return PSS_OK;
}
```

### pysubstringsearch_amd/csrc/scan.h

```cpp
#pragma once
#include "common.h"
#include "prims.h"

namespace pss {

constexpr u32 SC_BLOCK = 256;
constexpr u32 SC_MAX_BLOCKS = 1024;

__device__ __forceinline__ u64 block_excl_sum64(u64 v, u64 *scr, u64 *total)
{
    const u64 incl = wave_incl_sum64(v);
    if (lane_id() == kWave - 1) scr[wave_id()] = incl;
    __syncthreads();
    u64 base = 0, tot = 0;
    for (u32 w = 0; w < SC_BLOCK / kWave; ++w) {
        const u64 s = scr[w];
        if (w < (u32)wave_id()) base += s;
        tot += s;
    }
    __syncthreads();
    *total = tot;
    return base + incl - v;
}

struct InU32 {
    const u32 *p;
    __device__ u64 operator()(u64 i) const { return p[i]; }
};
template <typename In>
__global__ __launch_bounds__(SC_BLOCK) void scan_reduce_kernel(In in, u64 n, u64 per_block, u64 *partial)
{
    __shared__ u64 scr[SC_BLOCK / kWave];
    const u64 b0 = (u64)blockIdx.x * per_block, b1 = (b0 + per_block < n) ? b0 + per_block : n;
    u64 acc = 0;
    for (u64 i = b0 + threadIdx.x; i < b1; i += SC_BLOCK) acc += in(i);
    u64 tot;
    (void)block_excl_sum64(acc, scr, &tot);
    if (threadIdx.x == 0) partial[blockIdx.x] = tot;
}

template <int DUMMY>
__global__ __launch_bounds__(1024) void scan_partials_kernel(u64 *partial, u32 nb, u64 *total)
{
    __shared__ u64 s[16];
    const u32 t = threadIdx.x, lane = lane_id(), w = wave_id();
    const u64 v = t < nb ? partial[t] : 0;
    const u64 incl = wave_incl_sum64(v);
    if (lane == 63) s[w] = incl;
    __syncthreads();
    u64 base = 0, tot = 0;
    for (u32 k = 0; k < 16; ++k) {
        if (k < w) base += s[k];
        tot += s[k];
    }
    if (t < nb) partial[t] = base + incl - v;
    if (t == 0) *total = tot;
}

template <typename In>
__global__ __launch_bounds__(SC_BLOCK) void scan_apply_kernel(In in, u64 n, u64 per_block, const u64 *partial,
                                                                u64 *out, const u64 *total)
{
    __shared__ u64 scr[SC_BLOCK / kWave];
    const u64 b0 = (u64)blockIdx.x * per_block, b1 = (b0 + per_block < n) ? b0 + per_block : n;
    u64 carry = partial[blockIdx.x];
    for (u64 base = b0; base < b1; base += SC_BLOCK) {
        const u64 i = base + threadIdx.x;
        const u64 v = i < b1 ? in(i) : 0;
        u64 tot;
        const u64 ex = block_excl_sum64(v, scr, &tot);
        if (i < b1) out[i] = carry + ex;
        carry += tot;
    }
    if (blockIdx.x == 0 && threadIdx.x == 0) out[n] = *total;
}

template <typename In>
inline int device_excl_scan(DeviceCtx *ctx, In in, u64 n, u64 *partial, u64 *d_total, u64 *out)
{
    u64 per_block = (n + SC_MAX_BLOCKS - 1) / SC_MAX_BLOCKS;
    per_block = round_up(per_block ? per_block : 1, SC_BLOCK);
    const u32 nb = (u32)((n + per_block - 1) / per_block);
    const u32 nbl = nb ? nb : 1;
    hipLaunchKernelGGL(scan_reduce_kernel<In>, dim3(nbl), dim3(SC_BLOCK), 0, ctx->stream, in, n, per_block, partial);
    hipLaunchKernelGGL(scan_partials_kernel<0>, dim3(1), dim3(1024), 0, ctx->stream, partial, nbl, d_total);
    hipLaunchKernelGGL(scan_apply_kernel<In>, dim3(nbl), dim3(SC_BLOCK), 0, ctx->stream, in, n, per_block, partial, out,
                       d_total);
    PSS_HIP(hipGetLastError());
    return PSS_OK;
}

}
```

Baseline: 67.86.

## Keep MSD sort tail on device with chained scans and gated kernels

Replaces the three-kernel reduce/partials/apply scan with a single-pass decoupled look-back scan, and gates the finish, scan and gather kernels on device-side counters. The MSD tail can then be enqueued behind the local sort without a host round trip. Tile planning is split into a prefix kernel and a multi-block starts kernel. Several small host costs are also removed: per-build event creation, the repeated LUT upload (skipped when the work buffer generation is unchanged), and the separate memsets, now folded into a begin kernel. This adds complexity, persistent-style loops and generation tracking, with the risk of stale-LUT or look-back ordering bugs.

New measurement: 68.17, median of 6. No clear change (+0.5%).

```diff
diff --git a/pysubstringsearch_amd/csrc/common.cpp b/pysubstringsearch_amd/csrc/common.cpp
--- a/pysubstringsearch_amd/csrc/common.cpp
+++ b/pysubstringsearch_amd/csrc/common.cpp
@@ -45,6 +45,7 @@
         return PSS_ENOMEM;
     }
     cap = want;
+    ++gen;
     return PSS_OK;
 }
 
@@ -310,6 +311,7 @@
     PSS_HIP(hipHostMalloc(&c.pinned, c.pinned_cap, hipHostMallocDefault));
     PSS_HIP(hipHostGetDevicePointer(&c.pinned_dev, c.pinned, 0));
     for (hipEvent_t &e : c.search_ev) PSS_HIP(hipEventCreate(&e));
+    for (hipEvent_t &e : c.build_ev) PSS_HIP(hipEventCreate(&e));
     c.device = device;
     return PSS_OK;
 }
@@ -403,6 +405,7 @@
     {"PSS_MSD_NO_FUSE", "unset", "1", "MSD sort: ties flagged in the suffix array instead of emitted from the local sort"},
     {"PSS_MSD_NO_FINISH", "unset", "1", "MSD sort: small tie groups go to the rounds instead of being finished by one more text key after the local sort"},
     {"PSS_MSD_SLOW_LOCAL", "unset", "1", "MSD sort: the general (ballot LSD) local-sort kernel for every tile"},
+    {"PSS_MSD_HOST_TAIL", "unset", "1", "MSD sort in LSD order: finish, scan and gather launched by the host after its wait for the local sort (the sequence a declined tile takes) instead of standing behind it"},
     {"PSS_MSD_SCATTER", "unset", "1", "MSD sort in MSD order: the 8192-element partition kernels of round 2"},
     {"PSS_SS", "-1 (n >= 2^24, MSD declined)", "0|1", "initial sort: never / whenever the text has the size for it the sample sort over 16-byte elements"},
     {"PSS_SS_SEG", "1", "0", "sample sort: 0 = every tile merge-sorted as one array instead of bucket by bucket"},
diff --git a/pysubstringsearch_amd/csrc/common.h b/pysubstringsearch_amd/csrc/common.h
--- a/pysubstringsearch_amd/csrc/common.h
+++ b/pysubstringsearch_amd/csrc/common.h
@@ -42,6 +42,7 @@
 struct DevBuf {
     void *p = nullptr;
     size_t cap = 0;
+    uint64_t gen = 0;
     int reserve(size_t bytes);
     void release();
     template <typename T> T *as() const { return static_cast<T *>(p); }
@@ -112,6 +113,7 @@
     void *search_stage = nullptr;
     int ensure_search_stage();
     hipEvent_t search_ev[3] = {nullptr, nullptr, nullptr};
+    hipEvent_t build_ev[3] = {nullptr, nullptr, nullptr};
     void *small_hdr_ready = nullptr;
     struct Resident {
         hipStream_t stream = nullptr;
@@ -131,6 +133,7 @@
     uint32_t plan_logn = 0;
     int plan_path = 0;
     uint8_t plan_lut[256] = {};
+    uint64_t plan_lut_gen = 0;
     uint32_t plan_sigma = 0;
     uint64_t ss_plan_tag = 0;
     uint32_t ss_plan_radix = 0;
diff --git a/pysubstringsearch_amd/csrc/msd_sort.h b/pysubstringsearch_amd/csrc/msd_sort.h
--- a/pysubstringsearch_amd/csrc/msd_sort.h
+++ b/pysubstringsearch_amd/csrc/msd_sort.h
@@ -28,7 +28,7 @@
 struct MsdFront {
     const uint8_t *raw;
     const uint8_t *lut;
-    uint32_t *bad;
+    uint32_t pad0, pad1;
 };
 int msd_suffix_sort(DeviceCtx *ctx, const TextKeys *text, uint32_t n, int key_bits, uint64_t *A[2], uint32_t *sa_out,
                     void *work, uint32_t *h_small, bool profile, MsdStats *stats, bool *accepted, MsdActive *active = nullptr,
diff --git a/pysubstringsearch_amd/csrc/msd_sort.hip b/pysubstringsearch_amd/csrc/msd_sort.hip
--- a/pysubstringsearch_amd/csrc/msd_sort.hip
+++ b/pysubstringsearch_amd/csrc/msd_sort.hip
@@ -15,6 +15,7 @@
 constexpr int MSD_WAVES = MSD_BLOCK / kWave;
 constexpr int MSD_IPT = 16;
 constexpr u32 MSD_TILE = MSD_BLOCK * MSD_IPT;
+constexpr u32 MSD_TILE2 = 16384;
 constexpr u32 MSD_WIN = 6144;
 #ifndef PSS_LS_WINDOW
 #define PSS_LS_WINDOW 8
@@ -302,6 +303,93 @@
     if (d == 0) J1[MSD_BINS] = n;
 }
 
+__global__ __launch_bounds__(256) void msd_begin_kernel(u32 *zero, u32 words, u8 *codes_out, u32 pad0, u32 pad1)
+{
+    for (u32 i = threadIdx.x; i < words; i += 256) zero[i] = 0;
+    if (codes_out)
+        for (u32 i = pad0 + threadIdx.x; i < pad1; i += 256) codes_out[i] = 0;
+}
+
+__device__ __forceinline__ bool msd_plan_refused(const u32 *counters, const u32 *bad)
+{
+    return counters[1] > MSD_MAX_BUCKET || (bad && *bad);
+}
+__device__ __forceinline__ bool msd_tail_declined(const u32 *counters, const u32 *bad)
+{
+    return msd_plan_refused(counters, bad) || counters[4] != 0;
+}
+
+__global__ __launch_bounds__(256) void msd_prefix2_kernel(u32 *T, const u32 *T2, u32 num_ranges, u32 *totals)
+{
+    __shared__ u32 scr[256 / kWave + 1];
+    const u32 tid = threadIdx.x;
+    const bool second = blockIdx.x >= MSD_BINS;
+    const u32 d = second ? blockIdx.x - MSD_BINS : blockIdx.x;
+    u32 *row = T + (size_t)d * num_ranges;
+    const u32 *src = second ? T2 + (size_t)d * num_ranges : row;
+    u32 v[4], sum = 0;
+#pragma unroll
+    for (int j = 0; j < 4; ++j) {
+        const u32 r = tid * 4 + j;
+        v[j] = r < num_ranges ? src[r] : 0u;
+        sum += v[j];
+    }
+    u32 total = 0;
+    u32 run = block_excl_sum<256 / kWave>(sum, scr, &total);
+    if (!second) {
+#pragma unroll
+        for (int j = 0; j < 4; ++j) {
+            const u32 r = tid * 4 + j;
+            if (r < num_ranges) row[r] = run;
+            run += v[j];
+        }
+    }
+    if (tid == 0) totals[blockIdx.x] = total;
+}
+
+constexpr u32 MSD_STARTS_GRID = 32;
+__global__ __launch_bounds__(MSD_BINS) void msd_starts_kernel(const u32 *totals, u32 *J1, u32 *Jb, u32 n, MsdTile2 *tiles, u32 *counters)
+{
+    constexpr u32 TILE2 = MSD_TILE2;
+    constexpr u32 REGIONS = MSD_BINS / MSD_STARTS_GRID, TPR = MSD_BINS / REGIONS;
+    __shared__ u32 scr[MSD_BINS / kWave + 1];
+    __shared__ u32 s_start[MSD_BINS], s_cnt[MSD_BINS], s_first[MSD_BINS], s_dn[MSD_BINS];
+    const u32 d = threadIdx.x;
+    const u32 c = totals[d];
+    const u32 s = block_excl_sum<MSD_BINS / kWave>(c, scr, nullptr);
+    const u32 nr = (c + TILE2 - 1) / TILE2;
+    u32 total = 0, D = 0;
+    const u32 first = block_excl_sum<MSD_BINS / kWave>(nr, scr, &total);
+    const u32 dn = block_excl_sum<MSD_BINS / kWave>(nr ? 1u : 0u, scr, &D);
+    if (blockIdx.x == 0) {
+        J1[d] = s;
+        if (d == 0) {
+            J1[MSD_BINS] = n;
+            counters[0] = total + (MSD_BINS - D);
+        }
+    }
+    if (blockIdx.x == 1) {
+        Jb[d] = block_excl_sum<MSD_BINS / kWave>(totals[MSD_BINS + d], scr, nullptr);
+        if (d == 0) Jb[MSD_BINS] = n;
+    }
+    s_start[d] = s;
+    s_cnt[d] = c;
+    s_first[d] = first;
+    s_dn[d] = dn;
+    __syncthreads();
+    const u32 r = blockIdx.x * REGIONS + d / TPR, l = d % TPR;
+    const u32 rs = s_start[r], rc = s_cnt[r], rn = s_dn[r];
+    const u32 rnr = (rc + TILE2 - 1) / TILE2;
+    if (rnr == 0 && l == 0) {
+        const u32 dd = D + (r - rn);
+        tiles[total + (r - rn)] = MsdTile2{rs, 0u, dd | 0x80000000u};
+    }
+    for (u32 k = l; k < rnr; k += TPR) {
+        const u32 ts = rs + k * TILE2;
+        tiles[s_first[r] + k] = MsdTile2{ts, min(TILE2, rs + rc - ts), rn | (k + 1 == rnr ? 0x80000000u : 0u)};
+    }
+}
+
 __global__ __launch_bounds__(MSD_BINS) void msd_offsets_kernel(u32 *T, const u32 *seg_first, const u32 *seg_start, u32 *joint,
                                                                 u32 num_ranges_fixed, u32 n, u32 nseg)
 {
@@ -423,7 +511,6 @@
     }
 }
 
-constexpr u32 MSD_TILE2 = 16384;
 constexpr int MSD_PIECES2 = MSD_TILE2 / MSD_TILE;
 
 template <bool FROM_TEXT, int BLOCK, bool LSD = false>
@@ -608,25 +695,6 @@
 }
 
 
-__global__ __launch_bounds__(MSD_BINS) void msd_tiles2_kernel(const u32 *J1, MsdTile2 *tiles, u32 *counters)
-{
-    __shared__ u32 scr[MSD_BINS / kWave + 1];
-    const u32 d = threadIdx.x;
-    const u32 s = J1[d], e = J1[d + 1];
-    const u32 nr = (e - s + MSD_TILE2 - 1) / MSD_TILE2;
-    u32 total = 0, D = 0;
-    const u32 first = block_excl_sum<MSD_BINS / kWave>(nr, scr, &total);
-    const u32 dn = block_excl_sum<MSD_BINS / kWave>(nr ? 1u : 0u, scr, &D);
-    if (d == 0) counters[0] = total + (MSD_BINS - D);
-    if (nr == 0) {
-        const u32 dd = D + (d - dn);
-        tiles[total + (d - dn)] = MsdTile2{s, 0u, dd | 0x80000000u};
-    }
-    for (u32 k = 0; k < nr; ++k) {
-        const u32 ts = s + k * MSD_TILE2;
-        tiles[first + k] = MsdTile2{ts, min(MSD_TILE2, e - ts), dn | (k + 1 == nr ? 0x80000000u : 0u)};
-    }
-}
 
 __global__ __launch_bounds__(1024) void msd_scatter_lb_kernel(MsdArgs a)
 {
@@ -767,24 +835,62 @@
         return (k < ne && msd_tile_head(cstart, ne, n, (u32)k, tp)) ? 1u : 0u;
     }
 };
-__global__ __launch_bounds__(256) void msd_tiles_dev_kernel(const u32 *cstart, const u64 *nep, u32 n, const u64 *rank, const u64 *total,
-                                                              u32 *tile_first, TilePlan tp)
-{
-    const u32 ne = (u32)*nep;
+__global__ __launch_bounds__(256) void msd_tiles_kernel(const u32 *cstart, u32 ne, u32 n, const u64 *rank, const u64 *total,
+                                                          u32 *tile_first, TilePlan tp)
+{
     if (blockIdx.x == 0 && threadIdx.x == 0) tile_first[*total] = ne;
     for (u32 k = blockIdx.x * blockDim.x + threadIdx.x; k < ne; k += gridDim.x * blockDim.x) {
         if (msd_tile_head(cstart, ne, n, k, tp)) tile_first[rank[k]] = k;
     }
 }
 
-__global__ __launch_bounds__(256) void msd_tiles_kernel(const u32 *cstart, u32 ne, u32 n, const u64 *rank, const u64 *total,
-                                                          u32 *tile_first, TilePlan tp)
-{
-    if (blockIdx.x == 0 && threadIdx.x == 0) tile_first[*total] = ne;
-    for (u32 k = blockIdx.x * blockDim.x + threadIdx.x; k < ne; k += gridDim.x * blockDim.x) {
-        if (msd_tile_head(cstart, ne, n, k, tp)) tile_first[rank[k]] = k;
-    }
-}
+struct OutCompact {
+    const u32 *J;
+    u32 *cstart, *cj, *counters;
+    u64 *ne_out;
+    u32 mx;
+    __device__ void operator()(u64 j, u64 v, u64 rank)
+    {
+        if (v) {
+            const u32 s = J[j];
+            cstart[rank] = s;
+            cj[rank] = (u32)j;
+            mx = max(mx, J[j + 1] - s);
+        }
+    }
+    __device__ void flush()
+    {
+        const u32 m = wave_incl_max(mx);
+        if (lane_id() == kWave - 1 && m) atomicMax(&counters[1], m);
+        mx = 0;
+    }
+    __device__ void total(u64 ne) { *ne_out = ne; }
+};
+struct OutTileHeads {
+    const u64 *nep;
+    u32 *tile_first;
+    u64 *nt_out;
+    __device__ void operator()(u64 k, u64 v, u64 rank)
+    {
+        if (v) tile_first[rank] = (u32)k;
+    }
+    __device__ void flush() {}
+    __device__ void total(u64 nt)
+    {
+        tile_first[nt] = (u32)*nep;
+        *nt_out = nt;
+    }
+};
+struct OutBlkOff {
+    u64 *dst_off, *total_out;
+    __device__ void operator()(u64 t, u64 v, u64 ex) { dst_off[t] = ex; }
+    __device__ void flush() {}
+    __device__ void total(u64 sum) { *total_out = sum; }
+};
+struct GateTail {
+    const u32 *counters, *bad;
+    __device__ bool operator()() const { return !msd_tail_declined(counters, bad); }
+};
 
 struct MsdTile {
     u32 e0, count, tag0, nb;
@@ -833,14 +939,20 @@
 
 constexpr u32 GA_WORDS = MSD_TILE / 32;
 __global__ __launch_bounds__(256) void msd_gather_kernel(const MsdTile *tiles, const u32 *blk_cnt, const u64 *dst_off, u32 nt,
-                                                           const u32 *st_pos, const u32 *st_idx, u32 *pos, u32 *idx, u32 *grp)
+                                                           const u32 *st_pos, const u32 *st_idx, u32 *pos, u32 *idx, u32 *grp,
+                                                           const u64 *nt_dev, const u32 *counters_dev, const u32 *bad_dev)
 {
     __shared__ u32 s_occ[4][GA_WORDS], s_head[4][GA_WORDS], s_pre[4][GA_WORDS];
+    if (nt_dev) {
+        if (msd_tail_declined(counters_dev, bad_dev)) return;
+        nt = (u32)*nt_dev;
+    }
     const u32 w = wave_id(), lane = lane_id();
-    const u32 t = blockIdx.x * 4 + w;
-    if (t >= nt) return;
+    for (u32 t = blockIdx.x * 4 + w; t < nt; t += gridDim.x * 4) {
+    __builtin_amdgcn_fence(__ATOMIC_ACQ_REL, "wavefront");
+    __builtin_amdgcn_wave_barrier();
     const u32 c = blk_cnt[t] & 0xffffu;
-    if (c == 0) return;
+    if (c == 0) continue;
     const u32 e0 = tiles[t].e0;
     const u64 d = dst_off[t] & 0xffffffffull;
     u32 *occ = s_occ[w], *head = s_head[w], *pre = s_pre[w];
@@ -877,6 +989,7 @@
         idx[d + rank] = st_idx[e0 + i] & 0x7fffffffu;
         grp[d + rank] = e0 + hq + 1;
     }
+    }
 }
 
 
@@ -888,15 +1001,10 @@
     u32 h0, n;
 };
 
-__global__ __launch_bounds__(256) void msd_finish_kernel(const MsdTile *tiles, u32 *blk_cnt, u32 nt, u32 *st_pos, u32 *st_idx,
-                                                           u32 *sa_out, MsdFinish f)
-{
-    __shared__ u32 s_tie[4][FIN_WORDS], s_done[4][GA_WORDS];
-    const u32 w = wave_id(), lane = lane_id();
-    const u32 t = blockIdx.x * 4 + w;
-    if (t >= nt) return;
-    const u32 c = blk_cnt[t] & 0xffffu;
-    const u32 e0 = tiles[t].e0;
+__device__ __forceinline__ void msd_finish_tile(u32 *blk_cnt, u32 t, u32 c, u32 e0, u32 *st_pos, u32 *st_idx, u32 *sa_out,
+                                                const MsdFinish &f, u32 *tie, u32 *done)
+{
+    const u32 lane = lane_id();
     if (c == 0) return;
     u32 ps0 = 0, v0 = 0;
     if (lane < c) {
@@ -912,7 +1020,6 @@
             v = st_idx[e0 + i];
         }
     };
-    u32 *tie = s_tie[w], *done = s_done[w];
     for (u32 i = lane; i < FIN_WORDS; i += kWave) tie[i] = 0;
     for (u32 i = lane; i < GA_WORDS; i += kWave) done[i] = 0;
     __builtin_amdgcn_fence(__ATOMIC_ACQ_REL, "wavefront");
@@ -993,6 +1100,32 @@
         kept += (u32)__popcll(km);
     }
     if (lane == 0) blk_cnt[t] = kept | ((c - kept) << 16);
+}
+
+__global__ __launch_bounds__(256) void msd_finish_kernel(const MsdTile *tiles, u32 *blk_cnt, u32 nt, u32 *st_pos, u32 *st_idx,
+                                                           u32 *sa_out, MsdFinish f, const u64 *nt_dev, const u32 *counters_dev,
+                                                           const u32 *bad_dev)
+{
+    __shared__ u32 s_tie[4][FIN_WORDS], s_done[4][GA_WORDS];
+    if (nt_dev) {
+        if (msd_tail_declined(counters_dev, bad_dev)) return;
+        nt = (u32)*nt_dev;
+    }
+    const u32 w = wave_id();
+    const u32 stride = gridDim.x * 4;
+    u32 t = blockIdx.x * 4 + w;
+    if (t >= nt) return;
+    u32 c_next = blk_cnt[t], e_next = tiles[t].e0;
+    for (; t < nt; t += stride) {
+        const u32 c = c_next & 0xffffu, e0 = e_next;
+        if (t + stride < nt) {
+            c_next = blk_cnt[t + stride];
+            e_next = tiles[t + stride].e0;
+        }
+        __builtin_amdgcn_fence(__ATOMIC_ACQ_REL, "wavefront");
+        __builtin_amdgcn_wave_barrier();
+        msd_finish_tile(blk_cnt, t, c, e0, st_pos, st_idx, sa_out, f, s_tie[w], s_done[w]);
+    }
 }
 
 
@@ -1130,7 +1263,7 @@
                                                                      const u32 *counters_dev, const u32 *bad_dev)
 {
     if (nt_dev) {
-        if (counters_dev[1] > MSD_MAX_BUCKET || (bad_dev && *bad_dev)) return;
+        if (msd_plan_refused(counters_dev, bad_dev)) return;
         nt = (u32)*nt_dev;
     }
     const MsdEmit *em = fused ? &em_val : nullptr;
@@ -1357,6 +1490,10 @@
     return (size_t)n / (SS_WIN / 2) + ((size_t)MSD_BINS * MSD_BINS) / MSD_RAW_TAG_SPAN + 8;
 }
 
+constexpr u32 MSD_FETCH_WORDS = 32;
+constexpr u32 MSD_CHAIN_WORDS = 2 * 2048;
+constexpr u32 MSD_SMALL_WORDS = MSD_FETCH_WORDS + 3 * MSD_CHAIN_WORDS;
+
 static size_t msd_max_tiles2(uint32_t n) { return (size_t)n / MSD_TILE2 + MSD_BINS + 8; }
 
 static bool msd_use_lsd(uint32_t n)
@@ -1379,6 +1516,7 @@
            + (msd_max_tiles(n) + 32) * 16
            + (msd_max_tiles(n) + 32) * sizeof(MsdTile)
            + (SC_MAX_BLOCKS + 8) * 8 + 8192
+           + MSD_SMALL_WORDS * 4 + 2 * MSD_BINS * 4 + 512
            + (size_t)MSD_BINS * MSD_G1_RANGES * 4 + (MSD_BINS + 8) * 4
            + msd_max_tiles2(n) * (sizeof(MsdTile2) + (size_t)MSD_BINS * 4)
            + (nbk + 8) * 4 + 4096;
@@ -1414,7 +1552,15 @@
     u32 *J = reinterpret_cast<u32 *>(carve((nbk + 8) * 4));
     MsdRange *ranges2 = reinterpret_cast<MsdRange *>(carve(max_ranges2 * sizeof(MsdRange)));
     u32 *seg_first = reinterpret_cast<u32 *>(carve((MSD_BINS + 8) * 4));
-    u32 *counters = reinterpret_cast<u32 *>(carve(64));
+    u32 *small = reinterpret_cast<u32 *>(carve(MSD_SMALL_WORDS * 4));
+    u64 *const d_total = reinterpret_cast<u64 *>(small), *const d_total2 = d_total + 1, *const d_total3 = d_total + 2;
+    u32 *counters = small + 6;
+    u32 *d_bad = small + 22;
+    auto chain = [&](int i) {
+        u64 *st = reinterpret_cast<u64 *>(small + MSD_FETCH_WORDS + (size_t)i * MSD_CHAIN_WORDS);
+        return ScanChain{st, reinterpret_cast<u32 *>(st + MSD_CHAIN_WORDS / 2 - 1)};
+    };
+    u32 *totals = reinterpret_cast<u32 *>(carve(2 * MSD_BINS * 4));
     u64 *ranks = reinterpret_cast<u64 *>(carve((nbk + 8) * 8));
     u32 *cstart = reinterpret_cast<u32 *>(carve((nbk + 8) * 4));
     const size_t max_tiles = msd_max_tiles(n);
@@ -1423,7 +1569,6 @@
     u32 *blk_cnt = reinterpret_cast<u32 *>(carve((max_tiles + 8) * 4));
     u64 *dst_off = reinterpret_cast<u64 *>(carve((max_tiles + 8) * 8));
     u64 *partial = reinterpret_cast<u64 *>(carve((SC_MAX_BLOCKS + 8) * 8));
-    u64 *d_total = partial + SC_MAX_BLOCKS;
     const bool lsd = msd_use_lsd(n);
     const size_t max_tiles2 = msd_max_tiles2(n);
     u32 *T2 = nullptr, *Jb = nullptr, *status = nullptr, *cj = nullptr;
@@ -1480,24 +1625,30 @@
         return PSS_OK;
     };
 
-    PSS_HIP(hipMemsetAsync(counters, 0, 64, s));
+    if (scan_chain_words(std::max<u64>(nbk, max_tiles)) > MSD_CHAIN_WORDS / 2) {
+        set_error("msd_suffix_sort: %zu tiles do not fit the scan chains (internal error)", max_tiles);
+        return PSS_EDEVICE;
+    }
+    if (lsd) PSS_HIP(hipMemsetAsync(status, 0, max_tiles2 * MSD_BINS * 4, s));
+    hipLaunchKernelGGL(msd_begin_kernel, dim3(1), dim3(256), 0, s, small, MSD_SMALL_WORDS, front ? const_cast<u8 *>(text->codes) : (u8 *)nullptr,
+                       front ? front->pad0 : 0u, front ? front->pad1 : 0u);
     a.out = A[0];
     if (front) {
         a.raw = front->raw;
         a.lut = front->lut;
         a.codes_out = const_cast<u8 *>(text->codes);
-        a.bad = front->bad;
+        a.bad = d_bad;
         hipLaunchKernelGGL(msd_hist_raw_kernel, dim3(a.num_ranges1), dim3(MSD_BLOCK), 0, s, a);
     } else {
         hipLaunchKernelGGL(msd_hist_kernel<true>, dim3(a.num_ranges1), dim3(MSD_BLOCK), 0, s, a);
     }
-    static_assert(MSD_G1_RANGES <= 1024, "msd_offsets1_kernel takes four ranges per thread");
-    hipLaunchKernelGGL(msd_offsets1_kernel, dim3(MSD_BINS), dim3(256), 0, s, T, a.num_ranges1, seg_first);
-    hipLaunchKernelGGL(msd_offsets1b_kernel, dim3(1), dim3(MSD_BINS), 0, s, (const u32 *)seg_first, J1, n);
+    static_assert(MSD_G1_RANGES <= 1024, "msd_offsets1_kernel / msd_prefix2_kernel take four ranges per thread");
     if (lsd) {
-        hipLaunchKernelGGL(msd_offsets1_kernel, dim3(MSD_BINS), dim3(256), 0, s, T2, a.num_ranges1, seg_first);
-        hipLaunchKernelGGL(msd_offsets1b_kernel, dim3(1), dim3(MSD_BINS), 0, s, (const u32 *)seg_first, Jb, n);
-        PSS_HIP(hipMemsetAsync(status, 0, max_tiles2 * MSD_BINS * 4, s));
+        hipLaunchKernelGGL(msd_prefix2_kernel, dim3(2 * MSD_BINS), dim3(256), 0, s, T, (const u32 *)T2, a.num_ranges1, totals);
+        hipLaunchKernelGGL(msd_starts_kernel, dim3(MSD_STARTS_GRID), dim3(MSD_BINS), 0, s, (const u32 *)totals, J1, Jb, n, tiles2, counters);
+    } else {
+        hipLaunchKernelGGL(msd_offsets1_kernel, dim3(MSD_BINS), dim3(256), 0, s, T, a.num_ranges1, seg_first);
+        hipLaunchKernelGGL(msd_offsets1b_kernel, dim3(1), dim3(MSD_BINS), 0, s, (const u32 *)seg_first, J1, n);
     }
     PSS_TRY(mark());
     const bool wide = lsd || !(knob("PSS_MSD_SCATTER") && atoi(knob("PSS_MSD_SCATTER")) == 1);
@@ -1508,7 +1659,6 @@
     a.in = A[0];
     a.out = A[1];
     if (lsd) {
-        hipLaunchKernelGGL(msd_tiles2_kernel, dim3(1), dim3(MSD_BINS), 0, s, (const u32 *)J1, tiles2, counters);
         PSS_TRY(mark());
         const u32 grid2 = std::min<u32>((u32)max_tiles2, (u32)ctx->num_cus);
         hipLaunchKernelGGL(msd_scatter_lb_kernel, dim3(grid2), dim3(1024), 0, s, a);
@@ -1520,42 +1670,66 @@
         hipLaunchKernelGGL(msd_offsets_kernel, dim3(MSD_BINS), dim3(MSD_BINS), 0, s, T, (const u32 *)seg_first, (const u32 *)J1, J,
                            0u, n, MSD_BINS);
     }
-    PSS_TRY(device_excl_scan(ctx, InNonEmpty{J}, nbk, partial, d_total, ranks));
-    hipLaunchKernelGGL(msd_compact_kernel, dim3(1024), dim3(256), 0, s, J, (u32)nbk, ranks, cstart, counters, cj);
+    const bool one_trip = lsd && !knob("PSS_MSD_SLOW_LOCAL");
+    if (one_trip) {
+        PSS_TRY(device_excl_scan_chained(ctx, InNonEmpty{J}, OutCompact{J, cstart, cj, counters, d_total, 0u}, GateOpen{}, nbk,
+                                         (const u64 *)nullptr, chain(0), 4u * (u32)ctx->num_cus));
+    } else {
+        PSS_TRY(device_excl_scan(ctx, InNonEmpty{J}, nbk, partial, d_total, ranks));
+        hipLaunchKernelGGL(msd_compact_kernel, dim3(1024), dim3(256), 0, s, J, (u32)nbk, ranks, cstart, counters, cj);
+    }
     const int rem_bits = key_bits - 2 * MSD_D;
     MsdEmit em{};
     const int fused = active != nullptr;
     if (fused) em = MsdEmit{active->st_pos, active->st_idx, blk_cnt};
-    const bool one_trip = lsd && !knob("PSS_MSD_SLOW_LOCAL");
-    u64 *d_total2 = d_total + 1;
+    const bool finish = knob("PSS_MSD_NO_FINISH") == nullptr;
+    const bool host_tail = knob("PSS_MSD_HOST_TAIL") && atoi(knob("PSS_MSD_HOST_TAIL")) != 0;
+    MsdFinish fin{};
+    if (fused) {
+        const int ks = std::min(64 / text->code_bits, 16);
+        fin = MsdFinish{text->codes, text->code_bits, ks, text->plus_one, (u32)(text->drop ? text->key_chars - 1 : text->key_chars), n};
+    }
+    bool tail_enqueued = false;
+    const auto fetch = [&]() -> int {
+        PSS_HIP(hipMemcpyAsync(h_small, small, MSD_FETCH_WORDS * 4, hipMemcpyDeviceToHost, s));
+        PSS_HIP(hipStreamSynchronize(s));
+        return PSS_OK;
+    };
     u32 *const fail_list_dev = tile_first + max_tiles + 16;
     if (one_trip) {
         const TilePlan tpd{MSD_WIN, MSD_TILE_CAP, cj};
-        PSS_TRY(device_excl_scan(ctx, InTileHeadDev{cstart, d_total, n, tpd}, nbk, partial, d_total2, ranks));
-        hipLaunchKernelGGL(msd_tiles_dev_kernel, dim3(1024), dim3(256), 0, s, cstart, (const u64 *)d_total, n, ranks, (const u64 *)d_total2,
-                           tile_first, tpd);
+        PSS_TRY(device_excl_scan_chained(ctx, InTileHeadDev{cstart, d_total, n, tpd}, OutTileHeads{d_total, tile_first, d_total2}, GateOpen{},
+                                         nbk, (const u64 *)d_total, chain(1), 4u * (u32)ctx->num_cus));
         hipLaunchKernelGGL(msd_tile_desc_kernel, dim3((u32)((max_tiles + 255) / 256)), dim3(256), 0, s, cstart, tile_first, 0u, 0u, n,
                            tiles_all, (const u32 *)cj, (const u64 *)d_total2, (const u64 *)d_total);
         PSS_TRY(mark());
         hipLaunchKernelGGL(msd_local_fast_kernel, dim3(2u * (u32)ctx->num_cus), dim3(MSD_BLOCK), 0, s, A[1], (const MsdTile *)tiles_all, 0u,
                            rem_bits, ib, sa_out, fail_list_dev, counters + 4, fused, em, (const u64 *)d_total2, (const u32 *)counters,
-                           front ? (const u32 *)front->bad : (const u32 *)nullptr);
+                           (const u32 *)d_bad);
         PSS_TRY(mark());
-        PSS_HIP(hipMemcpyAsync(h_small + 8, d_total2, 8, hipMemcpyDeviceToHost, s));
-        PSS_HIP(hipMemcpyAsync(h_small + 10, counters + 4, 4, hipMemcpyDeviceToHost, s));
-    }
-    PSS_HIP(hipMemcpyAsync(h_small, d_total, 8, hipMemcpyDeviceToHost, s));
-    PSS_HIP(hipMemcpyAsync(h_small + 2, counters, 16, hipMemcpyDeviceToHost, s));
-    if (front) PSS_HIP(hipMemcpyAsync(h_small + 6, front->bad, 4, hipMemcpyDeviceToHost, s));
-    PSS_HIP(hipStreamSynchronize(s));
+        if (fused && !host_tail) {
+            const u32 grid_tail = 8u * (u32)ctx->num_cus;
+            if (finish)
+                hipLaunchKernelGGL(msd_finish_kernel, dim3(grid_tail), dim3(256), 0, s, (const MsdTile *)tiles_all, blk_cnt, 0u, active->st_pos,
+                                   active->st_idx, sa_out, fin, (const u64 *)d_total2, (const u32 *)counters, (const u32 *)d_bad);
+            PSS_TRY(device_excl_scan_chained(ctx, InBlkCnt{blk_cnt}, OutBlkOff{dst_off, d_total3}, GateTail{counters, d_bad}, max_tiles,
+                                             (const u64 *)d_total2, chain(2), 4u * (u32)ctx->num_cus));
+            hipLaunchKernelGGL(msd_gather_kernel, dim3(grid_tail), dim3(256), 0, s, (const MsdTile *)tiles_all, blk_cnt, dst_off, 0u,
+                               active->st_pos, active->st_idx, active->pos, active->idx, active->grp, (const u64 *)d_total2,
+                               (const u32 *)counters, (const u32 *)d_bad);
+            tail_enqueued = true;
+        }
+    }
+    PSS_TRY(fetch());
     const u32 ne = h_small[0];
-    const u32 maxb = h_small[3];
+    const u32 maxb = h_small[6 + 1];
+    const u32 bad_symbol = front ? h_small[22] : 0u;
     if (stats) {
         stats->buckets = ne;
         stats->max_bucket = maxb;
-        stats->bad_symbol = front ? h_small[6] : 0u;
-    }
-    if (front && h_small[6]) return PSS_OK;
+        stats->bad_symbol = bad_symbol;
+    }
+    if (bad_symbol) return PSS_OK;
     if (maxb > MSD_MAX_BUCKET) return PSS_OK;
     if (!lsd) {
         PSS_TRY(mark());
@@ -1568,22 +1742,23 @@
     u32 nt = 0;
     u32 *fail_list = fail_list_dev;
     if (one_trip) {
-        nt = h_small[8];
+        nt = h_small[2];
         if ((size_t)nt > max_tiles) {
             set_error("msd_suffix_sort: %u tiles planned, tables hold %zu (internal error)", nt, max_tiles);
             return PSS_EDEVICE;
         }
-        const u32 nfail = h_small[10];
+        const u32 nfail = h_small[6 + 4];
         if (stats) stats->slow_tiles = nfail;
-        if (nfail)
+        if (nfail) {
             hipLaunchKernelGGL(local_sort, dim3(nfail), dim3(MSD_BLOCK), 0, s, A[1], (const MsdTile *)tiles_all, rem_bits,
                                ib, sa_out, (const u32 *)fail_list, fused, em);
+            tail_enqueued = false;
+        }
     } else {
     const TilePlan tp{MSD_WIN, MSD_TILE_CAP, cj};
     PSS_TRY(device_excl_scan(ctx, InTileHead{cstart, ne, n, tp}, ne, partial, d_total, ranks));
     hipLaunchKernelGGL(msd_tiles_kernel, dim3(1024), dim3(256), 0, s, cstart, ne, n, ranks, (const u64 *)d_total, tile_first, tp);
-    PSS_HIP(hipMemcpyAsync(h_small, d_total, 8, hipMemcpyDeviceToHost, s));
-    PSS_HIP(hipStreamSynchronize(s));
+    PSS_TRY(fetch());
     nt = h_small[0];
     if ((size_t)nt > max_tiles) {
         set_error("msd_suffix_sort: %u tiles planned, tables hold %zu (internal error)", nt, max_tiles);
@@ -1602,9 +1777,8 @@
         hipLaunchKernelGGL(local_fast, dim3(grid), dim3(MSD_BLOCK), 0, s, A[1], (const MsdTile *)tiles, nt, rem_bits, ib,
                            sa_out, fail_list, counters + 4, fused, em, (const u64 *)nullptr, (const u32 *)nullptr, (const u32 *)nullptr);
         PSS_TRY(mark());
-        PSS_HIP(hipMemcpyAsync(h_small, counters + 4, 4, hipMemcpyDeviceToHost, s));
-        PSS_HIP(hipStreamSynchronize(s));
-        const u32 nfail = h_small[0];
+        PSS_TRY(fetch());
+        const u32 nfail = h_small[6 + 4];
         if (stats) stats->slow_tiles = nfail;
         if (nfail)
             hipLaunchKernelGGL(local_sort, dim3(nfail), dim3(MSD_BLOCK), 0, s, A[1], (const MsdTile *)tiles_all, rem_bits,
@@ -1612,22 +1786,19 @@
     }
     if (knob("PSS_MSD_SLOW_LOCAL")) PSS_TRY(mark());
     }
+    if (fused && !tail_enqueued) {
+        if (finish)
+            hipLaunchKernelGGL(msd_finish_kernel, dim3((nt + 3) / 4), dim3(256), 0, s, (const MsdTile *)tiles_all, blk_cnt, nt,
+                               active->st_pos, active->st_idx, sa_out, fin, (const u64 *)nullptr, (const u32 *)nullptr, (const u32 *)nullptr);
+        PSS_TRY(device_excl_scan(ctx, InBlkCnt{blk_cnt}, nt, partial, d_total3, dst_off));
+        hipLaunchKernelGGL(msd_gather_kernel, dim3((nt + 3) / 4), dim3(256), 0, s, (const MsdTile *)tiles_all, blk_cnt, dst_off, nt,
+                           active->st_pos, active->st_idx, active->pos, active->idx, active->grp, (const u64 *)nullptr,
+                           (const u32 *)nullptr, (const u32 *)nullptr);
+        PSS_TRY(fetch());
+    }
     if (fused) {
-        const bool finish = knob("PSS_MSD_NO_FINISH") == nullptr;
-        if (finish) {
-            const int ks = std::min(64 / text->code_bits, 16);
-            const MsdFinish fin{text->codes, text->code_bits, ks, text->plus_one,
-                                (u32)(text->drop ? text->key_chars - 1 : text->key_chars), n};
-            hipLaunchKernelGGL(msd_finish_kernel, dim3((nt + 3) / 4), dim3(256), 0, s, (const MsdTile *)tiles_all, blk_cnt, nt,
-                               active->st_pos, active->st_idx, sa_out, fin);
-        }
-        PSS_TRY(device_excl_scan(ctx, InBlkCnt{blk_cnt}, nt, partial, d_total, dst_off));
-        hipLaunchKernelGGL(msd_gather_kernel, dim3((nt + 3) / 4), dim3(256), 0, s, (const MsdTile *)tiles_all, blk_cnt, dst_off, nt,
-                           active->st_pos, active->st_idx, active->pos, active->idx, active->grp);
-        PSS_HIP(hipMemcpyAsync(h_small, d_total, 8, hipMemcpyDeviceToHost, s));
-        PSS_HIP(hipStreamSynchronize(s));
-        active->count = h_small[0];
-        if (stats) stats->finished = h_small[1];
+        active->count = h_small[4];
+        if (stats) stats->finished = h_small[5];
     }
     PSS_HIP(hipGetLastError());
     if (stats) {
diff --git a/pysubstringsearch_amd/csrc/sa_build.hip b/pysubstringsearch_amd/csrc/sa_build.hip
--- a/pysubstringsearch_amd/csrc/sa_build.hip
+++ b/pysubstringsearch_amd/csrc/sa_build.hip
@@ -252,9 +252,10 @@
     u32 *h_small = static_cast<u32 *>(ctx->pinned);
 
     BuildTimer timer;
-    PSS_HIP(hipEventCreate(&timer.ev0));
-    PSS_HIP(hipEventCreate(&timer.ev1));
-    PSS_HIP(hipEventCreate(&timer.ev_mid));
+    timer.own = false;
+    timer.ev0 = ctx->build_ev[0];
+    timer.ev1 = ctx->build_ev[1];
+    timer.ev_mid = ctx->build_ev[2];
     PSS_HIP(hipEventRecord(timer.ev0, s));
     if (ctx->restart_depth == 0) {
         ctx->restart_ms = 0.0;
@@ -381,13 +382,13 @@
     st.sigma = sigma;
     st.code_bits = (u32)b;
     st.key_chars = (u32)key_chars;
-    memcpy(h_small + 1024, lut, 256);
-    PSS_HIP(hipMemcpyAsync(d_lut, h_small + 1024, 256, hipMemcpyHostToDevice, s));
-    u32 *d_bad = d_counters + 44;
+    const uint64_t work_gen = ctx->slot[S_WORK].gen;
+    if (!(fronted && ctx->plan_lut_gen == work_gen)) {
+        ctx->plan_lut_gen = fronted ? work_gen : 0;
+        memcpy(h_small + 1024, lut, 256);
+        PSS_HIP(hipMemcpyAsync(d_lut, h_small + 1024, 256, hipMemcpyHostToDevice, s));
+    }
     if (front_any) {
-        const size_t tail0 = (size_t)n & ~(size_t)15;
-        PSS_HIP(hipMemsetAsync(codes + tail0, 0, n_pad - tail0, s));
-        PSS_HIP(hipMemsetAsync(d_bad, 0, 4, s));
     } else {
         hipLaunchKernelGGL(sa_recode_kernel, dim3(grid_stream), dim3(256), 0, s, T, n, (u32)n_pad, d_lut, codes);
         if (plain && knobs.side != 0 && knobs.anchor != 0 && ctx->side_plan_heff != 0 && ctx->side_plan_logn == logn &&
@@ -458,7 +459,7 @@
             act.grp = ctx->slot[S_GRP2].as<u32>();
             act.st_pos = reinterpret_cast<u32 *>(K[0]);
             act.st_idx = reinterpret_cast<u32 *>(K[0]) + n;
-            const MsdFront front{T, d_lut, d_bad};
+            const MsdFront front{T, d_lut, (uint32_t)((size_t)n & ~(size_t)15), (uint32_t)n_pad};
             PSS_TRY(msd_suffix_sort(ctx, &mk, n, kb, K, SA, ctx->slot[S_P0].p, h_small, profile, &ms, &accepted,
                                     knobs.no_msd_fuse ? nullptr : &act, front_any ? &front : nullptr));
             if (front_any && !accepted) {
@@ -580,6 +581,7 @@
         memcpy(ctx->plan_present, present_bits, 32);
         memcpy(ctx->plan_lut, lut, 256);
         ctx->plan_sigma = sigma;
+        ctx->plan_lut_gen = work_gen;
     }
     if (msd_done) {
     } else if (ties) PSS_TRY(suffix_sort_flags(ctx, K, V, n, key_bits0, &tk, work, &cur, profile, &ss));
diff --git a/pysubstringsearch_amd/csrc/sa_plan_impl.h b/pysubstringsearch_amd/csrc/sa_plan_impl.h
--- a/pysubstringsearch_amd/csrc/sa_plan_impl.h
+++ b/pysubstringsearch_amd/csrc/sa_plan_impl.h
@@ -143,8 +143,10 @@
 
 struct BuildTimer {
     hipEvent_t ev0 = nullptr, ev1 = nullptr, ev_mid = nullptr;
+    bool own = true;
     ~BuildTimer()
     {
+        if (!own) return;
         if (ev0) (void)hipEventDestroy(ev0);
         if (ev1) (void)hipEventDestroy(ev1);
         if (ev_mid) (void)hipEventDestroy(ev_mid);
diff --git a/pysubstringsearch_amd/csrc/scan.h b/pysubstringsearch_amd/csrc/scan.h
--- a/pysubstringsearch_amd/csrc/scan.h
+++ b/pysubstringsearch_amd/csrc/scan.h
@@ -90,4 +90,92 @@
     return PSS_OK;
 }
 
+constexpr u32 SC1_ITEMS = 4;
+constexpr u32 SC1_CHUNK = SC_BLOCK * SC1_ITEMS;
+constexpr u64 SC1_A = 1ull << 62, SC1_P = 2ull << 62, SC1_STATE = 3ull << 62, SC1_VALUE = SC1_A - 1ull;
+
+struct ScanChain {
+    u64 *state;
+    u32 *ticket;
+};
+inline size_t scan_chain_words(u64 n_max) { return (size_t)((n_max + SC1_CHUNK - 1) / SC1_CHUNK) + 1; }
+
+struct GateOpen {
+    __device__ bool operator()() const { return true; }
+};
+
+template <typename In, typename Out, typename Gate>
+__global__ __launch_bounds__(SC_BLOCK) void scan_chained_kernel(In in, Out out, Gate gate, u64 n_max, const u64 *n_dev, ScanChain ch)
+{
+    __shared__ u64 scr[SC_BLOCK / kWave];
+    __shared__ u64 s_carry;
+    __shared__ u32 s_ticket;
+    if (!gate()) return;
+    u64 n = n_max;
+    if (n_dev && *n_dev < n) n = *n_dev;
+    const u32 chunks = (u32)((n + SC1_CHUNK - 1) / SC1_CHUNK);
+    const u32 lane = (u32)lane_id();
+    for (;;) {
+        if (threadIdx.x == 0) s_ticket = atomicAdd(ch.ticket, 1u);
+        __syncthreads();
+        const u32 t = s_ticket;
+        if (t >= chunks) {
+            if (t == 0 && threadIdx.x == 0) out.total(0);
+            break;
+        }
+        const u64 i0 = (u64)t * SC1_CHUNK + (u64)threadIdx.x * SC1_ITEMS;
+        u64 v[SC1_ITEMS], sum = 0;
+#pragma unroll
+        for (u32 j = 0; j < SC1_ITEMS; ++j) {
+            v[j] = i0 + j < n ? in(i0 + j) : 0;
+            sum += v[j];
+        }
+        u64 tot;
+        const u64 ex = block_excl_sum64(sum, scr, &tot);
+        if (wave_id() == 0) {
+            u64 carry = 0;
+            if (t != 0) {
+                if (lane == 0) __hip_atomic_store(&ch.state[t], SC1_A | tot, __ATOMIC_RELAXED, __HIP_MEMORY_SCOPE_AGENT);
+                u32 p = t;
+                for (;;) {
+                    const u64 w = lane < p ? __hip_atomic_load(&ch.state[p - 1 - lane], __ATOMIC_RELAXED, __HIP_MEMORY_SCOPE_AGENT) : SC1_P;
+                    const u64 unready = __ballot((w & SC1_STATE) == 0);
+                    const u32 lim = unready ? (u32)__builtin_ctzll(unready) : 64u;
+                    const u64 pm = __ballot((w & SC1_STATE) == SC1_P) & (lim == 64u ? ~0ull : ((1ull << lim) - 1ull));
+                    const u32 take = pm ? (u32)__builtin_ctzll(pm) + 1u : lim;
+                    const u64 incl = wave_incl_sum64(lane < take ? (w & SC1_VALUE) : 0ull);
+                    carry += __shfl(incl, kWave - 1);
+                    if (pm) break;
+                    p -= take;
+                    if (take == 0) __builtin_amdgcn_s_sleep(1);
+                }
+            }
+            if (lane == 0) {
+                __hip_atomic_store(&ch.state[t], SC1_P | (carry + tot), __ATOMIC_RELAXED, __HIP_MEMORY_SCOPE_AGENT);
+                s_carry = carry;
+            }
+        }
+        __syncthreads();
+        const u64 carry = s_carry;
+        u64 run = carry + ex;
+#pragma unroll
+        for (u32 j = 0; j < SC1_ITEMS; ++j) {
+            if (i0 + j < n) out(i0 + j, v[j], run);
+            run += v[j];
+        }
+        out.flush();
+        if (t == chunks - 1 && threadIdx.x == 0) out.total(carry + tot);
+    }
 }
+
+template <typename In, typename Out, typename Gate>
+inline int device_excl_scan_chained(DeviceCtx *ctx, In in, Out out, Gate gate, u64 n_max, const u64 *n_dev, ScanChain ch, u32 max_blocks)
+{
+    u32 grid = (u32)((n_max + SC1_CHUNK - 1) / SC1_CHUNK);
+    grid = grid < 1 ? 1 : (grid > max_blocks ? max_blocks : grid);
+    hipLaunchKernelGGL((scan_chained_kernel<In, Out, Gate>), dim3(grid), dim3(SC_BLOCK), 0, ctx->stream, in, out, gate, n_max, n_dev, ch);
+    PSS_HIP(hipGetLastError());
+    return PSS_OK;
+}
+
+}
```
